# KirillKryukov/naf

Measured on AMD Instinct MI355X. Metric: unnaf GB/s (uncompressed bases out) on 100 GB synthetic FASTA, higher is better.
Workload: dtype u8; 1 GPU; unnaf decode of a 100.0 GB synthetic-ACGT FASTA archive on one GPU (the size BASELINE.json's metric is quoted on; configs[1] at 10 GB rides along as cfg10_*), 100 records, 80-col lines; archive made in-run by the GPU ennaf; .naf 24739662224 B -> FASTA 99999995684 B, text + archive + decoded text resident in HBM; parallelism=one archive, one GPU, no data-path collective

## Files before the change

naf_amd/csrc/ctx.h:

```cpp
#pragma once
#include "common.h"
#include "../../include/naf_gpu.h"
#include <hip/hip_runtime.h>
#include <stdio.h>
#include <stdarg.h>
#include <vector>
#include <functional>
#include <string>

struct ArenaChunk { u8 *base; size_t cap, used; };

struct KTime { const char *name; hipEvent_t a, b; };

#define ZSPLIT_MAX 8
struct ZSplit { int parts; hipEvent_t ev[ZSPLIT_MAX]; u64 out_end[ZSPLIT_MAX]; int done; void *status; };
struct FlatStream { u64 q0, A; };
#define FLAT_DECODED (~0ull)
struct ZFlat { const u8 *src; const FlatStream *si; u64 nslots; const u8 *sym; void *status; bool ready;
               const u8 *tail; u64 tail_q; u32 tail_n;
               const u8 *cls; u32 n_decoded; u32 n_walk;
               struct naf_gpu_ctx *aux; hipEvent_t decoded_ev; void *later; };
struct CtxOpts { std::vector<std::pair<std::string, std::string>> kv; std::string trace; bool tracing = false; };
struct naf_gpu_ctx {
    int device = 0;
    CtxOpts *opts = nullptr;
    naf_gpu_ctx *root = nullptr;
    hipStream_t stream = nullptr;
    bool own_stream = false;
    std::vector<ArenaChunk> chunks;
    size_t high_water = 0;
    u8 *h_stage = nullptr;
    size_t h_stage_cap = 0;
    void *d_predef = nullptr;
    void *d_seqctab = nullptr;
    char err[512] = {0};
    bool timing = false;
    std::vector<KTime> ktimes;
    std::vector<hipEvent_t> ev_pool;
    size_t ev_used = 0;
    std::vector<std::string> agg_names; std::vector<float> agg_ms; std::vector<int> agg_n;
    float stream_ms[5] = { 0, 0, 0, 0, 0 };
    naf_gpu_ctx *side = nullptr;
    naf_gpu_ctx *side2 = nullptr;
    naf_gpu_ctx *side3 = nullptr;
    naf_gpu_ctx *side4 = nullptr;
    void *sides_thread = nullptr; int sides_rc = 0;
    hipEvent_t fork_ev = nullptr;
    struct ZSplit *zsplit = nullptr;
    hipEvent_t split_ev[ZSPLIT_MAX + 2] = {};
    struct ZFlat *zflat = nullptr;
    void *io_pool = nullptr;
    void *shard_state = nullptr;
    struct HostWorker *worker = nullptr;
};

void ctx_worker_start(naf_gpu_ctx *x, std::function<void()> job);
void ctx_worker_join(naf_gpu_ctx *x);
int  ctx_sides_ready(naf_gpu_ctx *c);

int  ctx_fail(naf_gpu_ctx *c, int code, const char *fmt, ...);
const char *ctx_opt(const naf_gpu_ctx *c, const char *name);
static inline bool ctx_opt_is(const naf_gpu_ctx *c, const char *name, char v) { const char *e = ctx_opt(c, name); return e && e[0] == v; }
bool ctx_tracing(const naf_gpu_ctx *c);
void ctx_trace(naf_gpu_ctx *c, const char *fmt, ...);
#define HIP_TRY(c, call) do { hipError_t e_ = (call); if (e_ != hipSuccess) return ctx_fail((c), NAF_GPU_EHIP, "%s: %s (%s:%d)", #call, hipGetErrorString(e_), __FILE__, __LINE__); } while (0)

void  arena_reset(naf_gpu_ctx *c);
void *arena_alloc(naf_gpu_ctx *c, size_t bytes);
void  arena_settle(naf_gpu_ctx *c);
template <typename T> T *arena_new(naf_gpu_ctx *c, size_t n) { return (T *)arena_alloc(c, n * sizeof(T)); }

int ctx_readback(naf_gpu_ctx *c, void *h_dst, const void *d_src, size_t bytes);
int ctx_readback2(naf_gpu_ctx *c, void *h1, const void *d1, size_t n1, void *h2, const void *d2, size_t n2);
int ctx_readbackv(naf_gpu_ctx *c, int n, void *const *h, const void *const *d, const size_t *bytes);

void ktime_begin(naf_gpu_ctx *c, const char *name);
void ktime_end(naf_gpu_ctx *c);

#define LAUNCH(c, name, kern, grid, block, shmem, ...) do { \
    ktime_begin((c), name); \
    hipLaunchKernelGGL(kern, dim3(grid), dim3(block), (shmem), (c)->stream, __VA_ARGS__); \
    ktime_end((c)); } while (0)

static inline u32 cdiv(u64 a, u64 b) { return (u32)((a + b - 1) / b); }

int scan_exclusive_u64(naf_gpu_ctx *c, u64 *d_vals, size_t n, u64 *d_total);
int scan_inclusive_max_i32(naf_gpu_ctx *c, i32 *d_vals, size_t n);
int scan_inclusive_max_i64(naf_gpu_ctx *c, i64 *d_vals, size_t n);
int scan_exclusive_u64_multi(naf_gpu_ctx *c, u64 *const *arrs, int k, size_t n, u64 *const *totals);
int scan_inclusive_max_i64_multi(naf_gpu_ctx *c, i64 *const *arrs, int k, size_t n);

int zstd_decode(naf_gpu_ctx *c, const u8 *d_src, size_t src_len, int has_magic, u8 *d_dst, size_t dst_cap, size_t *out_len, const u8 *head = nullptr);
int zstd_init_tables(naf_gpu_ctx *c);
void ennaf_shard_state_free(naf_gpu_ctx *c);
void io_pool_free(naf_gpu_ctx *c);
struct EmitP;
int zstd_decode_fused_fasta(naf_gpu_ctx *c, const u8 *d_src, size_t src_len, int has_magic, size_t *out_len, const EmitP *P, u8 *text);
struct ZRange { u64 want_lo, want_hi, got_lo, got_hi; bool ranged; u8 *own_buf; };
int zstd_decode_range(naf_gpu_ctx *c, const u8 *d_src, size_t src_len, int has_magic, u8 *d_dst, size_t dst_cap, size_t *out_len, ZRange *rg, const u8 *head = nullptr);
int zstd_split_status(naf_gpu_ctx *c, const ZSplit *sp);
int zstd_flat_later(naf_gpu_ctx *c, ZFlat *zf);
void zstd_flat_drop(ZFlat *zf);
int zstd_small_batch(naf_gpu_ctx *c, int n, const u8 *const *src, const size_t *len, u8 *const *dst, const size_t *cap, bool *ok);
bool zstd_small_fits(size_t len, size_t cap);
int zstd_small_launch(naf_gpu_ctx *c, int n, const u8 *const *src, const size_t *len, u8 *const *dst, const size_t *cap, u32 **d_res_out);
enum { ZENC_PART = 16, ZENC_PART_FIRST = 32, ZENC_PART_LAST = 64, ZENC_PREFER_RAW = 128, ZENC_PREFER_FLAT = 256, ZENC_SHORT_CODES = 512, ZENC_FRAME_TREE = 1024 };
int zenc_level_window(int level);
int zenc_repeat_probe(naf_gpu_ctx *c, const u8 *d_src, size_t n, u32 *share_1024);
static inline u32 zenc_probe_every(u64 n) { u32 e = 64; while (((n >> 20) / e) > 128) e <<= 1; return e; }
struct ZencPlace { u8 *(*fn)(void *ud, size_t frame_len); void *ud; };
struct ZencJob;
#define ZENC_LOC_BND 20
struct ZencLoc { const u8 *loc; const i32 *blk_bnd; const u32 *blk_t0; u64 tiles; };
int zstd_encode_begin(naf_gpu_ctx *c, const u8 *d_src, size_t n, int level, int with_magic, int lz, int block_log_hint, int window_log, ZencJob **job, const u8 *direct = nullptr, u32 nd = 0, const ZencLoc *dloc = nullptr);
int zstd_encode_finish(naf_gpu_ctx *c, ZencJob *job, u8 *d_dst, size_t cap, size_t *out_len, const ZencPlace *place);
void zstd_encode_drop(ZencJob *job);
int zstd_encode_size(naf_gpu_ctx *c, ZencJob *job, size_t *frame_len);
const u64 *zstd_encode_total_ptr(const ZencJob *job);
void zstd_encode_set_total(ZencJob *job, u64 total);
int zstd_encode(naf_gpu_ctx *c, const u8 *d_src, size_t n, int level, u8 *d_dst, size_t cap, size_t *out_len, int with_magic, int lz = 0, int block_log_hint = 0, int window_log = 0, const ZencPlace *place = nullptr);
```

naf_amd/csrc/emit.hip:

```cpp
#include "ctx.h"
#include "wgscan.h"
#include "emit_core.h"
#include <thread>

__device__ __forceinline__ void st_text16(u8 *p, const uint4 &v, int nt)
{
    if (nt) {
        typedef unsigned int u32x4_t __attribute__((ext_vector_type(4)));
        u32x4_t nv; nv.x = v.x; nv.y = v.y; nv.z = v.z; nv.w = v.w;
        __builtin_nontemporal_store(nv, (u32x4_t *)p);
    } else *(uint4 *)p = v;
}

__global__ void k_len_flags(const u32 *units, u64 n, u64 *flag)
{
    u64 i = (u64)blockIdx.x * blockDim.x + threadIdx.x;
    if (i < n) flag[i] = units[i] != 0xFFFFFFFFu;
}
__global__ void k_len_acc(const u32 *units, u64 n, const u64 *ridx, u64 *rec_len, u64 N)
{
    u64 i = (u64)blockIdx.x * blockDim.x + threadIdx.x;
    if (i < n && ridx[i] < N) atomicAdd((unsigned long long *)&rec_len[ridx[i]], (unsigned long long)units[i]);
}

// ... 414 lines not shown
        if (k.qual_copy) { uint4 v; v.x = (u32)a; v.y = (u32)(a >> 32); v.z = (u32)b; v.w = (u32)(b >> 32); memcpy(o, &v, 16); return; }
        if (k.fast) {
            u64 lo, hi, g0 = k.g0;
            if (FOURBIT) { u64 nib = a; if (g0 & 1) nib = (nib >> 4) | (b << 60); expand16(P.lut, nib, lo, hi); }
            else {
                lo = a; hi = b;
                if (P.upper) {
                    auto up = [](u64 v) { u64 r = 0; for (int i = 0; i < 8; i++) { u32 c = (v >> (8 * i)) & 0xFF; if (c >= 'a' && c <= 'z') c -= 32; r |= (u64)c << (8 * i); } return r; };
                    lo = up(lo); hi = up(hi);
                }
            }
            if (any_toggle) {
                u64 kk = upper_bound_u64(P.toggles, klo, khi, g0);
                u32 state = (u32)(kk & 1), m16 = 0; u64 pos = g0;
                for (;;) {
                    u64 nxt = kk < khi ? P.toggles[kk] : ~0ull;
                    u64 end = nxt < g0 + 16 ? nxt : g0 + 16;
                    if (state && end > pos) m16 |= (u32)(((1u << (end - pos)) - 1) << (pos - g0));
                    if (nxt >= g0 + 16) break;
                    pos = nxt; state ^= 1; kk++;
                }
                lo += spread_bits8(m16 & 0xFF); hi += spread_bits8(m16 >> 8);
            } else if (P.masking && (klo & 1)) { lo += 0x2020202020202020ull; hi += 0x2020202020202020ull; }
            if (k.nl_b < 16) splice_newline(lo, hi, k.nl_b);
            u64 j15 = k.j0 + 15 - (15 > k.nl_b ? 1 : 0);
            if (j15 >= k.len) hi = (hi & 0x00FFFFFFFFFFFFFFull) | ((u64)'\n' << 56);
            uint4 v; v.x = (u32)lo; v.y = (u32)(lo >> 32); v.z = (u32)hi; v.w = (u32)(hi >> 32);
            memcpy(o, &v, 16);
            return;
        }
        for (u32 bb = 0; bb < k.nbytes; bb++) o[bb] = (u8)emit_byte<FOURBIT>(P, k.p0 + bb, rlo, rhi, klo, khi);
    };
    for (u64 tile = span_first; tile <= span_last; tile += 8192) {
        Chunk ka = prep(tile), kb = prep(tile + 4096);
        u64 a0, a1, b0, b1;
        fetch(ka, a0, a1); fetch(kb, b0, b1);
        finish(ka, a0, a1); finish(kb, b0, b1);
    }
}

#define ES_SPAN (32u * 1024u)
#define ES_CAP 1024

__device__ __forceinline__ void place16(u64 &lo, u64 &hi, u64 slo, u64 shi, u32 pos, u32 n)
{
    if (n <= 8) { shi = 0; slo &= low_bytes_mask((int)n); } else if (n < 16) shi &= low_bytes_mask((int)n - 8);
    if (pos == 0) { lo |= slo; hi |= shi; }
    else if (pos < 8) { lo |= slo << (8 * pos); hi |= (shi << (8 * pos)) | (slo >> (64 - 8 * pos)); }
    else if (pos == 8) hi |= slo;
    else hi |= slo << (8 * (pos - 8));
}

__device__ __forceinline__ void mask16_from(const u64 *tog, u32 n, u64 klo, u64 g0, u64 &lo, u64 &hi)
{
    u32 a = 0, b = n;
    while (a < b) { u32 mid = (a + b) >> 1; if (tog[mid] <= g0) a = mid + 1; else b = mid; }
    u32 kk = a, state = (u32)((klo + kk) & 1), m16 = 0; u64 pos = g0;
    for (;;) {
        u64 nxt = kk < n ? tog[kk] : ~0ull;
        u64 end = nxt < g0 + 16 ? nxt : g0 + 16;
        if (state && end > pos) m16 |= (u32)(((1u << (end - pos)) - 1) << (pos - g0));
        if (nxt >= g0 + 16) break;
        pos = nxt; state ^= 1; kk++;
    }
    lo += spread_bits8(m16 & 0xFF); hi += spread_bits8(m16 >> 8);
}
__device__ __forceinline__ void mask16(const EmitP &P, u64 klo, u64 khi, bool any_toggle, u64 g0, u64 &lo, u64 &hi)
{
    if (any_toggle) {
        if (khi - klo <= 0x7FFFFFFFull) mask16_from(P.toggles + klo, (u32)(khi - klo), klo, g0, lo, hi);
        else {
            u64 kk = upper_bound_u64(P.toggles, klo, khi, g0);
            u32 state = (u32)(kk & 1), m16 = 0; u64 pos = g0;
            for (;;) {
                u64 nxt = kk < khi ? P.toggles[kk] : ~0ull;
                u64 end = nxt < g0 + 16 ? nxt : g0 + 16;
                if (state && end > pos) m16 |= (u32)(((1u << (end - pos)) - 1) << (pos - g0));
                if (nxt >= g0 + 16) break;
                pos = nxt; state ^= 1; kk++;
            }
            lo += spread_bits8(m16 & 0xFF); hi += spread_bits8(m16 >> 8);
        }
    } else if (P.masking && (klo & 1)) { lo += 0x2020202020202020ull; hi += 0x2020202020202020ull; }
}

__device__ __forceinline__ void span_windows(const EmitP &P, u64 span_first, u64 span_last, u64 *sh)
{
    if (threadIdx.x < 2 && P.mode != EM_SEQ) {
        u64 p = threadIdx.x == 0 ? span_first : span_last;
        sh[threadIdx.x] = upper_bound_u64(P.rec_out, 0, P.N + 1, p) - 1;
    }
    __syncthreads();
    if (threadIdx.x < 2) {
        u64 k = 0;
        if (P.masking) {
            u64 g;
            if (P.mode == EM_SEQ) g = threadIdx.x == 0 ? span_first : span_last + 1;
            else g = threadIdx.x == 0 ? P.rec_base[sh[0]] : P.rec_base[sh[1] + 1];
            if (P.mode != EM_SEQ && threadIdx.x == 0) {
                u64 r = sh[0], off = span_first - P.rec_out[r], hl = P.hdr_len[r];
                if (off > hl) { u64 q = off - hl; u64 j = (P.mode == EM_FASTA && P.L) ? (q / (P.L + 1)) * P.L : (P.mode == EM_FASTQ ? 0 : q); if (j > P.rec_len[r]) j = P.rec_len[r]; g += j; }
            }
            k = upper_bound_u64(P.toggles, 0, P.n_toggles, g);
        }
        sh[2 + threadIdx.x] = k;
    }
    __syncthreads();
}

__global__ void k_hdr_len64(const u32 *hdr_len, u64 r0, u64 n, u64 *out)
{
    u64 i = (u64)blockIdx.x * blockDim.x + threadIdx.x;
    if (i < n) out[i] = hdr_len[r0 + i];
}
__device__ __forceinline__ void store_upto16(u8 *p, u64 lo, u64 hi, u32 n)
{
    if (n >= 16) { uint4 v; v.x = (u32)lo; v.y = (u32)(lo >> 32); v.z = (u32)hi; v.w = (u32)(hi >> 32); memcpy(p, &v, 16); return; }
    if (n & 8) { st64(p, lo); p += 8; lo = hi; }
    if (n & 4) { st32(p, (u32)lo); p += 4; lo >>= 32; }
    if (n & 2) { p[0] = (u8)lo; p[1] = (u8)(lo >> 8); p += 2; lo >>= 16; }
    if (n & 1) p[0] = (u8)lo;
}
template <u32 LANES = 16>
__device__ __forceinline__ void group_copy(u8 *dst, const u8 *src, u64 n, u32 g)
{
    for (u64 i = (u64)g * 16; i < n; i += LANES * 16) {
        u64 lo = ld64(src + i), hi = ld64(src + i + 8);
        store_upto16(dst + i, lo, hi, n - i < 16 ? (u32)(n - i) : 16u);
    }
}

__global__ __launch_bounds__(256) void k_hdr_build(EmitP P, u64 r0, u64 n, const u64 *hdr_off, u8 *text)
{
    u64 i = (u64)blockIdx.x * 32 + (threadIdx.x >> 3);
    u32 g = threadIdx.x & 7;
    if (i >= n) return;
    u64 r = r0 + i; u32 hl = P.hdr_len[r];
    u8 *o = text + hdr_off[i];
    u64 ids0 = 0, idl = 0, nm0 = 0, nml = 0;
    if (P.has_ids) { ids0 = r ? P.idz[r - 1] + 1 : 0; idl = P.idz[r] - ids0; }
    if (P.has_names) { nm0 = r ? P.nmz[r - 1] + 1 : 0; nml = P.nmz[r] - nm0; }
    if (g == 0) { o[0] = P.hdr_char; o[hl - 1] = '\n'; }
    if (P.has_ids) {
        group_copy<8>(o + 1, P.ids + ids0, idl, g);
        if (P.has_names && nml) { if (g == 0) o[1 + idl] = P.sep; group_copy<8>(o + 2 + idl, P.names + nm0, nml, g); }
    } else group_copy<8>(o + 1, P.names + nm0, nml, g);
}

template <bool FOURBIT, typename Geo>
__device__ __forceinline__ void compose_chunk(const EmitP &P, Geo &geo, u64 p0, u32 nbytes, u64 r, u64 klo, u64 khi, bool any_toggle, u32 Lp1_32, u8 *o)
{
    const bool hdrs = P.hdr_text != nullptr;
    u64 ro, rn, len, base, ho; u32 hl;
    geo(r, ro, rn, len, base, ho, hl);
    u64 lo = 0, hi = 0; u32 pos = 0;
    while (pos < nbytes) {
        u64 p = p0 + pos;
        while (p >= rn) { r++; geo(r, ro, rn, len, base, ho, hl); }
        u64 off = p - ro;
        const u8 *src = nullptr; u64 g = 0; bool is_bases = false;
        u64 n_main = 0; u32 tc = 0, n_tc = 0;
        if (off < hl) { src = P.hdr_text + ho + off; n_main = hl - off; }
        else {
            u64 q = off - hl;
            if (P.mode == EM_FASTQ) {
                if (q < len + 3) {
                    u64 skip = 0;
                    if (q < len) { is_bases = true; g = base + q; n_main = len - q; } else skip = q - len;
                    tc = 0x0A2B0Au >> (8 * (u32)skip); n_tc = 3 - (u32)skip;
                } else { src = P.qual + base + (q - len - 3); n_main = 2 * len + 3 - q; tc = '\n'; n_tc = 1; }
            } else {
                tc = '\n'; n_tc = 1;
                if (P.mode == EM_SEQUENCES || P.L == 0) { if (q < len) { is_bases = true; g = base + q; n_main = len - q; } }
                else {
                    u64 line, col;
                    if (Lp1_32 && (q >> 32) == 0) { u32 l32 = (u32)q / Lp1_32; line = l32; col = (u32)q - l32 * Lp1_32; }
                    else { line = q / (P.L + 1); col = q - line * (P.L + 1); }
                    u64 j = line * P.L + col;
                    if (col != P.L && j < len) { is_bases = true; g = base + j; n_main = len - j < P.L - col ? len - j : P.L - col; }
                }
            }
        }
        u32 rem = nbytes - pos;
        u32 n1 = n_main < rem ? (u32)n_main : rem;
        if (n1) {
            u64 slo, shi;
            if (is_bases) { bases16<FOURBIT>(P, g, slo, shi); if (P.mode != EM_FASTQ) mask16(P, klo, khi, any_toggle, g, slo, shi); }
            else if (!hdrs && off < hl) {
                slo = shi = 0;
                for (u32 b = 0; b < n1; b++) { u64 ch = header_char(P, r, off + b, hl); if (b < 8) slo |= ch << (8 * b); else shi |= ch << (8 * (b - 8)); }
            }
            else { slo = ld64(src); shi = n1 > 8 ? ld64(src + 8) : 0; }
            place16(lo, hi, slo, shi, pos, n1);
            pos += n1; rem -= n1;
        }
        if (n1 == n_main && rem && n_tc) { u32 n2 = n_tc < rem ? n_tc : rem; place16(lo, hi, tc, 0, pos, n2); pos += n2; }
    }
    if (nbytes == 16) { uint4 v; v.x = (u32)lo; v.y = (u32)(lo >> 32); v.z = (u32)hi; v.w = (u32)(hi >> 32); memcpy(o, &v, 16); }
    else for (u32 b = 0; b < nbytes; b++) o[b] = (u8)((b < 8 ? lo >> (8 * b) : hi >> (8 * (b - 8))) & 0xFF);
}

struct GeoGlobal {
    const EmitP &P;
    __device__ GeoGlobal(const EmitP &p) : P(p) {}
    __device__ __forceinline__ void operator()(u64 r, u64 &ro, u64 &rn, u64 &len, u64 &base, u64 &ho, u32 &hl) const
    { ro = P.rec_out[r]; rn = P.rec_out[r + 1]; len = P.rec_len[r]; base = P.rec_base[r]; hl = P.hdr_len[r]; ho = P.hdr_text ? P.hdr_off[r - P.hdr_r0] : 0; }
};

template <bool FOURBIT>
__global__ __launch_bounds__(256) void k_emit_short(EmitP P, u8 *out)
{
    __shared__ u64 sh[4];
    __shared__ u64 s_ro[ES_CAP + 1], s_len[ES_CAP], s_base[ES_CAP], s_ho[ES_CAP];
    __shared__ u32 s_hl[ES_CAP];
    u64 span_first = P.out_begin + (u64)blockIdx.x * ES_SPAN, span_last = span_first + ES_SPAN - 1;
    if (span_last >= P.out_end) span_last = P.out_end - 1;
    span_windows(P, span_first, span_last, sh);
    const u64 rlo = sh[0], rhi = sh[1], klo = sh[2], khi = sh[3];
    const bool any_toggle = P.masking && klo < khi;
    const u64 nrec = rhi - rlo + 1;
    const bool in_lds = nrec <= ES_CAP;
    const bool hdrs = P.hdr_text != nullptr;
    if (in_lds) {
        for (u32 i = threadIdx.x; i < (u32)nrec; i += 256) {
            u64 r = rlo + i; s_ro[i] = P.rec_out[r]; s_len[i] = P.rec_len[r]; s_base[i] = P.rec_base[r]; s_hl[i] = P.hdr_len[r];
            s_ho[i] = hdrs ? P.hdr_off[r - P.hdr_r0] : 0;
        }
        if (threadIdx.x == 0) s_ro[nrec] = P.rec_out[rhi + 1];
        __syncthreads();
    }
    const u32 Lp1_32 = (P.L + 1) >> 32 ? 0 : (u32)(P.L + 1);
    auto geo_lds = [&](u64 r, u64 &ro, u64 &rn, u64 &len, u64 &base, u64 &ho, u32 &hl) {
        u32 i = (u32)(r - rlo); ro = s_ro[i]; rn = s_ro[i + 1]; len = s_len[i]; base = s_base[i]; hl = s_hl[i]; ho = s_ho[i];
    };
    GeoGlobal geo_g(P);
    for (u64 tile = span_first; tile <= span_last; tile += 4096) {
        u64 p0 = tile + (u64)threadIdx.x * 16;
        if (p0 > span_last) continue;
        u32 nbytes = P.out_end - p0 < 16 ? (u32)(P.out_end - p0) : 16;
        u8 *o = out + (p0 - P.out_begin);
        if (in_lds) {
            u32 lo_ = 0, hi_ = (u32)nrec; while (lo_ < hi_) { u32 mid = (lo_ + hi_) >> 1; if (s_ro[mid] <= p0) lo_ = mid + 1; else hi_ = mid; }
            compose_chunk<FOURBIT>(P, geo_lds, p0, nbytes, rlo + lo_ - 1, klo, khi, any_toggle, Lp1_32, o);
        } else {
            u64 r = upper_bound_u64(P.rec_out, rlo, rhi + 1, p0) - 1;
            compose_chunk<FOURBIT>(P, geo_g, p0, nbytes, r, klo, khi, any_toggle, Lp1_32, o);
        }
    }
}

#define ER_STAGE 24576u
template <bool FOURBIT, u32 ER_LANES, u32 WGT>
__global__ __launch_bounds__(WGT) void k_emit_fastq_records(EmitP P, u8 *out)
{
    constexpr u32 ER_READS = WGT / ER_LANES, STAGE = ER_STAGE / (256u / WGT);
    __shared__ __attribute__((aligned(16))) u8 stage[STAGE + 32];
    const u32 g = threadIdx.x & (ER_LANES - 1);
    const u64 r0 = (u64)blockIdx.x * ER_READS, r = r0 + threadIdx.x / ER_LANES;
    const u64 rend = r0 + ER_READS < P.N ? r0 + ER_READS : P.N;
    const u64 wbase = P.rec_out[r0], wspan = P.rec_out[rend] - wbase;
    const bool in_lds = wspan <= STAGE;
    if (r < P.N) {
        const u64 len = P.rec_len[r], base = P.rec_base[r];
        const u32 hl = P.hdr_len[r];
        u8 *o = in_lds ? stage + (P.rec_out[r] - wbase) : out + P.rec_out[r];
        u64 ids0 = 0, idl = 0, nm0 = 0, nml = 0;
        if (P.has_ids) { ids0 = r ? P.idz[r - 1] + 1 : 0; idl = P.idz[r] - ids0; }
        if (P.has_names) { nm0 = r ? P.nmz[r - 1] + 1 : 0; nml = P.nmz[r] - nm0; }
        if (g == 0) { o[0] = P.hdr_char; o[hl - 1] = '\n'; }
        if (P.has_ids) {
            group_copy<ER_LANES>(o + 1, P.ids + ids0, idl, g);
            if (P.has_names && nml) { if (g == 0) o[1 + idl] = P.sep; group_copy<ER_LANES>(o + 2 + idl, P.names + nm0, nml, g); }
        } else group_copy<ER_LANES>(o + 1, P.names + nm0, nml, g);
        u8 *os = o + hl;
        for (u64 i = (u64)g * 16; i < len; i += 16 * ER_LANES) {
            u64 lo, hi; bases16<FOURBIT>(P, base + i, lo, hi);
            store_upto16(os + i, lo, hi, len - i < 16 ? (u32)(len - i) : 16u);
        }
        if (g == 0) { os[len] = '\n'; os[len + 1] = '+'; os[len + 2] = '\n'; os[2 * len + 3] = '\n'; }
        group_copy<ER_LANES>(os + len + 3, P.qual + base, len, g);
    }
    if (!in_lds) return;
    __syncthreads();
    u8 *dst = out + wbase; const u32 n = (u32)wspan;
    u32 head = (u32)((16 - ((uintptr_t)dst & 15)) & 15); if (head > n) head = n;
    if (threadIdx.x < head) dst[threadIdx.x] = stage[threadIdx.x];
    u32 words = (n - head) >> 4;
    for (u32 w = threadIdx.x; w < words; w += WGT) {
        u64 a, b2; __builtin_memcpy(&a, stage + head + 16 * w, 8); __builtin_memcpy(&b2, stage + head + 16 * w + 8, 8);
        uint4 v; v.x = (u32)a; v.y = (u32)(a >> 32); v.z = (u32)b2; v.w = (u32)(b2 >> 32);
        st_text16(dst + head + 16 * w, v, P.nt_store);
    }
    for (u32 k = head + 16 * words + threadIdx.x; k < n; k += WGT) dst[k] = stage[k];
}

#define EMIT_TOG_LDS 256u
struct TileIdx { u64 gline, k, khi; u32 col, fast; };
#define TI_HDR 0xFFFFFFFFu
struct TileFlat { u64 q0, A, q1, A1, q2, qf; };
struct TileFlatE { u64 base, a1_addr; u32 a1_sh, K0, K1, d1, d2, qoff, par0, pad; };
static_assert(sizeof(TileFlatE) == sizeof(TileFlat), "the derived record replaces the raw one in place");
#define FLAT_QM 4096
#define TILE_WG 255
__global__ __launch_bounds__(256) void k_tile_index(EmitP P, u64 ntiles, TileIdx *ti, u64 *tr, u32 *list, u32 *count, TileFlat *tsig, u32 spare, u32 *list2)
{
    __shared__ u64 s_k[256], s_r[256];
    const u64 t = (u64)blockIdx.x * TILE_WG + threadIdx.x;
    const u64 p = P.out_begin + t * 4096;
    TileIdx x; x.fast = 0; x.gline = 0; x.khi = 0; x.k = P.n_toggles; x.col = TI_HDR;
    TileFlat f; f.q0 = f.A = f.q1 = f.A1 = f.q2 = f.qf = 0;
    u64 r = ~0ull; u32 cbits = 1;
    const bool inside = t < ntiles && p < P.out_end;
    if (inside) {
        u64 g;
        if (P.mode == EM_SEQ) { r = 0; x.col = 0; g = p; x.gline = p; }
        else {
            r = upper_bound_u64(P.rec_out, 0, P.N + 1, p) - 1;
            u64 off = p - P.rec_out[r], hl = P.hdr_len[r], len = P.rec_len[r], j = 0;
            if (off >= hl) {
                u64 q = off - hl;
                if (P.mode == EM_FASTA && P.L) {
                    u64 line = q / (P.L + 1), col = q - line * (P.L + 1);
                    j = line * P.L + (col < P.L ? col : P.L);
                    if (P.L < 0xFFFFFFF0ull) { x.gline = P.rec_base[r] + line * P.L; x.col = (u32)col; }
                } else if (P.mode != EM_FASTQ) { j = q; x.col = 0; x.gline = P.rec_base[r] + q; }
                if (j > len) j = len;
            }
            g = P.rec_base[r] + j;
        }
        x.k = P.masking ? upper_bound_u64(P.toggles, 0, P.n_toggles, g) : 0;
        if (tsig) {
            const FlatStream *si = (const FlatStream *)P.fsi;
            const u64 q = g >> 1;
            u64 lo, hi, gs = q >> 13; if (gs >= P.fslots) gs = P.fslots - 1;
            if (si[gs].q0 <= q) { lo = gs; hi = gs + 1; u64 st = 1; while (hi < P.fslots && si[hi].q0 <= q) { lo = hi; st <<= 1; hi = lo + st; } if (hi > P.fslots) hi = P.fslots; }
            else { hi = gs; u64 st = 1; lo = gs - 1; while (lo > 0 && si[lo].q0 > q) { hi = lo; st <<= 1; lo = lo > st ? lo - st : 0; } }
            while (hi - lo > 1) { const u64 mid = (lo + hi) >> 1; if (si[mid].q0 <= q) lo = mid; else hi = mid; }
            f.q0 = si[lo].q0; f.A = si[lo].A; f.qf = q;
            if (P.fcls) {
                u32 c = 3; u64 b = lo >> 2; const u64 nb = P.fslots >> 2, qe = q + 2048 + 16;
                for (u32 k = 0; k < 6 && b < nb && si[4 * b].q0 <= qe; k++, b++) c &= P.fcls[b];
                if (b < nb && si[4 * b].q0 <= qe) c = 0;
                cbits = c;
            }
            u64 cs = lo + 1;
            while (cs < P.fslots && si[cs + 1].q0 == si[cs].q0) cs++;
            f.q1 = si[cs].q0; f.A1 = cs < P.fslots ? si[cs].A : 0;
            u64 ce = cs < P.fslots ? cs + 1 : cs;
            while (ce < P.fslots && si[ce + 1].q0 == si[ce].q0) ce++;
            f.q2 = si[ce].q0;
        }
    }
    s_k[threadIdx.x] = x.k; s_r[threadIdx.x] = r;
    __syncthreads();
    if (threadIdx.x == TILE_WG) return;
    TileFlatE e; e.base = (u64)P.fsrc; e.a1_addr = (u64)P.fsrc; e.a1_sh = 4; e.K0 = e.K1 = 0; e.d1 = e.d2 = 0x7FFFFFFFu; e.qoff = 0; e.par0 = 0; e.pad = 0;
    if (t >= ntiles) {
        if (t == ntiles) { tr[t] = ~0ull; ti[t] = x; if (tsig && spare) *(TileFlatE *)&tsig[t] = e; }
        else if (tsig && t < ntiles + spare) { ti[t].fast = 0; *(TileFlatE *)&tsig[t] = e; }
        return;
    }
    tr[t] = r;
    if (!inside) { ti[t] = x; if (tsig) *(TileFlatE *)&tsig[t] = e; list[atomicAdd(count, 1u)] = (u32)t; return; }
    const u64 r_next = s_r[threadIdx.x + 1];
    x.khi = s_k[threadIdx.x + 1];
    const bool wrap = P.mode == EM_FASTA && P.L != 0;
    bool fast = x.col != TI_HDR && r == r_next && P.out_begin + (t + 1) * 4096 <= P.out_end && !P.force_slow && (!wrap || P.L >= 16);
    bool packed = false;
    if (tsig) {
        packed = fast && (cbits & 2);
        if (fast && !(cbits & 1)) fast = false;
        if (fast) {
            fast = f.qf + 2048 + 16 < f.q2 || f.q2 == f.q1;
            if (P.ftail && f.qf + 2048 + 16 >= P.ftail_q) fast = false;
            if (f.q2 != f.q1 && (f.A1 > f.A ? f.A1 - f.A : f.A - f.A1) >= (1ull << 29)) fast = false;
        }
        if (fast) {
            const u64 gline = x.gline;
            const u64 dd1 = f.q1 - f.qf, dd2 = f.q2 - f.qf;
            e.d1 = dd1 > 0x7FFFFFFFull ? 0x7FFFFFFFu : (u32)dd1; e.d2 = dd2 > 0x7FFFFFFFull ? 0x7FFFFFFFu : (u32)dd2;
            const u64 T0 = f.A - 4 * (f.qf - f.q0), T1 = f.A1 + 4 * (u64)e.d1;
            const bool two = f.q2 != f.q1;
            const u64 tmin = two && T1 < T0 ? T1 : T0;
            const u64 ub = (tmin - 40 - 4 * (u64)FLAT_QM) & ~7ull;
            e.base = (u64)P.fsrc + (u64)((i64)ub >> 3);
            e.K0 = (u32)(T0 - 40 - ub); e.K1 = two ? (u32)(T1 - 40 - ub) : e.K0;
            e.qoff = (u32)((gline >> 1) - f.qf); e.par0 = (u32)gline & 1u;
            const u64 t1 = (f.A1 < 40 ? 40 : f.A1) - 40;
            e.a1_addr = (u64)P.fsrc + (t1 >> 3); e.a1_sh = (u32)(t1 & 7) + 4;
        }
        *(TileFlatE *)&tsig[t] = e;
    }
    x.fast = fast ? 1u : (packed ? 2u : 0u);
    ti[t] = x;
    if (!fast) { if (packed) list2[atomicAdd(count + 1, 1u)] = (u32)t; else list[atomicAdd(count, 1u)] = (u32)t; }
}

template <bool FOURBIT>
__device__ __forceinline__ void emit_tile_body(const EmitP &P, const TileIdx &a, u8 *out_tile)
{
    __shared__ u64 s_tog[EMIT_TOG_LDS];
    const u32 ntog = (u32)(a.khi - a.k < EMIT_TOG_LDS ? a.khi - a.k : EMIT_TOG_LDS);
    const bool use_tog = P.masking && a.k < a.khi && a.khi - a.k <= EMIT_TOG_LDS;
    if (use_tog) { for (u32 i = threadIdx.x; i < ntog; i += 256) s_tog[i] = P.toggles[a.k + i]; __syncthreads(); }
    const u32 lane16 = threadIdx.x * 16;
    u64 g0; u32 nl_b = 64;
    if (P.mode == EM_FASTA && P.L != 0) {
        const u32 Lp1 = (u32)P.L + 1;
        u32 c = a.col + lane16, dl;
        if (Lp1 < 32768) dl = __umulhi(c, P.Ldiv_magic); else dl = c >= Lp1 ? 1u : 0u;
        u32 col = c - dl * Lp1;
        g0 = a.gline + (u64)dl * (u32)P.L + col;
        u32 d = (u32)P.L - col;
        nl_b = d < 16 ? d : 64;
    } else g0 = a.gline + lane16;
    u64 lo, hi;
    if (FOURBIT) {
        u64 addr = (u64)P.seq + (g0 >> 1);
        const uint4 q = ldg_at<uint4>(addr & ~7ull);
        u64 q0 = (u64)q.x | ((u64)q.y << 32), q1 = (u64)q.z | ((u64)q.w << 32);
        u32 sh = (u32)(addr & 7) * 8 + (u32)(g0 & 1) * 4;
        expand16(P.lut, sh ? (q0 >> sh) | (q1 << (64 - sh)) : q0, lo, hi);
    } else bases16<false>(P, g0, lo, hi);
    if (use_tog) mask16_from(s_tog, ntog, a.k, g0, lo, hi);
    else mask16(P, a.k, a.khi, P.masking && a.k < a.khi, g0, lo, hi);
    if (nl_b < 16) splice_newline(lo, hi, (int)nl_b);
    uint4 v; v.x = (u32)lo; v.y = (u32)(lo >> 32); v.z = (u32)hi; v.w = (u32)(hi >> 32);
    st_text16(out_tile + lane16, v, P.nt_store);
}
template <bool FOURBIT>
__global__ __launch_bounds__(256) void k_emit_tile(EmitP P, const TileIdx *ti, u8 *out)
{
    const TileIdx a = ti[blockIdx.x];
    if (a.fast != 1) return;
    emit_tile_body<FOURBIT>(P, a, out + (u64)blockIdx.x * 4096);
}
template <bool FOURBIT, u32 TW>
__device__ __forceinline__ void emit_tiles_wave(const EmitP &P, const TileIdx *ti, u8 *out, const u64 (&tn)[TW], u32 want, u64 (*s_tog)[EMIT_TOG_LDS])
{
    const u32 lane = threadIdx.x;
    TileIdx A[TW]; bool live[TW];
#pragma unroll
    for (u32 j = 0; j < TW; j++) { A[j] = ti[tn[j] == ~0ull ? 0 : tn[j]]; live[j] = tn[j] != ~0ull && A[j].fast == want; }
    u64 g0s[TW][4]; u32 nls[TW][4]; uint4 Q[TW][4];
#pragma unroll
    for (u32 j = 0; j < TW; j++) {
        const TileIdx &a = A[j];
#pragma unroll
        for (u32 r = 0; r < 4; r++) {
            const u32 lane16 = (r * 64 + lane) * 16;
            u64 g0; u32 nl_b = 64;
            if (P.mode == EM_FASTA && P.L != 0) {
                const u32 Lp1 = (u32)P.L + 1;
                u32 c = a.col + lane16, dl;
                if (Lp1 < 32768) dl = __umulhi(c, P.Ldiv_magic); else dl = c >= Lp1 ? 1u : 0u;
                u32 col = c - dl * Lp1;
                g0 = a.gline + (u64)dl * (u32)P.L + col;
                u32 d = (u32)P.L - col;
                nl_b = d < 16 ? d : 64;
            } else g0 = a.gline + lane16;
            g0s[j][r] = g0; nls[j][r] = nl_b;
            if (FOURBIT) Q[j][r] = live[j] ? ldg_at<uint4>(((u64)P.seq + (g0 >> 1)) & ~7ull) : make_uint4(0, 0, 0, 0);
        }
    }
    if (P.masking) {
#pragma unroll
        for (u32 j = 0; j < TW; j++) {
            const u64 nt = A[j].khi - A[j].k;
            for (u32 i = lane; i < EMIT_TOG_LDS; i += 64) s_tog[j][i] = (live[j] && i < nt && nt <= EMIT_TOG_LDS) ? P.toggles[A[j].k + i] : 0ull;
        }
        __syncthreads();
    }
#pragma unroll
    for (u32 j = 0; j < TW; j++) {
        if (!live[j]) continue;
        const TileIdx &a = A[j];
        const u32 ntog = (u32)(a.khi - a.k < EMIT_TOG_LDS ? a.khi - a.k : EMIT_TOG_LDS);
        const bool use_tog = P.masking && a.k < a.khi && a.khi - a.k <= EMIT_TOG_LDS;
#pragma unroll
        for (u32 r = 0; r < 4; r++) {
            const u64 g0 = g0s[j][r];
            u64 lo, hi;
            if (FOURBIT) {
                const u64 addr = (u64)P.seq + (g0 >> 1);
                const uint4 q = Q[j][r];
                const u64 q0 = (u64)q.x | ((u64)q.y << 32), q1 = (u64)q.z | ((u64)q.w << 32);
                const u32 sh = (u32)(addr & 7) * 8 + (u32)(g0 & 1) * 4;
                expand16(P.lut, sh ? (q0 >> sh) | (q1 << (64 - sh)) : q0, lo, hi);
            } else bases16<false>(P, g0, lo, hi);
            if (use_tog) mask16_from(s_tog[j], ntog, a.k, g0, lo, hi);
            else mask16(P, a.k, a.khi, P.masking && a.k < a.khi, g0, lo, hi);
            if (nls[j][r] < 16) splice_newline(lo, hi, (int)nls[j][r]);
            uint4 v; v.x = (u32)lo; v.y = (u32)(lo >> 32); v.z = (u32)hi; v.w = (u32)(hi >> 32);
            st_text16(out + tn[j] * 4096 + (r * 64 + lane) * 16, v, P.nt_store);
        }
    }
}
template <bool FOURBIT, u32 TW>
__global__ __launch_bounds__(64) void k_emit_tile_wave(EmitP P, const TileIdx *ti, u8 *out, u64 ntiles)
{
    __shared__ u64 s_tog[TW][EMIT_TOG_LDS];
    u64 tn[TW];
#pragma unroll
    for (u32 j = 0; j < TW; j++) { const u64 t = (u64)blockIdx.x * TW + j; tn[j] = t < ntiles ? t : ~0ull; }
    emit_tiles_wave<FOURBIT, TW>(P, ti, out, tn, 1u, s_tog);
}
template <bool FOURBIT>
__global__ __launch_bounds__(64) void k_emit_tile_list_wave(EmitP P, const TileIdx *ti, const u32 *list, const u32 *count, u8 *out)
{
    __shared__ u64 s_tog[1][EMIT_TOG_LDS];
    const u32 n = *count;
    for (u32 i = blockIdx.x; i < n; i += gridDim.x) {
        const u64 tn[1] = { list[i] };
        emit_tiles_wave<FOURBIT, 1>(P, ti, out, tn, 2u, s_tog);
        __syncthreads();
    }
}
template <bool FOURBIT>
__global__ __launch_bounds__(256) void k_emit_tile_list(EmitP P, const TileIdx *ti, const u32 *list, const u32 *count, u8 *out)
{
    const u32 n = *count;
    for (u32 i = blockIdx.x; i < n; i += gridDim.x) {
        const u32 t = list[i];
        const TileIdx a = ti[t];
        emit_tile_body<FOURBIT>(P, a, out + (u64)t * 4096);
        __syncthreads();
    }
}

__global__ void k_flat_pair(EmitP P, u32 *pair)
{
    const u32 t = threadIdx.x;
    {
        const u32 pa = P.fsym[t >> 4], pb = P.fsym[t & 15];
        pair[16 + t] = expand_codes4(P.lut, (pa & 15u) | ((pa >> 4) << 8) | ((pb & 15u) << 16) | ((pb >> 4) << 24));
        if (t < 16) {
            const u32 d = t; u32 sel[4], orv[4];
            for (u32 i = 0; i < 4; i++) {
                sel[i] = 0; orv[i] = 0;
                for (u32 j = 0; j < 4; j++) { const u32 q = 4 * i + j; sel[i] |= (q < d ? 4 + j : (q == d ? 0x0Cu : 3 + j)) << (8 * j); if (q == d) orv[i] |= 0x0Au << (8 * j); }
            }
            for (u32 i = 0; i < 4; i++) { pair[272 + 8 * d + i] = sel[i]; pair[272 + 8 * d + 4 + i] = orv[i]; }
        }
    }
    if (t >= 12) return;
    const u8 *lut = (const u8 *)P.lut;
    u32 v = 0;
    for (u32 k = 0; k < 4; k++) {
        const u32 pk = P.fsym[4 * (t & 3) + k];
        const u32 b = t < 4 ? pk : (t < 8 ? lut[pk & 15] : lut[pk >> 4]);
        v |= b << (8 * k);
    }
    pair[t] = v;
}
#define FLAT_TPW 8
template <u32 TPW>
__global__ __launch_bounds__(256) void k_emit_tile_flat(EmitP P, const TileIdx *ti, const TileFlat *tsig, u8 *out, u64 ntiles, u32 xcd_chunk)
{
    u32 wg = blockIdx.x;
    if (xcd_chunk) { wg = (blockIdx.x & 7u) * xcd_chunk + (blockIdx.x >> 3); if ((u64)wg * TPW >= ntiles) return; }
    __shared__ u64 s_tog[TPW][EMIT_TOG_LDS];
    __shared__ uint4 s_spl[32];
    if (threadIdx.x < 16) {
        const u32 d = threadIdx.x; u32 sel[4], orv[4];
        for (u32 i = 0; i < 4; i++) {
            sel[i] = 0; orv[i] = 0;
            for (u32 j = 0; j < 4; j++) { const u32 p = 4 * i + j; sel[i] |= (p < d ? 4 + j : (p == d ? 0x0Cu : 3 + j)) << (8 * j); if (p == d) orv[i] |= 0x0Au << (8 * j); }
        }
        s_spl[2 * d] = make_uint4(sel[0], sel[1], sel[2], sel[3]); s_spl[2 * d + 1] = make_uint4(orv[0], orv[1], orv[2], orv[3]);
    }
    __shared__ u32 s_pair[256];
    {
        const u32 pa = P.fsym[threadIdx.x >> 4], pb = P.fsym[threadIdx.x & 15];
        s_pair[threadIdx.x] = expand_codes4(P.lut, (pa & 15u) | ((pa >> 4) << 8) | ((pb & 15u) << 16) | ((pb >> 4) << 24));
    }
    const u32 lane16 = threadIdx.x * 16;
    TileIdx A[TPW]; TileFlatE F[TPW]; bool live[TPW];
    {
        static_assert(sizeof(TileIdx) == 32 && sizeof(TileFlatE) == 48, "records are read as 16-byte words");
        const u64 t0 = (u64)wg * TPW;
        const uint4 *pa = (const uint4 *)(ti + t0), *pf = (const uint4 *)(tsig + t0);
        uint4 ra[2 * TPW], rf[3 * TPW];
#pragma unroll
        for (u32 i = 0; i < 2 * TPW; i++) ra[i] = pa[i];
#pragma unroll
        for (u32 i = 0; i < 3 * TPW; i++) rf[i] = pf[i];
#pragma unroll
        for (u32 j = 0; j < TPW; j++) {
            __builtin_memcpy(&A[j], &ra[2 * j], 32); __builtin_memcpy(&F[j], &rf[3 * j], 48);
            live[j] = t0 + j < ntiles && A[j].fast == 1;
        }
    }
    u64 X[TPW]; u32 offs[TPW], grels[TPW], nls[TPW], haves[TPW];
#pragma unroll
    for (u32 j = 0; j < TPW; j++) {
        const TileIdx &a = A[j]; const TileFlatE &e = F[j];
        u32 grel, nl_b = 64;
        if (P.mode == EM_FASTA && P.L != 0) {
            const u32 Lp1 = (u32)P.L + 1;
            u32 c = a.col + lane16, dl;
            if (Lp1 < 32768) dl = __umulhi(c, P.Ldiv_magic); else dl = c >= Lp1 ? 1u : 0u;
            u32 col = c - dl * Lp1;
            grel = dl * (u32)P.L + col;
            u32 d = (u32)P.L - col;
            nl_b = d < 16 ? d : 64;
        } else grel = lane16;
        grels[j] = grel; nls[j] = nl_b;
        const u32 par = e.par0 + grel;
        const u32 need = 8 + (par & 1u);
        const u32 qrel = (par >> 1) + e.qoff;
        const bool second = qrel >= e.d1;
        const u32 qm = live[j] ? ~0u : 0u;
        const u32 off = (second ? e.K1 : e.K0) - ((4 * qrel) & qm);
        const u32 rem = (second ? e.d2 : e.d1) - qrel;
        X[j] = ldg_at_unaligned<u64>(e.base + (off >> 3));
        offs[j] = off;
        haves[j] = need > rem ? rem : 16u;
    }
    if (P.masking) {
        u64 tg[TPW];
#pragma unroll
        for (u32 j = 0; j < TPW; j++) {
            const u64 nt = A[j].khi - A[j].k;
            tg[j] = (live[j] && threadIdx.x < nt && nt <= EMIT_TOG_LDS) ? P.toggles[A[j].k + threadIdx.x] : 0ull;
        }
#pragma unroll
        for (u32 j = 0; j < TPW; j++) s_tog[j][threadIdx.x] = tg[j];
    }
    __syncthreads();
#pragma unroll
    for (u32 j = 0; j < TPW; j++) {
        const u64 t = (u64)wg * TPW + j;
        if (!live[j]) continue;
        const TileIdx &a = A[j];
        const u64 g0 = a.gline + grels[j];
        u64 h36 = X[j] >> ((offs[j] & 7) + 4);
        if (haves[j] < 9) {
            const u64 y = ldg_at_unaligned<u64>(F[j].a1_addr);
            const u64 n36 = (y >> F[j].a1_sh) & 0xFFFFFFFFFull;
            const u32 keep = 4 * haves[j];
            h36 = (h36 & ~(0xFFFFFFFFFull >> keep)) | (n36 >> keep);
        }
        const u32 h = (u32)(h36 >> 4), n9 = (u32)h36 & 15u;
        u64 lo, hi;
        {
            u32 w0 = s_pair[h >> 24], w1 = s_pair[(h >> 16) & 0xFFu], w2 = s_pair[(h >> 8) & 0xFFu], w3 = s_pair[h & 0xFFu];
            if (g0 & 1) {
                const u32 c9 = s_pair[n9 << 4];
                w0 = __builtin_amdgcn_alignbyte(w1, w0, 1); w1 = __builtin_amdgcn_alignbyte(w2, w1, 1);
                w2 = __builtin_amdgcn_alignbyte(w3, w2, 1); w3 = __builtin_amdgcn_alignbyte(c9, w3, 1);
            }
            lo = (u64)w0 | ((u64)w1 << 32); hi = (u64)w2 | ((u64)w3 << 32);
        }
        const u32 ntog = (u32)(a.khi - a.k < EMIT_TOG_LDS ? a.khi - a.k : EMIT_TOG_LDS);
        const bool use_tog = P.masking && a.k < a.khi && a.khi - a.k <= EMIT_TOG_LDS;
        if (use_tog) mask16_from(s_tog[j], ntog, a.k, g0, lo, hi);
        else mask16(P, a.k, a.khi, P.masking && a.k < a.khi, g0, lo, hi);
        uint4 v; v.x = (u32)lo; v.y = (u32)(lo >> 32); v.z = (u32)hi; v.w = (u32)(hi >> 32);
        if (nls[j] < 16) {
            const uint4 sel = s_spl[2 * nls[j]], orv = s_spl[2 * nls[j] + 1];
            const u32 x0 = v.x, x1 = v.y, x2 = v.z, x3 = v.w;
            v.x = __builtin_amdgcn_perm(x0, 0u, sel.x) | orv.x; v.y = __builtin_amdgcn_perm(x1, x0, sel.y) | orv.y;
            v.z = __builtin_amdgcn_perm(x2, x1, sel.z) | orv.z; v.w = __builtin_amdgcn_perm(x3, x2, sel.w) | orv.w;
        }
        st_text16(out + t * 4096 + lane16, v, P.nt_store);
    }
}

template <u32 TW>
__global__ __launch_bounds__(64) void k_emit_tile_flat_wave(EmitP P, const TileIdx *ti, const TileFlat *tsig, u8 *out, u64 ntiles, u32 xcd_chunk)
{
    u32 wg = blockIdx.x;
    if (xcd_chunk) { wg = (blockIdx.x & 7u) * xcd_chunk + (blockIdx.x >> 3); if ((u64)wg * TW >= ntiles) return; }
    __shared__ u64 s_tog[TW][EMIT_TOG_LDS];
    __shared__ uint4 s_spl[32];
    __shared__ u32 s_pair[256];
    const u32 lane = threadIdx.x;
    if (lane < 32) s_spl[lane] = ((const uint4 *)(P.fpair + 272))[lane];
    ((uint4 *)s_pair)[lane] = ((const uint4 *)(P.fpair + 16))[lane];
    TileIdx A[TW]; TileFlatE F[TW]; bool live[TW];
    {
        const u64 t0 = (u64)wg * TW;
        const uint4 *pa = (const uint4 *)(ti + t0), *pf = (const uint4 *)(tsig + t0);
        uint4 ra[2 * TW], rf[3 * TW];
#pragma unroll
        for (u32 i = 0; i < 2 * TW; i++) ra[i] = pa[i];
#pragma unroll
        for (u32 i = 0; i < 3 * TW; i++) rf[i] = pf[i];
#pragma unroll
        for (u32 j = 0; j < TW; j++) {
            __builtin_memcpy(&A[j], &ra[2 * j], 32); __builtin_memcpy(&F[j], &rf[3 * j], 48);
            live[j] = t0 + j < ntiles && A[j].fast == 1;
        }
    }
    u64 X[TW][4]; u32 grels[TW][4], pk[TW][4];
#pragma unroll
    for (u32 j = 0; j < TW; j++) {
        const TileIdx &a = A[j]; const TileFlatE &e = F[j];
#pragma unroll
        for (u32 r = 0; r < 4; r++) {
            const u32 lane16 = (r * 64 + lane) * 16;
            u32 grel, nl_b = 64;
            if (P.mode == EM_FASTA && P.L != 0) {
                const u32 Lp1 = (u32)P.L + 1;
                u32 c = a.col + lane16, dl;
                if (Lp1 < 32768) dl = __umulhi(c, P.Ldiv_magic); else dl = c >= Lp1 ? 1u : 0u;
                u32 col = c - dl * Lp1;
                grel = dl * (u32)P.L + col;
                u32 d = (u32)P.L - col;
                nl_b = d < 16 ? d : 64;
            } else grel = lane16;
            grels[j][r] = grel;
            const u32 par = e.par0 + grel;
            const u32 need = 8 + (par & 1u);
            const u32 qrel = (par >> 1) + e.qoff;
            const bool second = qrel >= e.d1;
            const u32 qm = live[j] ? ~0u : 0u;
            const u32 off = (second ? e.K1 : e.K0) - ((4 * qrel) & qm);
            const u32 rem = (second ? e.d2 : e.d1) - qrel;
            X[j][r] = ldg_at_unaligned<u64>(e.base + (off >> 3));
            pk[j][r] = nl_b | ((need > rem ? rem : 16u) << 8) | ((off & 7u) << 16);
        }
    }
    if (P.masking) {
#pragma unroll
        for (u32 j = 0; j < TW; j++) {
            const u64 nt = A[j].khi - A[j].k;
            for (u32 i = lane; i < EMIT_TOG_LDS; i += 64) s_tog[j][i] = (live[j] && i < nt && nt <= EMIT_TOG_LDS) ? P.toggles[A[j].k + i] : 0ull;
        }
    }
    __syncthreads();
#pragma unroll
    for (u32 j = 0; j < TW; j++) {
        const u64 t = (u64)wg * TW + j;
        if (!live[j]) continue;
        const TileIdx &a = A[j];
        const u32 ntog = (u32)(a.khi - a.k < EMIT_TOG_LDS ? a.khi - a.k : EMIT_TOG_LDS);
        const bool use_tog = P.masking && a.k < a.khi && a.khi - a.k <= EMIT_TOG_LDS;
#pragma unroll
        for (u32 r = 0; r < 4; r++) {
            const u64 g0 = a.gline + grels[j][r];
            const u32 nl = pk[j][r] & 0xFFu, have = (pk[j][r] >> 8) & 0xFFu;
            u64 h36 = X[j][r] >> ((pk[j][r] >> 16) + 4);
            if (have < 9) {
                const u64 y = ldg_at_unaligned<u64>(F[j].a1_addr);
                const u64 n36 = (y >> F[j].a1_sh) & 0xFFFFFFFFFull;
                const u32 keep = 4 * have;
                h36 = (h36 & ~(0xFFFFFFFFFull >> keep)) | (n36 >> keep);
            }
            const u32 h = (u32)(h36 >> 4), n9 = (u32)h36 & 15u;
            u64 lo, hi;
            {
                u32 w0 = s_pair[h >> 24], w1 = s_pair[(h >> 16) & 0xFFu], w2 = s_pair[(h >> 8) & 0xFFu], w3 = s_pair[h & 0xFFu];
                if (g0 & 1) {
                    const u32 c9 = s_pair[n9 << 4];
                    w0 = __builtin_amdgcn_alignbyte(w1, w0, 1); w1 = __builtin_amdgcn_alignbyte(w2, w1, 1);
                    w2 = __builtin_amdgcn_alignbyte(w3, w2, 1); w3 = __builtin_amdgcn_alignbyte(c9, w3, 1);
                }
                lo = (u64)w0 | ((u64)w1 << 32); hi = (u64)w2 | ((u64)w3 << 32);
            }
            if (use_tog) mask16_from(s_tog[j], ntog, a.k, g0, lo, hi);
            else mask16(P, a.k, a.khi, P.masking && a.k < a.khi, g0, lo, hi);
            uint4 v; v.x = (u32)lo; v.y = (u32)(lo >> 32); v.z = (u32)hi; v.w = (u32)(hi >> 32);
            if (nl < 16) {
                const uint4 sel = s_spl[2 * nl], orv = s_spl[2 * nl + 1];
                const u32 x0 = v.x, x1 = v.y, x2 = v.z, x3 = v.w;
                v.x = __builtin_amdgcn_perm(x0, 0u, sel.x) | orv.x; v.y = __builtin_amdgcn_perm(x1, x0, sel.y) | orv.y;
                v.z = __builtin_amdgcn_perm(x2, x1, sel.z) | orv.z; v.w = __builtin_amdgcn_perm(x3, x2, sel.w) | orv.w;
            }
            st_text16(out + t * 4096 + (r * 64 + lane) * 16, v, P.nt_store);
        }
    }
}

template <bool FOURBIT>
__device__ __forceinline__ void emit_rest_tile(const EmitP &P, const TileIdx *ti, const u64 *tr, u64 t, u8 *out, u32 chunk)
{
    const TileIdx a = ti[t];
    u64 p0 = P.out_begin + t * 4096 + chunk * 16;
    if (p0 >= P.out_end) return;
    u32 nbytes = P.out_end - p0 < 16 ? (u32)(P.out_end - p0) : 16;
    const u32 Lp1_32 = (P.L + 1) >> 32 ? 0 : (u32)(P.L + 1);
    u8 *o = out + (p0 - P.out_begin);
    if (P.mode == EM_SEQ) {
        for (u32 bb = 0; bb < nbytes; bb++) o[bb] = (u8)emit_byte<FOURBIT>(P, p0 + bb, 0, 0, a.k, a.khi);
        return;
    }
    u64 rlo = tr[t], rhi = tr[t + 1] == ~0ull ? P.N - 1 : tr[t + 1];
    u64 r = upper_bound_u64(P.rec_out, rlo, rhi + 1, p0) - 1;
    GeoGlobal geo_g(P);
    compose_chunk<FOURBIT>(P, geo_g, p0, nbytes, r, a.k, a.khi, P.masking && a.k < a.khi, Lp1_32, o);
}
#define EMIT_REST_GRID 4096
template <bool FOURBIT>
__global__ __launch_bounds__(64) void k_emit_rest(EmitP P, const TileIdx *ti, const u64 *tr, const u32 *list, const u32 *count, u8 *out)
{
    const u32 n = *count;
    for (u32 i = blockIdx.x; i < 4 * n; i += gridDim.x) emit_rest_tile<FOURBIT>(P, ti, tr, list[i >> 2], out, (i & 3) * 64 + threadIdx.x);
}

__global__ void k_range_bases(EmitP P, u64 *out2)
{
    if (threadIdx.x || blockIdx.x) return;
    if (P.mode == EM_SEQ) { out2[0] = P.out_begin; out2[1] = P.out_end; out2[2] = out2[3] = 0; return; }
    u64 pb = P.out_begin, pe = P.out_end - 1;
    u64 r0 = upper_bound_u64(P.rec_out, 0, P.N + 1, pb) - 1, r1 = upper_bound_u64(P.rec_out, 0, P.N + 1, pe) - 1;
    out2[2] = r0; out2[3] = r1;
    auto lower = [&](u64 r, u64 p) -> u64 {
        u64 off = p - P.rec_out[r], hl = P.hdr_len[r], len = P.rec_len[r];
        if (off <= hl) return 0;
        u64 q = off - hl, j;
        if (P.mode == EM_FASTQ) j = 0;
        else if (P.mode == EM_FASTA && P.L) j = (q / (P.L + 1)) * P.L;
        else j = q;
        return j > len ? len : j;
    };
    auto upper = [&](u64 r, u64 p) -> u64 {
        u64 off = p - P.rec_out[r], hl = P.hdr_len[r], len = P.rec_len[r];
        if (off < hl) return 0;
        u64 q = off - hl, j;
        if (P.mode == EM_FASTQ) j = len;
        else if (P.mode == EM_FASTA && P.L) j = (q / (P.L + 1) + 1) * P.L;
        else j = q + 1;
        return j > len ? len : j;
    };
    out2[0] = P.rec_base[r0] + lower(r0, pb);
    out2[1] = P.rec_base[r1] + upper(r1, pe);
}

__global__ void k_last_nonempty(const u64 *rec_len, u64 N, unsigned long long *out)
{
    u64 r = (u64)blockIdx.x * blockDim.x + threadIdx.x;
    if (r < N && rec_len[r]) atomicMax(out, (unsigned long long)(r + 1));
}
template <bool FOURBIT>
__global__ void k_emit_surplus(EmitP P, u64 base0, u64 S, u64 cc, u64 L, int wrap, u64 lo, u64 hi, u8 *out)
{
    const u64 j = lo + (u64)blockIdx.x * blockDim.x + threadIdx.x;
    if (j >= hi) return;
    u64 g; bool nl = false;
    if (!wrap || L == 0 || S <= cc) g = base0 + j;
    else if (j < cc) g = base0 + j;
    else if (j == cc) { nl = true; g = 0; }
    else { const u64 j2 = j - cc - 1, line = j2 / (L + 1), col = j2 - line * (L + 1); if (col == L) { nl = true; g = 0; } else g = base0 + cc + line * L + col; }
    u32 ch = '\n';
    if (!nl) { ch = base_char<FOURBIT>(P, g); if (P.masking && base_masked(P, g, 0, P.n_toggles)) ch += 32; }
    out[j - lo] = (u8)ch;
}

static int zero_positions(naf_gpu_ctx *c, const u8 *d_buf, u64 n, u64 N, u64 **out, bool names)
{
    u64 *pos = arena_new<u64>(c, N + 1);
    if (!pos) return NAF_GPU_ENOMEM;
    u64 tiles = (n + ZT_TILE - 1) / ZT_TILE;
    u64 *cnt = arena_new<u64>(c, tiles + 2);
    if (!cnt) return NAF_GPU_ENOMEM;
    u64 *d_total = cnt + tiles + 1;
    if (tiles) LAUNCH(c, "unnaf_zero_count", k_zero_count, tiles, 256, 0, d_buf, n, cnt);
    int rc = scan_exclusive_u64(c, cnt, tiles, d_total); if (rc) return rc;
    u64 total = 0;
    rc = ctx_readback(c, &total, d_total, 8); if (rc) return rc;
    if (total < N) return ctx_fail(c, NAF_GPU_EFORMAT, names ? "corrupted names - can't read name %llu\n" : "currupted ids - can't read id %llu\n", (unsigned long long)total);
    if (tiles) LAUNCH(c, "unnaf_zero_scatter", k_zero_scatter, tiles, 256, 0, d_buf, n, (const u64 *)cnt, pos, N);
    *out = pos;
    return 0;
}

enum { H_OK = 0, H_EMPTY, H_TRUNC, H_MAGIC, H_VERSION, H_SEQTYPE, H_SEPARATOR, H_VLE_LEAD, H_VLE_OVERFLOW, H_SANE_SECTION , H_SANE_COUNT = H_SANE_SECTION + 6 };
struct ContainerOut { naf_gpu_header h; int code; u8 frame_head[6][24]; };
NAF_HD int naf_parse_container(const u8 *p, size_t len, naf_gpu_header *h)
{
    size_t pos = 0;
    memset(h, 0, sizeof *h);
    if (len == 0) return H_EMPTY;
    if (len < 3) return H_TRUNC;
    if (p[0] != 0x01 || p[1] != 0xF9 || p[2] != 0xEC) return H_MAGIC;
    pos = 3;
    if (pos >= len) return H_TRUNC;
    h->version = p[pos++];
    if (h->version < 1 || h->version > 2) return H_VERSION;
    h->seq_type = NAF_SEQ_DNA;
    if (h->version > 1) {
        if (pos >= len) return H_TRUNC;
        int t = p[pos++];
        h->seq_type = t;
        if (t < 1 || t > 3) return H_SEQTYPE;
    }
    if (len - pos < 2) return H_TRUNC;
    h->flags = p[pos++]; h->separator = p[pos++];
    if (h->separator < 0x20 || h->separator > 0x7E) return H_SEPARATOR;
    int e = 0;
    auto rd = [&](u64 *v) -> int {
        u64 a = 0; if (pos >= len) return H_TRUNC;
        u8 ch = p[pos++];
        if (ch == 128) return H_VLE_LEAD;
        while (ch & 128) { if (a & (127ull << 57)) return H_VLE_OVERFLOW; a = (a << 7) | (ch & 127); if (pos >= len) return H_TRUNC; ch = p[pos++]; }
        if (a & (127ull << 57)) return H_VLE_OVERFLOW;
        *v = (a << 7) | ch; return 0;
    };
    if ((e = rd(&h->line_length)) || (e = rd(&h->n_sequences))) return e;
    if (h->flags & 0x40) { if ((e = rd(&h->title_len))) return e; h->title_off = pos; if (h->title_len > len - pos) return H_TRUNC; pos += h->title_len; }
    const int bit[6] = { 0x20, 0x10, 0x08, 0x04, 0x02, 0x01 };
    for (int i = 0; i < 6; i++) {
        if (!(h->flags & bit[i])) continue;
        if ((e = rd(&h->orig_size[i])) || (e = rd(&h->comp_size[i]))) return e;
        if (h->comp_size[i] > len - pos) return H_TRUNC;
        h->payload_off[i] = pos; pos += h->comp_size[i];
    }
    for (int i = 0; i < 6; i++) {
        const u64 cs = h->comp_size[i] + 4;
        const u64 lim = cs > (1ull << 46) ? ~0ull : cs << (i == 4 ? 17 : 16);
        if (h->orig_size[i] > lim) return H_SANE_SECTION + i;
    }
    if (h->n_sequences > ((u64)len << 16)) return H_SANE_COUNT;
    return H_OK;
}
static void container_error_text(int code, const naf_gpu_header *h, char *buf, size_t cap)
{
    static const char *what[6] = { "can't decompress ids\n", "can't decompress names\n", "can't decompress lengths\n", "can't decompress mask\n",
                                   "can't decompress sequence\n", "can't decompress quality\n" };
    switch (code) {
    case H_EMPTY: snprintf(buf, cap, "empty input"); break;
    case H_TRUNC: snprintf(buf, cap, "incomplete or truncated input\n"); break;
    case H_MAGIC: snprintf(buf, cap, "not a NAF format\n"); break;
    case H_VERSION: snprintf(buf, cap, "unknown version (%d) of NAF format\n", h->version); break;
    case H_SEQTYPE: snprintf(buf, cap, "unknown sequence type (%d) found in NAF file\n", h->seq_type); break;
    case H_SEPARATOR: snprintf(buf, cap, "unsupported name separator character\n"); break;
    case H_VLE_LEAD: snprintf(buf, cap, "invalid input: error parsing variable length encoded number\n"); break;
    case H_VLE_OVERFLOW: snprintf(buf, cap, "invalid input: overflow reading a variable length encoded number\n"); break;
    case H_SANE_COUNT: snprintf(buf, cap, "corrupted header: more sequences than the archive can describe\n"); break;
    default: if (code >= H_SANE_SECTION && code < H_SANE_SECTION + 6) snprintf(buf, cap, "%s", what[code - H_SANE_SECTION]); else snprintf(buf, cap, "malformed NAF header\n");
    }
}

extern "C" int naf_gpu_parse_header_host(const void *h_naf, size_t len, naf_gpu_header *h, char errbuf[128])
{
    if (!h) return NAF_GPU_EARG;
    const int code = naf_parse_container((const u8 *)h_naf, len, h);
    if (!code) return 0;
    if (errbuf) container_error_text(code, h, errbuf, 128);
    return NAF_GPU_EFORMAT;
}

__global__ void k_parse_container(const u8 *d, u64 len, ContainerOut *out)
{
    if (threadIdx.x || blockIdx.x) return;
    out->code = naf_parse_container(d, (size_t)len, &out->h);
    for (int i = 0; i < 6; i++) {
        const u64 n = out->code ? 0 : (out->h.comp_size[i] < 24 ? out->h.comp_size[i] : 24);
        for (u64 k = 0; k < 24; k++) out->frame_head[i][k] = k < n ? d[out->h.payload_off[i] + k] : 0;
    }
}

static int parse_container_device(naf_gpu_ctx *c, const void *d_naf, size_t len, ContainerOut *co)
{
    ContainerOut *d_co = arena_new<ContainerOut>(c, 1); if (!d_co) return NAF_GPU_ENOMEM;
    LAUNCH(c, "unnaf_parse_container", k_parse_container, 1, 64, 0, (const u8 *)d_naf, (u64)len, d_co);
    int rc = ctx_readback(c, co, d_co, sizeof *co); if (rc) return rc;
    if (co->code) { char buf[160]; container_error_text(co->code, &co->h, buf, sizeof buf); return ctx_fail(c, NAF_GPU_EFORMAT, "%s", buf); }
    return 0;
}

extern "C" int naf_gpu_parse_header(naf_gpu_ctx *c, const void *d_naf, size_t len, naf_gpu_header *h)
{
    if (!c || !h) return NAF_GPU_EARG;
    arena_reset(c);
    ContainerOut co;
    int rc = parse_container_device(c, d_naf, len, &co);
    *h = co.h;
    return rc;
}

enum { S_IDS = 0, S_NAMES, S_LEN, S_MASK, S_SEQ, S_QUAL };

struct UnnafPlan {
    naf_gpu_header h; u8 frame_head[6][24]; EmitP P; u64 total; bool fourbit; bool empty;
    u64 seq_bytes; bool need_qual;
    u64 main_total, surplus, sur_c, sur_base0;
};

static int load_section(naf_gpu_ctx *c, const u8 *d_naf, const naf_gpu_header &h, int i, u64 expect, const char *what, u8 **out, const u8 *head = nullptr)
{
    u8 *buf = (u8 *)arena_alloc(c, expect + 32);
    if (!buf) return NAF_GPU_ENOMEM;
    size_t n = 0;
    int rc = zstd_decode(c, d_naf + h.payload_off[i], h.comp_size[i], 0, buf, expect, &n, head);
    if (rc == NAF_GPU_ECAP || (rc == 0 && n != expect)) return ctx_fail(c, NAF_GPU_EFORMAT, "can't decompress %s\n", what);
    if (rc) return rc;
    *out = buf;
    return 0;
}

static int unnaf_prepare(naf_gpu_ctx *c, const u8 *d_naf, size_t naf_len, const naf_gpu_unnaf_opts *o, UnnafPlan &pl)
{
    ContainerOut co;
    int rc = parse_container_device(c, d_naf, naf_len, &co); if (rc) return rc;
    pl.h = co.h; memcpy(pl.frame_head, co.frame_head, sizeof pl.frame_head);
    const naf_gpu_header &h = pl.h;
    EmitP &P = pl.P; memset(&P, 0, sizeof P);
    int has_mask = (h.flags >> 2) & 1, has_data = (h.flags >> 1) & 1, has_qual = h.flags & 1;
    int mode = o->out_type == NAF_OUT_DEFAULT ? (has_qual ? NAF_OUT_FASTQ : NAF_OUT_FASTA) : o->out_type;
    pl.empty = false; pl.total = 0; pl.need_qual = false; pl.main_total = pl.surplus = pl.sur_c = pl.sur_base0 = 0;
    pl.fourbit = h.seq_type <= NAF_SEQ_RNA;
    u64 N = h.n_sequences, T = h.orig_size[S_SEQ];
    pl.seq_bytes = pl.fourbit ? (T + 1) / 2 : T;
    if (N == 0 || !has_data) { pl.empty = true; return 0; }
    if (mode == NAF_OUT_FASTQ && !has_qual) return ctx_fail(c, NAF_GPU_EFORMAT, "FASTQ output requested, but input has no qualities\n");
    if (mode == NAF_OUT_4BIT) {
        if (!pl.fourbit) return ctx_fail(c, NAF_GPU_EFORMAT, "input has no 4-bit encoded data, but %s sequences\n", h.seq_type == NAF_SEQ_PROTEIN ? "protein" : "text");
        P.mode = -1; pl.total = pl.main_total = pl.seq_bytes; return 0;
    }
    P.mode = mode == NAF_OUT_FASTA ? EM_FASTA : mode == NAF_OUT_FASTQ ? EM_FASTQ : mode == NAF_OUT_SEQ ? EM_SEQ : EM_SEQUENCES;
    P.N = N; P.T = T;
    P.L = o->line_length >= 0 ? (u64)o->line_length : h.line_length;
    P.sep = h.separator; P.hdr_char = P.mode == EM_FASTQ ? '@' : '>';
    P.masking = o->use_mask && has_mask && P.mode != EM_FASTQ && pl.fourbit;
    P.upper = !pl.fourbit && !o->use_mask;
    const char *tab = h.seq_type == NAF_SEQ_RNA ? "-UGKCYSBAWRDMHVN" : "-TGKCYSBAWRDMHVN";
    memcpy(P.lut, tab, 16);
    const char *fs = ctx_opt(c, "FORCE_SLOW"); P.force_slow = fs && fs[0] == '1';
    P.nt_store = 1;
    pl.need_qual = P.mode == EM_FASTQ;

    return 0;
}

template <typename Hook>
static int unnaf_sections_main(naf_gpu_ctx *c, const u8 *d_naf, UnnafPlan &pl, naf_gpu_ctx *aux, Hook early, bool early_has_work, naf_gpu_ctx *aux_names)
{
    const naf_gpu_header &h = pl.h;
    EmitP &P = pl.P;
    int has_ids = (h.flags >> 5) & 1, has_names = (h.flags >> 4) & 1, has_len = (h.flags >> 3) & 1;
    u64 N = h.n_sequences, T = h.orig_size[S_SEQ];
    int rc;
    if (P.mode == EM_SEQ) {
        pl.total = pl.main_total = T;
    } else {
        if (!has_len) return ctx_fail(c, NAF_GPU_EFORMAT, "archive has no lengths");
        P.has_ids = 0; P.has_names = 0;
        const bool want_names = P.mode == EM_FASTA || P.mode == EM_FASTQ;
        if (want_names) { P.has_ids = has_ids; P.has_names = has_names; }
        u8 *pre[3] = { nullptr, nullptr, nullptr };
        auto small3 = [&](naf_gpu_ctx *x) -> int {
            const int sec[3] = { S_IDS, S_NAMES, S_LEN }; const bool wanted[3] = { want_names && has_ids != 0, want_names && has_names != 0, true };
            const u8 *src[3]; size_t len[3], cap[3]; u8 *dst[3]; bool ok[3]; int idx[3], m = 0;
            for (int k = 0; k < 3; k++) {
                if (!wanted[k] || h.orig_size[sec[k]] == 0) continue;
                u8 *b = (u8 *)arena_alloc(x, h.orig_size[sec[k]] + 32); if (!b) return NAF_GPU_ENOMEM;
                src[m] = d_naf + h.payload_off[sec[k]]; len[m] = h.comp_size[sec[k]]; dst[m] = b; cap[m] = h.orig_size[sec[k]]; idx[m++] = k;
            }
            if (!m) return 0;
            int r = zstd_small_batch(x, m, src, len, dst, cap, ok); if (r) return r;
            for (int q = 0; q < m; q++) if (ok[q]) pre[idx[q]] = dst[q];
            return 0;
        };
        auto ids_names = [&](naf_gpu_ctx *x, int which = 3) -> int {
            int r;
            if ((which & 1) && want_names && has_ids) {
                u8 *b = pre[0]; u64 *z = nullptr;
                if (h.orig_size[S_IDS] == 0) return ctx_fail(x, NAF_GPU_EFORMAT, "corrupted ids - not 0-terminated\n");
                if (!b && (r = load_section(x, d_naf, h, S_IDS, h.orig_size[S_IDS], "ids", &b, pl.frame_head[S_IDS]))) return r;
                if ((r = zero_positions(x, b, h.orig_size[S_IDS], N, &z, false))) return r;
                P.ids = b; P.idz = z;
            }
            if ((which & 2) && want_names && has_names) {
                u8 *b = pre[1]; u64 *z = nullptr;
                if (h.orig_size[S_NAMES] == 0) return ctx_fail(x, NAF_GPU_EFORMAT, "corrupted names - not 0-terminated\n");
                if (!b && (r = load_section(x, d_naf, h, S_NAMES, h.orig_size[S_NAMES], "names", &b, pl.frame_head[S_NAMES]))) return r;
                if ((r = zero_positions(x, b, h.orig_size[S_NAMES], N, &z, true))) return r;
                P.names = b; P.nmz = z;
            }
            return 0;
        };
        u64 *rec_len = nullptr;
        auto lengths = [&](naf_gpu_ctx *x) -> int {
            int r;
            u8 *lens = pre[2];
            if (!lens && (r = load_section(x, d_naf, h, S_LEN, h.orig_size[S_LEN], "lengths", &lens, pl.frame_head[S_LEN]))) return r;
            u64 n_len = h.orig_size[S_LEN] / 4;
            u64 *flag = arena_new<u64>(x, n_len + 2); rec_len = arena_new<u64>(x, N + 1);
            if (!flag || !rec_len) return NAF_GPU_ENOMEM;
            HIP_TRY(x, hipMemsetAsync(rec_len, 0, (N + 1) * 8, x->stream));
            if (n_len) LAUNCH(x, "unnaf_len_flags", k_len_flags, cdiv(n_len, 256), 256, 0, (const u32 *)lens, n_len, flag);
            if ((r = scan_exclusive_u64(x, flag, n_len, flag + n_len + 1))) return r;
            if (n_len) LAUNCH(x, "unnaf_len_acc", k_len_acc, cdiv(n_len, 256), 256, 0, (const u32 *)lens, n_len, (const u64 *)flag, rec_len, N);
            u64 nrec = 0;
            if ((r = ctx_readback(x, &nrec, flag + n_len + 1, 8))) return r;
            if (nrec < N) return ctx_fail(x, NAF_GPU_EFORMAT, "corrupted lengths: %llu records described, %llu expected", (unsigned long long)nrec, (unsigned long long)N);
            return 0;
        };
        u64 tot[2] = { 0, 0 };
        bool fused_done = false;
        {
            const char *sf = ctx_opt(c, "SIDE_FUSED");
            const int sec[3] = { S_IDS, S_NAMES, S_LEN }; const bool wanted[3] = { want_names && has_ids != 0, want_names && has_names != 0, true };
            bool fits = !(sf && sf[0] == '0') && N <= SIDE_FUSED_N && h.orig_size[S_LEN] % 4 == 0;
            for (int k = 0; k < 3; k++) if (wanted[k] && !zstd_small_fits(h.comp_size[sec[k]], h.orig_size[sec[k]])) fits = false;
            for (int k = 0; k < 3; k++) if (wanted[k] && h.orig_size[sec[k]] == 0) fits = false;
            if (fits) {
                u64 st[6] = { 0, 0, 0, 0, 0, 0 };
                auto fused = [&](naf_gpu_ctx *x) -> int {
                    const u8 *src[3]; size_t len[3], cap[3]; u8 *dst[3]; u8 *buf[3] = { nullptr, nullptr, nullptr }; int m = 0, r;
                    SideJob J; memset(&J, 0, sizeof J);
                    for (int k = 0; k < 3; k++) {
                        if (!wanted[k]) continue;
                        u8 *b = (u8 *)arena_alloc(x, h.orig_size[sec[k]] + 32); if (!b) return NAF_GPU_ENOMEM;
                        src[m] = d_naf + h.payload_off[sec[k]]; len[m] = h.comp_size[sec[k]]; dst[m] = b; cap[m] = h.orig_size[sec[k]];
                        J.cap[m] = (u32)cap[m]; J.len[m] = (u32)len[m]; buf[k] = b; m++;
                    }
                    u32 *d_res = nullptr;
                    if ((r = zstd_small_launch(x, m, src, len, dst, cap, &d_res))) return r;
                    J.res = d_res; J.n_jobs = (u32)m;
                    J.ids = buf[0]; J.ids_n = h.orig_size[S_IDS]; J.names = buf[1]; J.names_n = h.orig_size[S_NAMES];
                    J.lens = (const u32 *)buf[2]; J.n_len = h.orig_size[S_LEN] / 4;
                    J.N = N; J.L = P.L; J.has_ids = P.has_ids; J.has_names = P.has_names; J.mode = P.mode;
                    J.idz = P.has_ids ? arena_new<u64>(x, N + 1) : nullptr; J.nmz = P.has_names ? arena_new<u64>(x, N + 1) : nullptr;
                    J.rec_len = arena_new<u64>(x, N + 1); J.hdr_len = arena_new<u32>(x, N + 1);
                    J.rec_out = arena_new<u64>(x, N + 2); J.rec_base = arena_new<u64>(x, N + 2); J.status = arena_new<u64>(x, 8);
                    if ((P.has_ids && !J.idz) || (P.has_names && !J.nmz) || !J.rec_len || !J.hdr_len || !J.rec_out || !J.rec_base || !J.status) return NAF_GPU_ENOMEM;
                    LAUNCH(x, "unnaf_side_tables", k_side_tables, 1, 256, 0, J);
                    if ((r = ctx_readback(x, st, J.status, sizeof st))) return r;
                    if (st[0] != 1) return 0;
                    P.ids = buf[0]; P.idz = J.idz; P.names = buf[1]; P.nmz = J.nmz;
                    P.rec_len = J.rec_len; P.hdr_len = J.hdr_len; P.rec_out = J.rec_out; P.rec_base = J.rec_base;
                    fused_done = true;
                    return 0;
                };
                int rf = 0;
                if (aux) { ctx_worker_start(aux, [&] { rf = fused(aux); }); early(); ctx_worker_join(aux); if (rf) memcpy(c->err, aux->err, sizeof c->err); }
                else rf = fused(c);
                if (rf) return rf;
                if (fused_done) {
                    if (st[3] < N) return ctx_fail(c, NAF_GPU_EFORMAT, "corrupted lengths: %llu records described, %llu expected", (unsigned long long)st[3], (unsigned long long)N);
                    if (P.has_ids && st[1] < N) return ctx_fail(c, NAF_GPU_EFORMAT, "currupted ids - can't read id %llu\n", (unsigned long long)st[1]);
                    if (P.has_names && st[2] < N) return ctx_fail(c, NAF_GPU_EFORMAT, "corrupted names - can't read name %llu\n", (unsigned long long)st[2]);
                    tot[0] = st[4]; tot[1] = st[5];
                }
            }
        }
        if (fused_done) rec_len = (u64 *)P.rec_len;
        else {
        const bool aux_run = aux && want_names && (has_ids || has_names);
        int rc_aux = 0, rc_len = 0;
        const bool len_on_aux = aux_run && early_has_work;
        int rc_small = 0;
        if (aux_run && !len_on_aux) rc_small = small3(c);
        bool names_beside = aux_run && aux_names && !len_on_aux && has_ids && has_names && h.orig_size[S_IDS] >= (1u << 20) && h.orig_size[S_NAMES] >= (1u << 20);
        { const char *nb = ctx_opt(c, "NAMES_BESIDE"); if (nb && nb[0] == '0') names_beside = false; }
        int rc_names = 0;
        if (names_beside) ctx_worker_start(aux_names, [&] { rc_names = ids_names(aux_names, 2); });
        if (aux_run) ctx_worker_start(aux, [&] { if (len_on_aux) rc_small = small3(aux); rc_aux = rc_small ? rc_small : ids_names(aux, names_beside ? 1 : 3); if (len_on_aux && !rc_small) rc_len = lengths(aux); });
        early();
        if (!aux_run) rc_small = small3(c);
        if (!len_on_aux) rc_len = rc_small ? rc_small : lengths(c);
        if (aux_run) { ctx_worker_join(aux); hipStreamSynchronize(aux->stream); }
        if (names_beside) { ctx_worker_join(aux_names); hipStreamSynchronize(aux_names->stream); }
        if (rc_len) { if (len_on_aux) memcpy(c->err, aux->err, sizeof c->err); return rc_len; }
        if (!aux_run) rc_aux = ids_names(c);
        else if (rc_aux) memcpy(c->err, aux->err, sizeof c->err);
        if (rc_aux) return rc_aux;
        if (rc_names) { memcpy(c->err, aux_names->err, sizeof c->err); return rc_names; }
        P.rec_len = rec_len;
        u32 *hdr_len = arena_new<u32>(c, N + 1);
        u64 *rec_out = arena_new<u64>(c, N + 2), *rec_base = arena_new<u64>(c, N + 2);
        if (!hdr_len || !rec_out || !rec_base) return NAF_GPU_ENOMEM;
        LAUNCH(c, "unnaf_rec_sizes", k_rec_sizes, cdiv(N, 256), 256, 0, N, (const u64 *)rec_len, P.idz, P.nmz, P.has_ids, P.has_names, P.mode, P.L, hdr_len, rec_out, rec_base);
        HIP_TRY(c, hipMemsetAsync(rec_out + N, 0, 8, c->stream));
        HIP_TRY(c, hipMemsetAsync(rec_base + N, 0, 8, c->stream));
        if ((rc = scan_exclusive_u64(c, rec_out, N + 1, (u64 *)nullptr))) return rc;
        if ((rc = scan_exclusive_u64(c, rec_base, N + 1, (u64 *)nullptr))) return rc;
        if ((rc = ctx_readback2(c, &tot[0], rec_out + N, 8, &tot[1], rec_base + N, 8))) return rc;
        P.hdr_len = hdr_len; P.rec_out = rec_out; P.rec_base = rec_base;
        }
        if (tot[1] > T) return ctx_fail(c, NAF_GPU_EFORMAT, "sum of lengths (%llu) exceeds the stored sequence length (%llu)", (unsigned long long)tot[1], (unsigned long long)T);
        if (P.mode == EM_FASTQ && h.orig_size[S_QUAL] < tot[1])
            return ctx_fail(c, NAF_GPU_EFORMAT, "corrupted quality: %llu quality codes stored for %llu bases\n", (unsigned long long)h.orig_size[S_QUAL], (unsigned long long)tot[1]);
        if (P.mode == EM_SEQUENCES && T == 0) tot[0] = 0;
        pl.total = pl.main_total = tot[0]; pl.surplus = 0; pl.sur_c = 0;
        if (tot[1] < T && P.mode != EM_FASTQ) {
            const u64 S = T - tot[1];
            u64 tail = S;
            if (P.mode == EM_FASTA) {
                unsigned long long *d_last = arena_new<unsigned long long>(c, 2); if (!d_last) return NAF_GPU_ENOMEM;
                HIP_TRY(c, hipMemsetAsync(d_last, 0, 16, c->stream));
                LAUNCH(c, "unnaf_last_nonempty", k_last_nonempty, cdiv(N, 256), 256, 0, (const u64 *)rec_len, N, d_last);
                u64 last1 = 0; if ((rc = ctx_readback(c, &last1, d_last, 8))) return rc;
                if (last1 == 0) tail = 0;
                else {
                    u64 len_last = 0; if ((rc = ctx_readback(c, &len_last, rec_len + (last1 - 1), 8))) return rc;
                    const u64 L = P.L;
                    const u64 cc = L ? ((len_last % L) ? L - len_last % L : 0) : 0;
                    pl.sur_c = cc;
                    if (L && S > cc) { const u64 R = S - cc; tail = cc + 1 + R + (R - 1) / L; }
                }
            }
            pl.surplus = tail ? S : 0; pl.sur_base0 = tot[1];
            pl.total = pl.main_total + tail;
        }
    }
    return 0;
}

static int unnaf_sections(naf_gpu_ctx *c, const u8 *d_naf, UnnafPlan &pl, naf_gpu_ctx *aux = nullptr, naf_gpu_ctx *aux_mask = nullptr, naf_gpu_ctx *aux_names = nullptr)
{
    const naf_gpu_header &h = pl.h;
    EmitP &P = pl.P;
    auto mask_part = [&](naf_gpu_ctx *x) -> int {
        int r;
        u8 *mu = nullptr; u64 n_mask = h.orig_size[S_MASK];
        {
            const char *mr = ctx_opt(c, "MASK_RLE");
            const u64 cs = h.comp_size[S_MASK];
            if (cs >= 4 && cs <= MASK_RLE_SRC && n_mask >= 2 * cs && !(mr && mr[0] == '0')) {
                const u8 fhd = pl.frame_head[S_MASK][0];
                const u32 fcs_flag = fhd >> 6, single = (fhd >> 5) & 1;
                struct { u32 hdr_size; bool ok; } fh;
                fh.hdr_size = 1 + (single ? 0 : 1) + (fcs_flag == 0 ? single : (fcs_flag == 1 ? 2 : (fcs_flag == 2 ? 4 : 8)));
                fh.ok = !(fhd & 0x0F);
                if (fh.ok && fh.hdr_size < cs) {
                    u64 *tg = arena_new<u64>(x, MASK_RLE_TOG + 1), *d_res = arena_new<u64>(x, 4);
                    if (!tg || !d_res) return NAF_GPU_ENOMEM;
                    LAUNCH(x, "unnaf_mask_rle", k_mask_rle_frame, 1, 256, (u32)((cs + 15) & ~15ull), d_naf + h.payload_off[S_MASK], (u32)cs, fh.hdr_size, n_mask, tg, MASK_RLE_TOG, d_res);
                    u64 res[3] = { 0, 0, 0 };
                    if ((r = ctx_readback(x, res, d_res, 24))) return r;
                    if (res[0] == 1) { P.toggles = tg; P.n_toggles = res[1]; return 0; }
                }
            }
        }
        if ((r = load_section(x, d_naf, h, S_MASK, n_mask, "mask", &mu, pl.frame_head[S_MASK]))) return r;
        u64 tiles = (n_mask + MT_TILE - 1) / MT_TILE;
        u64 *ts = arena_new<u64>(x, tiles + 2), *tc = arena_new<u64>(x, tiles + 2);
        if (!ts || !tc) return NAF_GPU_ENOMEM;
        if (tiles) LAUNCH(x, "unnaf_mask_count", k_mask_count, tiles, 256, 0, (const u8 *)mu, n_mask, ts, tc);
        if ((r = scan_exclusive_u64(x, ts, tiles, (u64 *)nullptr))) return r;
        if ((r = scan_exclusive_u64(x, tc, tiles, tc + tiles + 1))) return r;
        u64 ntog = 0;
        if ((r = ctx_readback(x, &ntog, tc + tiles + 1, 8))) return r;
        u64 *tg = arena_new<u64>(x, ntog + 1);
        if (!tg) return NAF_GPU_ENOMEM;
        if (tiles) LAUNCH(x, "unnaf_mask_scatter", k_mask_scatter, tiles, 256, 0, (const u8 *)mu, n_mask, (const u64 *)ts, (const u64 *)tc, tg, ntog);
        P.toggles = tg; P.n_toggles = ntog;
        return 0;
    };
    int rc_mask = 0;
    const bool mask_started = P.masking && aux_mask;
    if (mask_started) ctx_worker_start(aux_mask, [&] { rc_mask = mask_part(aux_mask); });
    bool mask_early = false; char mask_err[sizeof c->err];
    auto early = [&]() {
        if (P.masking && !mask_started && P.mode != EM_SEQ && aux) { mask_early = true; rc_mask = mask_part(c); if (rc_mask) memcpy(mask_err, c->err, sizeof c->err); }
    };
    int rc = unnaf_sections_main(c, d_naf, pl, aux, early, P.masking && !mask_started && P.mode != EM_SEQ && aux != nullptr, aux_names);
    if (mask_started) { ctx_worker_join(aux_mask); hipStreamSynchronize(aux_mask->stream); }
    if (rc) return rc;
    if (mask_started && rc_mask) { memcpy(c->err, aux_mask->err, sizeof c->err); return rc_mask; }
    if (mask_early) { if (rc_mask) { memcpy(c->err, mask_err, sizeof c->err); return rc_mask; } }
    else if (P.masking && !mask_started && (rc = mask_part(c))) return rc;
    return 0;
}

static int unnaf_run(naf_gpu_ctx *c, const u8 *d_naf, size_t naf_len, const naf_gpu_unnaf_opts *o,
                     u64 out_begin, u64 out_end, bool whole, u8 *d_out, size_t out_cap, size_t *out_len, bool size_only)
{
    if (!c || !d_naf || !o || !out_len) return NAF_GPU_EARG;
    arena_reset(c);
    if (whole && !size_only) { int rs = ctx_sides_ready(c); if (rs) return rs; }
    UnnafPlan pl;
    int rc = unnaf_prepare(c, d_naf, naf_len, o, pl); if (rc) return rc;
    if (pl.empty) { *out_len = 0; return 0; }
    const naf_gpu_header &h = pl.h;
    ZRange rgs, rgq; ZRange *prs = nullptr, *prq = nullptr;
    memset(&rgs, 0, sizeof rgs); memset(&rgq, 0, sizeof rgq);
    u8 *seq = nullptr;
    auto payload_seq = [&]() -> int {
        int r;
        u64 seq_need = prs ? (rgs.want_hi - rgs.want_lo) + 2 * 131072 + 64 : pl.seq_bytes + 64;
        if (seq_need > pl.seq_bytes + 64) seq_need = pl.seq_bytes + 64;
        seq = (u8 *)arena_alloc(c, seq_need);
        if (!seq) return NAF_GPU_ENOMEM;
        size_t n = 0;
        r = zstd_decode_range(c, d_naf + h.payload_off[S_SEQ], h.comp_size[S_SEQ], 0, seq, prs ? seq_need : pl.seq_bytes, &n, prs, pl.frame_head[S_SEQ]);
        if (r == NAF_GPU_ECAP && prs) {
            seq = (u8 *)arena_alloc(c, pl.seq_bytes + 64); if (!seq) return NAF_GPU_ENOMEM;
            r = zstd_decode(c, d_naf + h.payload_off[S_SEQ], h.comp_size[S_SEQ], 0, seq, pl.seq_bytes, &n); prs = nullptr;
        }
        if (r == NAF_GPU_ECAP || (r == 0 && n != pl.seq_bytes)) return ctx_fail(c, NAF_GPU_EFORMAT, "can't decompress sequence\n");
        if (r) return r;
        pl.P.seq = (prs && prs->ranged) ? (prs->own_buf ? prs->own_buf : seq) - prs->got_lo : seq;
        return 0;
    };
    auto payload_qual = [&](naf_gpu_ctx *qc) -> int {
        int r;
        u64 qn = h.orig_size[S_QUAL];
        u64 q_need = prq ? (rgq.want_hi - rgq.want_lo) + 2 * 131072 + 64 : qn + 64;
        if (q_need > qn + 64) q_need = qn + 64;
        u8 *q = (u8 *)arena_alloc(qc, q_need); if (!q) return NAF_GPU_ENOMEM;
        size_t qgot = 0;
        r = zstd_decode_range(qc, d_naf + h.payload_off[S_QUAL], h.comp_size[S_QUAL], 0, q, prq ? q_need : qn, &qgot, prq, pl.frame_head[S_QUAL]);
        if (r == NAF_GPU_ECAP && prq) {
            q = (u8 *)arena_alloc(qc, qn + 64); if (!q) return NAF_GPU_ENOMEM;
            r = zstd_decode(qc, d_naf + h.payload_off[S_QUAL], h.comp_size[S_QUAL], 0, q, qn, &qgot); prq = nullptr;
        }
        if (r == NAF_GPU_ECAP || (r == 0 && qgot != qn)) return ctx_fail(qc, NAF_GPU_EFORMAT, "can't decompress quality\n");
        if (r) return r;
        pl.P.qual = (prq && prq->ranged) ? (prq->own_buf ? prq->own_buf : q) - prq->got_lo : q;
        return 0;
    };
    auto payload = [&]() -> int { int r = payload_seq(); if (r) return r; return pl.need_qual ? payload_qual(c) : 0; };
    const char *fuse = ctx_opt(c, "FUSE");
    const bool fuse_on = fuse && fuse[0] == '1';
    const bool par = whole && !size_only && pl.P.mode != -1 && c->side && !fuse_on;
    bool payload_done = false;
    ZSplit split; split.parts = 0; split.done = 0; split.status = nullptr;
    ZFlat zflat; memset(&zflat, 0, sizeof zflat);
    struct FlatGuard { ZFlat *z; ~FlatGuard() { zstd_flat_drop(z); } } flat_guard{ &zflat };
    const char *ff = ctx_opt(c, "FLAT_FUSE"), *ek0 = ctx_opt(c, "EMIT");
    const bool try_flat = !size_only && pl.fourbit && !fuse_on && !pl.P.force_slow && !(ff && ff[0] == '0') && !(ek0 && ek0[0]) &&
                          (pl.P.mode == EM_FASTA || pl.P.mode == EM_SEQ || pl.P.mode == EM_SEQUENCES) && pl.P.N && h.orig_size[S_SEQ] / pl.P.N >= 16384 &&
                          (pl.P.mode != EM_FASTA || pl.P.L == 0 || pl.P.L >= 16);
    if (par) {
        arena_reset(c->side);
        HIP_TRY(c, hipEventRecord(c->fork_ev, c->stream));
        HIP_TRY(c, hipStreamWaitEvent(c->side->stream, c->fork_ev, 0));
        int rc_side = 0, rc_q = 0;
        const bool qpar = pl.need_qual && c->side2;
        if (qpar) { arena_reset(c->side2); HIP_TRY(c, hipStreamWaitEvent(c->side2->stream, c->fork_ev, 0)); }
        if (c->side3) { arena_reset(c->side3); HIP_TRY(c, hipStreamWaitEvent(c->side3->stream, c->fork_ev, 0)); }
        if (c->side4) { arena_reset(c->side4); HIP_TRY(c, hipStreamWaitEvent(c->side4->stream, c->fork_ev, 0)); }
        ctx_worker_start(c->side, [&] { rc_side = unnaf_sections(c->side, d_naf, pl, c->side3, nullptr, c->side4); });
        if (qpar) ctx_worker_start(c->side2, [&] { rc_q = payload_qual(c->side2); });
        const char *nsp = ctx_opt(c, "SPLIT");
        const int nparts = nsp ? atoi(nsp) : 4;
        if (!pl.need_qual && c->side2 && nparts >= 2 && nparts <= ZSPLIT_MAX && pl.P.mode != -1) {
            split.parts = nparts; split.done = 0;
            for (int k = 0; k < nparts; k++) split.ev[k] = c->split_ev[k];
            c->zsplit = &split;
            arena_reset(c->side2);
        }
        if (try_flat) { zflat.ready = false; zflat.aux = c->zsplit ? c->side2 : nullptr; c->zflat = &zflat; }
        rc = payload_seq();
        c->zsplit = nullptr; c->zflat = nullptr;
        if (!rc && pl.need_qual && !qpar) rc = payload_qual(c);
        ctx_worker_join(c->side);
        if (qpar) ctx_worker_join(c->side2);
        if (rc_side) { memcpy(c->err, c->side->err, sizeof c->err); return rc_side; }
        if (rc) return rc;
        if (rc_q) { memcpy(c->err, c->side2->err, sizeof c->err); return rc_q; }
        HIP_TRY(c, hipStreamSynchronize(c->side->stream));
        if (qpar) HIP_TRY(c, hipStreamSynchronize(c->side2->stream));
        payload_done = true;
    } else if (pl.P.mode != -1) {
        if ((rc = unnaf_sections(c, d_naf, pl))) return rc;
    }
    if (whole) { out_begin = 0; out_end = pl.total; }
    if (out_end > pl.total) out_end = pl.total;
    if (out_begin > out_end) out_begin = out_end;
    *out_len = out_end - out_begin;
    if (size_only) { *out_len = pl.total; return 0; }
    if (*out_len > out_cap) return ctx_fail(c, NAF_GPU_ECAP, "unnaf output needs %llu bytes, capacity %zu", (unsigned long long)*out_len, out_cap);
    if (*out_len == 0) return 0;
    const u64 m_begin = out_begin < pl.main_total ? out_begin : pl.main_total, m_end = out_end < pl.main_total ? out_end : pl.main_total;
    const bool has_main = m_end > m_begin, has_tail = out_end > pl.main_total;
    pl.P.out_begin = m_begin; pl.P.out_end = m_end;
    u64 rec0 = 0, rec1 = pl.P.N ? pl.P.N - 1 : 0;
    if (!whole && pl.P.mode != -1) {
        u64 g[4] = { pl.sur_base0, pl.sur_base0, rec1, rec1 };
        if (has_main) {
            u64 *d_g = arena_new<u64>(c, 4); if (!d_g) return NAF_GPU_ENOMEM;
            LAUNCH(c, "unnaf_range_bases", k_range_bases, 1, 64, 0, pl.P, d_g);
            if ((rc = ctx_readback(c, g, d_g, 32))) return rc;
        }
        rec0 = g[2]; rec1 = g[3];
        if (g[1] < g[0]) g[1] = g[0];
        if (has_tail) g[1] = pl.P.T;
        rgs.want_lo = pl.fourbit ? g[0] / 2 : g[0]; rgs.want_hi = pl.fourbit ? (g[1] + 1) / 2 : g[1];
        rgq.want_lo = g[0]; rgq.want_hi = g[1];
        prs = &rgs; prq = &rgq;
    }
    if (whole && pl.P.mode == EM_FASTA && pl.fourbit && (pl.P.L == 0 || pl.P.L >= 16) && !pl.P.force_slow && fuse_on && !pl.surplus) {
        size_t n2 = 0;
        rc = zstd_decode_fused_fasta(c, d_naf + h.payload_off[S_SEQ], h.comp_size[S_SEQ], 0, &n2, &pl.P, d_out);
        if (rc == 0) {
            if (n2 != pl.seq_bytes) return ctx_fail(c, NAF_GPU_EFORMAT, "can't decompress sequence\n");
            return 0;
        }
        if (rc != -100) return rc;
    }
    if (!payload_done) {
        if (try_flat) { zflat.ready = false; c->zflat = &zflat; }
        rc = payload();
        c->zflat = nullptr;
        if (rc) return rc;
    }
    if (zflat.ready) { pl.P.fsrc = zflat.src; pl.P.fsi = zflat.si; pl.P.fslots = zflat.nslots; pl.P.fsym = zflat.sym; pl.P.ftail = zflat.tail; pl.P.ftail_q = zflat.tail_q; pl.P.ftail_n = zflat.tail_n; pl.P.fcls = zflat.cls; }
    if (pl.P.mode == -1) {
        HIP_TRY(c, hipMemcpyAsync(d_out, seq + out_begin, out_end - out_begin, hipMemcpyDeviceToDevice, c->stream));
        return 0;
    }
    if (has_main) {
        const char *ek = ctx_opt(c, "EMIT");
        bool short_rec = pl.P.mode != EM_SEQ && pl.total / pl.P.N < 16384;
        if (ek && !strcmp(ek, "short")) short_rec = pl.P.mode != EM_SEQ;
        if (ek && !strcmp(ek, "long")) short_rec = false;
        if (pl.P.force_slow) { short_rec = false; ek = "span"; }
        if (whole && pl.P.mode == EM_FASTQ && !pl.P.force_slow && !(ek && ek[0])) {
            {
                const u64 avg = pl.P.N ? (pl.P.out_end - pl.P.out_begin) / pl.P.N + 1 : 1;
                const u32 lanes = avg * 64 <= ER_STAGE * 7 / 8 ? 4u : avg * 32 <= ER_STAGE * 7 / 8 ? 8u : 16u;
                const bool w1 = !(ctx_opt(c, "EMIT_WAVE") && ctx_opt(c, "EMIT_WAVE")[0] == '0');
                const u32 wgt = w1 ? 64u : 256u, grid = (u32)cdiv(pl.P.N, wgt / lanes);
#define ER_LAUNCH(FB, LN) do { if (w1) LAUNCH(c, "unnaf_emit_records", (k_emit_fastq_records<FB, LN, 64>), grid, 64, 0, pl.P, d_out); \
                               else LAUNCH(c, "unnaf_emit_records", (k_emit_fastq_records<FB, LN, 256>), grid, 256, 0, pl.P, d_out); } while (0)
                if (pl.fourbit) { if (lanes == 4) ER_LAUNCH(true, 4); else if (lanes == 8) ER_LAUNCH(true, 8); else ER_LAUNCH(true, 16); }
                else { if (lanes == 4) ER_LAUNCH(false, 4); else if (lanes == 8) ER_LAUNCH(false, 8); else ER_LAUNCH(false, 16); }
#undef ER_LAUNCH
            }
        } else if (short_rec) {
            if (pl.P.mode == EM_FASTA || pl.P.mode == EM_FASTQ) {
                u64 nr = rec1 - rec0 + 1, htot = 0;
                u64 *ho = arena_new<u64>(c, nr + 2); if (!ho) return NAF_GPU_ENOMEM;
                LAUNCH(c, "unnaf_hdr_len64", k_hdr_len64, cdiv(nr, 256), 256, 0, pl.P.hdr_len, rec0, nr, ho);
                if ((rc = scan_exclusive_u64(c, ho, nr, ho + nr + 1))) return rc;
                if ((rc = ctx_readback(c, &htot, ho + nr + 1, 8))) return rc;
                u8 *ht = (u8 *)arena_alloc(c, htot + 32); if (!ht) return NAF_GPU_ENOMEM;
                LAUNCH(c, "unnaf_hdr_build", k_hdr_build, cdiv(nr, 32), 256, 0, pl.P, rec0, nr, (const u64 *)ho, ht);
                pl.P.hdr_off = ho; pl.P.hdr_text = ht; pl.P.hdr_r0 = rec0;
            }
            u32 grid = cdiv(m_end - m_begin, ES_SPAN);
            if (pl.fourbit) LAUNCH(c, "unnaf_emit_short", k_emit_short<true>, grid, 256, 0, pl.P, d_out);
            else LAUNCH(c, "unnaf_emit_short", k_emit_short<false>, grid, 256, 0, pl.P, d_out);
        } else if (ek && !strcmp(ek, "span")) {
            u32 grid = cdiv(m_end - m_begin, EMIT_SPAN);
            if (pl.fourbit) LAUNCH(c, "unnaf_emit", k_emit<true>, grid, 256, 0, pl.P, d_out);
            else LAUNCH(c, "unnaf_emit", k_emit<false>, grid, 256, 0, pl.P, d_out);
        } else {
            u64 ntiles = cdiv(m_end - m_begin, 4096);
            TileIdx *ti = arena_new<TileIdx>(c, ntiles + 2 + FLAT_TPW); u64 *tr = arena_new<u64>(c, ntiles + 2);
            u32 *list = arena_new<u32>(c, ntiles + 1), *cnt = arena_new<u32>(c, 2);
            u32 *list2 = (zflat.ready && zflat.cls) ? arena_new<u32>(c, ntiles + 1) : list;
            if (!ti || !tr || !list || !cnt || !list2) return NAF_GPU_ENOMEM;
            if (!split.done) HIP_TRY(c, hipMemsetAsync(cnt, 0, 8, c->stream));
            u64 Lp1 = pl.P.L + 1;
            pl.P.Ldiv_magic = (Lp1 >= 2 && Lp1 < 32768) ? (u32)((1ull << 32) / Lp1 + 1) : 0;
            naf_gpu_ctx *ic = split.done ? c->side2 : c;
            const bool tile_wave = !(ctx_opt(c, "EMIT_WAVE") && ctx_opt(c, "EMIT_WAVE")[0] == '0');
            if (split.done) HIP_TRY(c, hipMemsetAsync(cnt, 0, 8, ic->stream));
            TileFlat *tsig = nullptr;
            if (zflat.ready) {
                tsig = arena_new<TileFlat>(c, ntiles + 2 + FLAT_TPW); u32 *fpair = arena_new<u32>(c, 400); if (!tsig || !fpair) return NAF_GPU_ENOMEM;
                LAUNCH(ic, "unnaf_flat_pair", k_flat_pair, 1, 256, 0, pl.P, fpair);
                pl.P.fpair = fpair;
            }
            LAUNCH(ic, "unnaf_tile_index", k_tile_index, cdiv(ntiles + 1 + FLAT_TPW, TILE_WG), 256, 0, pl.P, ntiles, ti, tr, list, cnt, tsig, (u32)FLAT_TPW, list2);
            naf_gpu_ctx *xc = c;
            const bool flat_job = zflat.ready && zflat.later;
            if (zflat.ready && zflat.aux) {
                HIP_TRY(c, hipEventRecord(c->split_ev[0], c->stream));
                if (!flat_job) { HIP_TRY(c, hipStreamWaitEvent(zflat.aux->stream, c->split_ev[0], 0)); xc = zflat.aux; }
            }
            u64 t_done = 0;
            if (split.done) {
                HIP_TRY(c, hipEventRecord(c->split_ev[ZSPLIT_MAX], ic->stream));
                for (int k = 0; k + 1 < split.parts; k++) {
                    u64 bases_ready = split.out_end[k] * (pl.fourbit ? 2u : 1u);
                    u64 t_hi = bases_ready / 4096; t_hi = t_hi > 1 ? t_hi - 1 : 0;
                    if (t_hi > ntiles) t_hi = ntiles;
                    if (t_hi <= t_done) continue;
                    HIP_TRY(c, hipStreamWaitEvent(ic->stream, split.ev[k], 0));
                    if (tile_wave && pl.fourbit) LAUNCH(ic, "unnaf_emit", (k_emit_tile_wave<true, 2>), cdiv(t_hi - t_done, 2u), 64, 0, pl.P, (const TileIdx *)(ti + t_done), d_out + t_done * 4096, (u64)(t_hi - t_done));
                    else if (tile_wave) LAUNCH(ic, "unnaf_emit", (k_emit_tile_wave<false, 2>), cdiv(t_hi - t_done, 2u), 64, 0, pl.P, (const TileIdx *)(ti + t_done), d_out + t_done * 4096, (u64)(t_hi - t_done));
                    else if (pl.fourbit) LAUNCH(ic, "unnaf_emit", k_emit_tile<true>, (u32)(t_hi - t_done), 256, 0, pl.P, (const TileIdx *)(ti + t_done), d_out + t_done * 4096);
                    else LAUNCH(ic, "unnaf_emit", k_emit_tile<false>, (u32)(t_hi - t_done), 256, 0, pl.P, (const TileIdx *)(ti + t_done), d_out + t_done * 4096);
                    t_done = t_hi;
                }
                HIP_TRY(c, hipEventRecord(c->split_ev[ZSPLIT_MAX + 1], ic->stream));
                HIP_TRY(c, hipStreamWaitEvent(c->stream, c->split_ev[ZSPLIT_MAX], 0));
            }
            if (zflat.ready) {
                const u32 nwg = cdiv(ntiles, 4u), chunk = (nwg + 7) / 8;
                const char *ew = ctx_opt(c, "EMIT_WAVE");
                const bool mixed = flat_job || (zflat.cls && zflat.n_decoded);
                const bool wave = !(ew && ew[0] == '0') && (!mixed || zflat.n_walk == 0);
                if (wave && pl.P.masking && pl.P.n_toggles >= ntiles) { const u32 ch = ((u32)ntiles + 7) / 8; LAUNCH(c, "unnaf_emit_flat", k_emit_tile_flat_wave<1>, ch * 8, 64, 0, pl.P, (const TileIdx *)ti, (const TileFlat *)tsig, d_out, (u64)ntiles, ch); }
                else if (wave) { const u32 ch = (cdiv(ntiles, 2u) + 7) / 8; LAUNCH(c, "unnaf_emit_flat", k_emit_tile_flat_wave<2>, ch * 8, 64, 0, pl.P, (const TileIdx *)ti, (const TileFlat *)tsig, d_out, (u64)ntiles, ch); }
                else
                LAUNCH(c, "unnaf_emit_flat", k_emit_tile_flat<4>, chunk * 8, 256, 0, pl.P, (const TileIdx *)ti, (const TileFlat *)tsig, d_out, (u64)ntiles, chunk);
                if (flat_job) {
                    if ((rc = zstd_flat_later(c, &zflat))) return rc;
                    if (zflat.aux) xc = zflat.aux;
                }
                if (zflat.cls && zflat.n_decoded) {
                    const u64 est = (u64)zflat.n_decoded * 64 + 64;
                    const u32 lgrid = (u32)(est < ntiles ? (est < 16384 ? est : 16384) : (ntiles < 16384 ? ntiles : 16384));
                    if (wave) LAUNCH(xc, "unnaf_emit", k_emit_tile_list_wave<true>, lgrid, 64, 0, pl.P, (const TileIdx *)ti, (const u32 *)list2, (const u32 *)(cnt + 1), d_out);
                    else LAUNCH(xc, "unnaf_emit", k_emit_tile_list<true>, lgrid, 256, 0, pl.P, (const TileIdx *)ti, (const u32 *)list2, (const u32 *)(cnt + 1), d_out);
                }
            }
            else if (t_done < ntiles) {
                if (tile_wave && pl.fourbit) LAUNCH(c, "unnaf_emit", (k_emit_tile_wave<true, 2>), cdiv(ntiles - t_done, 2u), 64, 0, pl.P, (const TileIdx *)(ti + t_done), d_out + t_done * 4096, (u64)(ntiles - t_done));
                else if (tile_wave) LAUNCH(c, "unnaf_emit", (k_emit_tile_wave<false, 2>), cdiv(ntiles - t_done, 2u), 64, 0, pl.P, (const TileIdx *)(ti + t_done), d_out + t_done * 4096, (u64)(ntiles - t_done));
                else if (pl.fourbit) LAUNCH(c, "unnaf_emit", k_emit_tile<true>, (u32)(ntiles - t_done), 256, 0, pl.P, (const TileIdx *)(ti + t_done), d_out + t_done * 4096);
                else LAUNCH(c, "unnaf_emit", k_emit_tile<false>, (u32)(ntiles - t_done), 256, 0, pl.P, (const TileIdx *)(ti + t_done), d_out + t_done * 4096);
            }
            const u32 rest_grid = 4u * (u32)(ntiles < EMIT_REST_GRID ? ntiles : EMIT_REST_GRID);
            if (pl.fourbit) LAUNCH(xc, "unnaf_emit_rest", k_emit_rest<true>, rest_grid, 64, 0, pl.P, (const TileIdx *)ti, (const u64 *)tr, (const u32 *)list, (const u32 *)cnt, d_out);
            else LAUNCH(xc, "unnaf_emit_rest", k_emit_rest<false>, rest_grid, 64, 0, pl.P, (const TileIdx *)ti, (const u64 *)tr, (const u32 *)list, (const u32 *)cnt, d_out);
            if (xc != c) { HIP_TRY(c, hipEventRecord(c->split_ev[1], xc->stream)); HIP_TRY(c, hipStreamWaitEvent(c->stream, c->split_ev[1], 0)); }
            if (split.done) HIP_TRY(c, hipStreamWaitEvent(c->stream, c->split_ev[ZSPLIT_MAX + 1], 0));
            if (zflat.ready && ctx_tracing(c)) {
                u32 hc[2] = { 0, 0 };
                if (!ctx_readback(c, hc, cnt, 8)) ctx_trace(c, "[flat tiles] total %llu rest %u decoded %u\n", (unsigned long long)ntiles, hc[0], hc[1]);
            }
        }
    }
    if (has_tail) {
        const u64 lo = (out_begin > pl.main_total ? out_begin : pl.main_total) - pl.main_total, hi = out_end - pl.main_total;
        u8 *dst = d_out + (pl.main_total + lo - out_begin);
        const int wrap = pl.P.mode == EM_FASTA;
        if (pl.fourbit) LAUNCH(c, "unnaf_emit_surplus", k_emit_surplus<true>, cdiv(hi - lo, 256), 256, 0, pl.P, pl.sur_base0, pl.surplus, pl.sur_c, pl.P.L, wrap, lo, hi, dst);
        else LAUNCH(c, "unnaf_emit_surplus", k_emit_surplus<false>, cdiv(hi - lo, 256), 256, 0, pl.P, pl.sur_base0, pl.surplus, pl.sur_c, pl.P.L, wrap, lo, hi, dst);
    }
    HIP_TRY(c, hipGetLastError());
    if ((rc = zstd_split_status(c, &split))) return rc;
    if (zflat.ready) { ZSplit fs; fs.parts = 0; fs.done = 1; fs.status = zflat.status; if ((rc = zstd_split_status(c, &fs))) return rc; }
    return 0;
}

extern "C" int naf_gpu_unnaf_size(naf_gpu_ctx *c, const void *d_naf, size_t naf_len, const naf_gpu_unnaf_opts *o, size_t *out_len)
{
    return unnaf_run(c, (const u8 *)d_naf, naf_len, o, 0, 0, true, nullptr, 0, out_len, true);
}
extern "C" int naf_gpu_unnaf(naf_gpu_ctx *c, const void *d_naf, size_t naf_len, const naf_gpu_unnaf_opts *o, void *d_out, size_t out_cap, size_t *out_len)
{
    int rc = unnaf_run(c, (const u8 *)d_naf, naf_len, o, 0, 0, true, (u8 *)d_out, out_cap, out_len, false);
    if (c) arena_settle(c);
    return rc;
}
extern "C" int naf_gpu_unnaf_range(naf_gpu_ctx *c, const void *d_naf, size_t naf_len, const naf_gpu_unnaf_opts *o,
                                   uint64_t out_begin, uint64_t out_end, void *d_out, size_t out_cap, size_t *out_len)
{
    int rc = unnaf_run(c, (const u8 *)d_naf, naf_len, o, out_begin, out_end, false, (u8 *)d_out, out_cap, out_len, false);
    if (c) arena_settle(c);
    return rc;
}

#include "emit_select.h"

__global__ __launch_bounds__(256) void k_histogram(const u8 *p, u64 n, unsigned long long *counts)
{
    __shared__ u32 h[4][256];
    for (u32 i = threadIdx.x; i < 1024; i += 256) ((u32 *)h)[i] = 0;
    __syncthreads();
    u32 *my = h[threadIdx.x >> 6];
    const u64 per = 65536;
    u64 lo = (u64)blockIdx.x * per, hi = lo + per < n ? lo + per : n;
    for (u64 i = lo + (u64)threadIdx.x * 8; i < hi; i += 256 * 8) {
        if (i + 8 <= hi) { u64 w = ld64(p + i); for (int k = 0; k < 8; k++) atomicAdd(&my[(w >> (8 * k)) & 0xFF], 1u); }
        else for (u64 k = i; k < hi; k++) atomicAdd(&my[p[k]], 1u);
    }
    __syncthreads();
    u32 v = h[0][threadIdx.x] + h[1][threadIdx.x] + h[2][threadIdx.x] + h[3][threadIdx.x];
    if (v) atomicAdd(&counts[threadIdx.x], (unsigned long long)v);
}
extern "C" int naf_gpu_histogram(naf_gpu_ctx *c, const void *d_buf, size_t n, uint64_t counts[256])
{
    if (!c || !counts || (!d_buf && n)) return NAF_GPU_EARG;
    arena_reset(c);
    unsigned long long *d = arena_new<unsigned long long>(c, 256); if (!d) return NAF_GPU_ENOMEM;
    HIP_TRY(c, hipMemsetAsync(d, 0, 256 * 8, c->stream));
    if (n) LAUNCH(c, "histogram", k_histogram, cdiv(n, 65536), 256, 0, (const u8 *)d_buf, (u64)n, d);
    return ctx_readback(c, counts, d, 256 * 8);
}
```

naf_amd/csrc/zstd_dec.hip:

```cpp
#include "ctx.h"
#include "wgscan.h"
#include "zstd_dec_core.h"
#include "emit_core.h"

struct ZStat {
    u32 nblk; u32 err; u64 end_off;
    u32 n_huf_def, n_seq_blk, max_huf_log, rep_slow;
    u32 huf_pool_used, fse_pool_used;
    u64 total_seq, total_out;
    u32 ticket, n_plain_huf;
    u32 max_seq_regen, n_flat;
    u32 n_huf_distinct, n_huf_built;
    u32 max_lit_regen, n_huf_pending;
    u32 last_raw, flat_main_inv;
    u32 n_exec_done, n_wave;
#ifdef NAF_EXEC_PROF
    unsigned long long prof[8];
#endif
};

static __device__ __forceinline__ void set_err(ZStat *st, u32 e) { if (e) atomicMax(&st->err, e); }
static __device__ __forceinline__ u64 shfl_u64(u64 v, int l) { u32 lo = __shfl((u32)v, l, 64), hi = __shfl((u32)(v >> 32), l, 64); return ((u64)hi << 32) | lo; }

#define SCAN_WIN (48u * 1024u)
// ... 3117 lines not shown
            __syncthreads();
            out += size;
            if (last) break;
            continue;
        }
        ZBlock b; b.src_off = 0; b.bsize = size; b.btype = BT_COMP; b.last = (u8)last;
        zstd_parse_block(c, b);
        if (b.err) { err = b.err; break; }
        if ((u64)out + b.lit_regen > cap) { err = SMALL_TOO_BIG; break; }
        u8 *lp = b.nseq ? lit : dst + out;
        if (b.lit_type == LIT_RAW) for (u32 k = lane; k < b.lit_regen; k += 64) lp[k] = c[b.lit_off + k];
        else if (b.lit_type == LIT_RLE) { const u8 v = c[b.lit_off]; for (u32 k = lane; k < b.lit_regen; k += 64) lp[k] = v; }
        else {
            if (b.lit_type == LIT_HUF) {
                __syncthreads();
                if (lane == 0) { W.b = b; W.b.src_off = 0; }
                __syncthreads();
                build_huf_one_lds(c, &W.b, 0, nullptr, 0, &W.st, W.H, (u8 *)huf);
                __syncthreads();
                const u32 lg = W.H.log;
                if (!lg) { err = ZE_CORRUPT; break; }
                huf_log = lg; have_huf = true;
            } else if (!have_huf) { err = ZE_CORRUPT; break; }
            const u8 *sp = c + b.huf_streams_off;
            bool bad = false;
            if (b.nstreams == 1) { if (lane == 0) bad = huf_decode_stream(sp, b.huf_streams_size, (const u16 *)huf, huf_log, lp, b.lit_regen) != 0; }
            else {
                const u32 s1 = ld16(sp), s2 = ld16(sp + 2), s3 = ld16(sp + 4), tot = b.huf_streams_size - 6, per = (b.lit_regen + 3) / 4;
                if (s1 + s2 + s3 >= tot || !s1 || !s2 || !s3 || per * 3 > b.lit_regen) { err = ZE_CORRUPT; break; }
                if (lane < 4) {
                    const u32 k = lane;
                    const u32 o = k == 0 ? 0 : (k == 1 ? s1 : (k == 2 ? s1 + s2 : s1 + s2 + s3)), z = k == 0 ? s1 : (k == 1 ? s2 : (k == 2 ? s3 : tot - s1 - s2 - s3));
                    bad = huf_decode_stream(sp + 6 + o, z, (const u16 *)huf, huf_log, lp + k * per, k < 3 ? per : b.lit_regen - 3 * per) != 0;
                }
            }
            if (__ballot(bad)) { err = ZE_CORRUPT; break; }
        }
        __syncthreads();
        if (!b.nseq) { out += b.lit_regen; if (last) break; continue; }
        if (b.nseq > SMALL_SEQ) { err = SMALL_TOO_BIG; break; }
        u32 p = b.seq_off; bool tbad = false;
        for (int k = 0; k < 3 && !tbad; k++) {
            const u32 m = b.modes[k];
            if (m == SM_PREDEF) { tab[k].t = predef + po[k]; tab[k].log = pl[k]; tab[k].rle = false; tab[k].rle_sym = 0; have_tab[k] = true; }
            else if (m == SM_RLE) { tab[k].t = predef; tab[k].log = 0; tab[k].rle = true; tab[k].rle_sym = b.fse_tab[k]; have_tab[k] = true; p++; }
            else if (m == SM_FSE) {
                u32 nsym, lg;
                const u32 d = fse_read_ncount(c + p, b.bsize - p, max_log[k], max_sym[k], norm, &nsym, &lg);
                if (!d || lg != b.fse_log[k] || !fse_build_table(fse + fo[k], norm, nsym, lg, nx)) { tbad = true; break; }
                p += d; tab[k].t = fse + fo[k]; tab[k].log = lg; tab[k].rle = false; tab[k].rle_sym = 0; have_tab[k] = true;
            } else if (!have_tab[k]) tbad = true;
        }
        if (tbad || p != b.seq_bits_off) { err = ZE_CORRUPT; break; }
        u64 tl = 0, tm = 0; u32 ro[3];
        u8 e = 0xFF;
        if (b.modes[0] == SM_PREDEF && b.modes[1] == SM_PREDEF && b.modes[2] == SM_PREDEF)
            e = zstd_decode_sequences_predef<const FseE *, const u32 *, false>(c + b.seq_bits_off, b.seq_bits_size, b.nseq, predef, predef + 64, predef + 96, llt, mlt, sll, sml, sof, ro, &tl, &tm, nullptr);
        if (e == 0xFF) e = zstd_decode_sequences(c + b.seq_bits_off, b.seq_bits_size, b.nseq, tab, sll, sml, sof, ro, &tl, &tm);
        if (e) { err = e; break; }
        if (tl > b.lit_regen) { err = ZE_CORRUPT; break; }
        const u64 regen = b.lit_regen + tm;
        if (regen > ZBLOCK_MAX) { err = ZE_CORRUPT; break; }
        if ((u64)out + regen > cap) { err = SMALL_TOO_BIG; break; }
        __syncthreads();
        u32 op = out, l = 0; bool xbad = false;
        for (u32 q0 = 0; q0 < b.nseq && !xbad; q0 += 64) {
            const u32 q = q0 + lane; const bool on = q < b.nseq;
            const u32 ll = on ? sll[q] : 0, ml = on ? sml[q] : 0;
            const u32 ill = wave_scan_inclusive<u32, OpAdd>(ll), iml = wave_scan_inclusive<u32, OpAdd>(ml);
            const u32 my_l = l + ill - ll, my_op = op + (ill - ll) + (iml - ml);
            { u32 k = 0; for (; k + 8 <= ll; k += 8) st64(dst + my_op + k, ld64(lit + my_l + k)); for (; k < ll; k++) dst[my_op + k] = lit[my_l + k]; }
            __syncthreads();
            const u32 cnt = b.nseq - q0 < 64 ? b.nseq - q0 : 64;
            for (u32 j = 0; j < cnt; j++) {
                const u32 mop = (u32)__shfl((int)(my_op + ll), (int)j, 64), mlj = (u32)__shfl((int)ml, (int)j, 64), of = sym_resolve(sof[q0 + j], rep);
                if (of == 0 || of > mop) { xbad = true; break; }
                if (of >= mlj || of >= 64) for (u32 k0 = 0; k0 < mlj; k0 += 64) { const u32 k = k0 + lane; if (k < mlj) { const u8 v = dst[mop + k - of]; dst[mop + k] = v; } __syncthreads(); }
                else { for (u32 k = lane; k < mlj; k += 64) dst[mop + k] = dst[mop - of + k % of]; __syncthreads(); }
            }
            op += (u32)__shfl((int)(ill + iml), 63, 64); l += (u32)__shfl((int)ill, 63, 64);
        }
        if (xbad) { err = ZE_CORRUPT; break; }
        { const u32 rest = b.lit_regen - l; for (u32 k = lane; k < rest; k += 64) dst[op + k] = lit[l + k]; op += rest; }
        __syncthreads();
        { const u32 r0 = sym_resolve(ro[0], rep), r1 = sym_resolve(ro[1], rep), r2 = sym_resolve(ro[2], rep); rep[0] = r0; rep[1] = r1; rep[2] = r2; }
        out = op;
        if (last) break;
    }
    if (!err && fh.checksum) { if (pos + 4 > len) err = ZE_TRUNC; else pos += 4; }
    if (!err && fh.has_fcs && fh.content_size != out) err = ZE_CORRUPT;
    res->err = err; res->out = out; res->pos = pos;
}
__global__ __launch_bounds__(64) void k_small_frame(const u8 *src, u32 len, u8 *dst, u32 cap, const FseE *predef, u32 *res)
{
    __builtin_amdgcn_s_setprio(3);
    __shared__ __attribute__((aligned(16))) u8 s_src[SMALL_SRC + 16], s_out[SMALL_OUT + 16], s_lit[SMALL_OUT + 16];
    __shared__ u32 s_ll[SMALL_SEQ], s_ml[SMALL_SEQ], s_of[SMALL_SEQ];
    __shared__ SmallWS W;
    __shared__ __attribute__((aligned(16))) u16 huf[HUF_TAB_MAX / 2];
    __shared__ FseE fse[512 + 256 + 512];
    __shared__ FseE s_predef[160];
    __shared__ i16 norm[64];
    __shared__ u16 nx[64];
    __shared__ SmallRes r;
    __shared__ u32 s_llt[36], s_mlt[53];
    zstd_seq_code_tables(s_llt, s_mlt, threadIdx.x, 64);
    for (u32 k = threadIdx.x; k < len; k += 64) s_src[k] = src[k];
    for (u32 k = threadIdx.x; k < 16; k += 64) s_src[len + k] = 0;
    for (u32 k = threadIdx.x; k < 160; k += 64) s_predef[k] = predef[k];
    __syncthreads();
    small_frame_decode(s_src, len, s_out, cap < SMALL_OUT ? cap : SMALL_OUT, s_lit, s_ll, s_ml, s_of, s_predef, W, huf, fse, norm, nx, &r, s_llt, s_mlt);
    __syncthreads();
    if (r.err == 0) for (u32 k = threadIdx.x; k < r.out; k += 64) dst[k] = s_out[k];
    if (threadIdx.x == 0) { res[0] = r.err; res[1] = r.out; res[2] = r.pos; }
}

struct SmallJobs { const u8 *src[4]; u8 *dst[4]; u32 len[4], cap[4]; };
__global__ __launch_bounds__(64) void k_small_frames(SmallJobs J, const FseE *predef, u32 *res)
{
    __builtin_amdgcn_s_setprio(3);
    __shared__ __attribute__((aligned(16))) u8 s_src[SMALL_SRC + 16], s_out[SMALL_OUT + 16], s_lit[SMALL_OUT + 16];
    __shared__ u32 s_ll[SMALL_SEQ], s_ml[SMALL_SEQ], s_of[SMALL_SEQ];
    __shared__ SmallWS W;
    __shared__ __attribute__((aligned(16))) u16 huf[HUF_TAB_MAX / 2];
    __shared__ FseE fse[512 + 256 + 512];
    __shared__ FseE s_predef[160];
    __shared__ i16 norm[64];
    __shared__ u16 nx[64];
    __shared__ SmallRes r;
    __shared__ u32 s_llt[36], s_mlt[53];
    zstd_seq_code_tables(s_llt, s_mlt, threadIdx.x, 64);
    const u32 j = blockIdx.x;
    const u8 *src = J.src[j]; const u32 len = J.len[j], cap = J.cap[j]; u8 *dst = J.dst[j];
    for (u32 k = threadIdx.x; k < len; k += 64) s_src[k] = src[k];
    for (u32 k = threadIdx.x; k < 16; k += 64) s_src[len + k] = 0;
    for (u32 k = threadIdx.x; k < 160; k += 64) s_predef[k] = predef[k];
    __syncthreads();
    small_frame_decode(s_src, len, s_out, cap < SMALL_OUT ? cap : SMALL_OUT, s_lit, s_ll, s_ml, s_of, s_predef, W, huf, fse, norm, nx, &r, s_llt, s_mlt);
    __syncthreads();
    if (r.err == 0) for (u32 k = threadIdx.x; k < r.out; k += 64) dst[k] = s_out[k];
    if (threadIdx.x == 0) { res[4 * j] = r.err; res[4 * j + 1] = r.out; res[4 * j + 2] = r.pos; }
}
int zstd_small_batch(naf_gpu_ctx *c, int n, const u8 *const *src, const size_t *len, u8 *const *dst, const size_t *cap, bool *ok)
{
    SmallJobs J; memset(&J, 0, sizeof J); int m = 0, map[4];
    for (int k = 0; k < n && k < 4; k++) {
        ok[k] = false;
        if (len[k] == 0 || len[k] > SMALL_SRC || cap[k] > SMALL_OUT) continue;
        J.src[m] = src[k]; J.len[m] = (u32)len[k]; J.dst[m] = dst[k]; J.cap[m] = (u32)cap[k]; map[m++] = k;
    }
    if (!m) return 0;
    u32 *d_res = arena_new<u32>(c, 16); if (!d_res) return NAF_GPU_ENOMEM;
    LAUNCH(c, "zstd_small_frame", k_small_frames, m, 64, 0, J, (const FseE *)c->d_predef, d_res);
    u32 res[16]; int rc = ctx_readback(c, res, d_res, 16 * (size_t)m); if (rc) return rc;
    for (int q = 0; q < m; q++) ok[map[q]] = res[4 * q] == 0 && res[4 * q + 1] == J.cap[q] && res[4 * q + 2] == J.len[q];
    return 0;
}
bool zstd_small_fits(size_t len, size_t cap) { return len != 0 && len <= SMALL_SRC && cap <= SMALL_OUT; }
int zstd_small_launch(naf_gpu_ctx *c, int n, const u8 *const *src, const size_t *len, u8 *const *dst, const size_t *cap, u32 **d_res_out)
{
    SmallJobs J; memset(&J, 0, sizeof J);
    if (n < 1 || n > 4) return NAF_GPU_EARG;
    for (int k = 0; k < n; k++) { if (!zstd_small_fits(len[k], cap[k])) return NAF_GPU_EARG; J.src[k] = src[k]; J.len[k] = (u32)len[k]; J.dst[k] = dst[k]; J.cap[k] = (u32)cap[k]; }
    u32 *d_res = arena_new<u32>(c, 16); if (!d_res) return NAF_GPU_ENOMEM;
    LAUNCH(c, "zstd_small_frame", k_small_frames, n, 64, 0, J, (const FseE *)c->d_predef, d_res);
    *d_res_out = d_res;
    return 0;
}

int zstd_init_tables(naf_gpu_ctx *c)
{
    static const i16 LL[36] = { 4,3,2,2,2,2,2,2,2,2,2,2,2,1,1,1,2,2,2,2,2,2,2,2,2,3,2,1,1,1,1,1,-1,-1,-1,-1 };
    static const i16 OF[29] = { 1,1,1,1,1,1,2,2,2,1,1,1,1,1,1,1,1,1,1,1,1,1,1,1,-1,-1,-1,-1,-1 };
    static const i16 ML[53] = { 1,4,3,2,2,2,2,2,2,1,1,1,1,1,1,1,1,1,1,1,1,1,1,1,1,1,1,1,1,1,1,1,1,1,1,1,1,1,1,1,1,1,1,1,1,1,-1,-1,-1,-1,-1,-1,-1 };
    FseE tabs[64 + 32 + 64]; u16 next[64];
    if (!fse_build_table(tabs, LL, 36, 6, next) || !fse_build_table(tabs + 64, OF, 29, 5, next) || !fse_build_table(tabs + 96, ML, 53, 6, next))
        return ctx_fail(c, NAF_GPU_EZSTD, "predefined FSE tables");
    HIP_TRY(c, hipMalloc(&c->d_predef, sizeof tabs));
    HIP_TRY(c, hipMemcpy(c->d_predef, tabs, sizeof tabs, hipMemcpyHostToDevice));
    return 0;
}


static u32 huf_par_plog(const naf_gpu_ctx *c, u32 max_lit_regen, u64 n_blocks)
{
    const char *e = ctx_opt(c, "HUF_PAR");
    if (e && e[0] == '0') return 0;
    const char *t = ctx_opt(c, "HUF_PART");
    u32 target = t ? (u32)atoi(t) : 128u; if (target < 64) target = 64;
    const u32 nmax = (max_lit_regen + 3) / 4;
    u32 plog = 0;
    while (plog < 6 && (nmax >> (plog + 1)) >= target) plog++;
    if (e && e[0] >= '1' && e[0] <= '6') { const u32 f = (u32)(e[0] - '0'); return f < plog ? f : plog; }
    if (n_blocks * (u64)max_lit_regen >= (u64)nmax * 86016) return 0;
    const char *ll = ctx_opt(c, "HUF_LANES_LOG");
    const u32 lanes_log = ll && atoi(ll) >= 10 && atoi(ll) <= 24 ? (u32)atoi(ll) : (nmax >= 16384 ? 20u : 18u);
    while (plog && ((n_blocks * 4) << plog) > (1ull << lanes_log)) plog--;
    return plog;
}
static u32 huf_par_margin_env(const naf_gpu_ctx *c) { const char *m = ctx_opt(c, "HUF_MARGIN"); return m ? (u32)atoi(m) : 0u; }

#define ZSTD_NEED_TWO_PASS (-100)
static int launch_build_huf(naf_gpu_ctx *c, u32 count, const u8 *src, ZBlock *blk, u32 nblk, u8 *pool, u32 pool_cap, ZStat *st, u32 first, const u64 *range4, u32 always_table, const i32 *own_huf, u32 gate, u32 phase)
{
    const char *e = ctx_opt(c, "HUF_BUILD16");
    if (e && e[0] == '0') LAUNCH(c, "zstd_build_huf", k_build_huf, cdiv(count, 64), 64, 0, src, blk, nblk, pool, pool_cap, st, first, range4, always_table, own_huf, gate, phase);
    else if (ctx_opt_is(c, "HUF_BUILD_WG", '1')) LAUNCH(c, "zstd_build_huf", k_build_huf16<16>, cdiv(count, 16), 256, 0, src, blk, nblk, pool, pool_cap, st, first, range4, always_table, own_huf, gate, phase);
    else LAUNCH(c, "zstd_build_huf", k_build_huf16<4>, cdiv(count, 4), 64, 0, src, blk, nblk, pool, pool_cap, st, first, range4, always_table, own_huf, gate, phase);
    return 0;
}
static int zerr(naf_gpu_ctx *c, u32 e, const char *where)
{
    const char *m = e == ZE_TRUNC ? "truncated" : e == ZE_CORRUPT ? "corrupt" : e == ZE_UNSUP ? "unsupported feature" : "table pool";
    return ctx_fail(c, NAF_GPU_EZSTD, "zstd frame %s (%s)", m, where);
}

static int zstd_decode_one(naf_gpu_ctx *c, const u8 *d_src, size_t src_len, u8 *d_dst, size_t dst_cap,
                           size_t *out_len, size_t *consumed, ZRange *rg, const EmitP *fuse, u8 *text, const u8 *head = nullptr)
{
    int rc;
    if (!rg && !fuse && src_len && src_len <= SMALL_SRC && dst_cap <= SMALL_OUT) {
        u32 *d_res = arena_new<u32>(c, 4);
        if (!d_res) return NAF_GPU_ENOMEM;
        LAUNCH(c, "zstd_small_frame", k_small_frame, 1, 64, 0, d_src, (u32)src_len, d_dst, (u32)dst_cap, (const FseE *)c->d_predef, d_res);
        u32 res[3]; if ((rc = ctx_readback(c, res, d_res, 12))) return rc;
        if (res[0] == 0) { *out_len = res[1]; *consumed = res[2]; return 0; }
        if (res[0] != SMALL_TOO_BIG) return zerr(c, res[0], "small frame");
    }
    u8 hb[18]; size_t hl = src_len < 18 ? src_len : 18;
    if (head) memcpy(hb, head, hl);
    else { rc = ctx_readback(c, hb, d_src, hl); if (rc) return rc; }
    ZFrameHdr fh = zstd_parse_frame_header(hb, hl);
    if (fh.err) return zerr(c, (u32)fh.err, "frame header");

    ZStat *st = arena_new<ZStat>(c, 1);
    if (!st) return NAF_GPU_ENOMEM;
    HIP_TRY(c, hipMemsetAsync(st, 0, sizeof(ZStat), c->stream));
    ZBlock *blk = nullptr; ZStat hs; bool indexed = false;
    const char *nospec = ctx_opt(c, "SERIAL_INDEX");
    const char *fl_env = ctx_opt(c, "FLAT");
    const u32 always_table = (fl_env && fl_env[0] == '0') ? 1u : 0u;
    const char *smin = ctx_opt(c, "SPEC_MIN");
    const u32 spec_min = smin ? (u32)atoi(smin) : 512u;
    const char *un_env = ctx_opt(c, "UNIFORM");
    const bool uni_wanted = c->zflat && !fuse && !always_table && !(un_env && un_env[0] == '0');
    u32 chunk = SPEC_CHUNK, win1 = SPEC_WINDOW1, win2 = SPEC_WINDOW;
    if (src_len <= 4ull * SPEC_CHUNK) {
        chunk = 256; while (chunk < SPEC_CHUNK_SMALL && (u64)chunk * 128 < src_len) chunk *= 2;
        win1 = win2 = chunk;
    } else if (src_len <= 256ull * SPEC_CHUNK && fh.hdr_size + 3 <= hl) {
        const u32 h0 = (u32)hb[fh.hdr_size] | ((u32)hb[fh.hdr_size + 1] << 8) | ((u32)hb[fh.hdr_size + 2] << 16);
        const u32 b0 = ((h0 >> 1) & 3) == 1 ? 4u : (h0 >> 3) + 3;
        u32 want = SPEC_CHUNK_SMALL; while (want < SPEC_CHUNK && want < 16 * b0) want *= 2;
        if (want < SPEC_CHUNK) { chunk = want; if (win1 > chunk) win1 = chunk; if (win2 > chunk) win2 = chunk; }
    }
    if (src_len >= 2048 && !(nospec && nospec[0] == '1')) {
        u32 nchunks = (u32)((src_len + chunk - 1) / chunk);
        u64 *first = arena_new<u64>(c, nchunks + 1), *land = arena_new<u64>(c, nchunks + 2), *G = arena_new<u64>(c, nchunks + 1);
        u64 *start = arena_new<u64>(c, nchunks + 2), *cnt = arena_new<u64>(c, (size_t)nchunks + 4);
        if (!first || !land || !G || !start || !cnt) return NAF_GPU_ENOMEM;
        HIP_TRY(c, hipMemsetAsync(first, 0xFF, (size_t)nchunks * 8, c->stream));
        u64 *h0 = (u64 *)c->h_stage; *h0 = fh.hdr_size;
        HIP_TRY(c, hipMemcpyAsync(first, h0, 8, hipMemcpyHostToDevice, c->stream));
        u32 gl = cdiv(nchunks, 64);
        {
            const char *se = ctx_opt(c, "STRIDE_INDEX");
            if (ctx_tracing(c)) ctx_trace(c, "[stride?] len %zu hdr %u hl %zu first %02x %02x %02x\n", src_len, fh.hdr_size, hl, hb[fh.hdr_size], hb[fh.hdr_size + 1], hb[fh.hdr_size + 2]);
            if (src_len > 4ull * SPEC_CHUNK && fh.hdr_size + 3 <= hl && !(se && se[0] == '0')) {
                const u32 h0 = (u32)hb[fh.hdr_size] | ((u32)hb[fh.hdr_size + 1] << 8) | ((u32)hb[fh.hdr_size + 2] << 16);
                const u32 S = 3 + (h0 >> 3);
                const u64 nmax64 = (src_len - fh.hdr_size) / S;
                if (((h0 >> 1) & 3) == BT_COMP && !(h0 & 1) && (h0 >> 3) <= ZBLOCK_MAX && S >= 256 && nmax64 >= 64 && nmax64 < 0x7FFFFF00ull) {
                    const u32 nmax = (u32)nmax64;
                    u32 *sres = (u32 *)(cnt + nchunks + 2); ZBlock *sblk = arena_new<ZBlock>(c, (size_t)nmax + STRIDE_TAIL);
                    if (!sblk) return NAF_GPU_ENOMEM;
                    HIP_TRY(c, hipMemsetAsync(sres, 0xFF, 8, c->stream));
                    LAUNCH(c, "zstd_index_stride", k_stride_probe, cdiv(nmax, 256), 256, 0, d_src, (u64)src_len, (u64)fh.hdr_size, S, h0, nmax, sres);
                    LAUNCH(c, "zstd_index_stride", k_stride_tail, 1, 64, 0, d_src, (u64)src_len, (u64)fh.hdr_size, S, nmax, sres, sblk, st);
                    UniInfo *U = nullptr; FlatStream *usi = nullptr; u8 *usym = nullptr;
                    if (uni_wanted) {
                        U = arena_new<UniInfo>(c, 1); ZBlock *ublk = arena_new<ZBlock>(c, STRIDE_TAIL + 1);
                        usi = arena_new<FlatStream>(c, 4 * ((size_t)nmax + STRIDE_TAIL) + 1); usym = (u8 *)arena_alloc(c, 16);
                        if (!U || !ublk || !usi || !usym) return NAF_GPU_ENOMEM;
                        LAUNCH(c, "zstd_flat_uniform", k_uni_head, 1, 64, 0, d_src, (u64)fh.hdr_size, S, h0, nmax, (const u32 *)sres, (const ZBlock *)sblk, (const ZStat *)st, U, ublk, spec_min);
                        LAUNCH(c, "zstd_flat_uniform", k_uni_streams, cdiv(4ull * ((u64)nmax + STRIDE_TAIL) + 1, 256) + 1, 256, 0, d_src, (u64)fh.hdr_size, S, (const ZBlock *)ublk, U, usi, usym);
                    }
                    LAUNCH(c, "zstd_index_stride", k_stride_write, cdiv(nmax, 256), 256, 0, (u64)fh.hdr_size, S, h0, (const u32 *)sres, sblk, (const u32 *)U);
                    u32 res2[2] = { 0, 0 }; UniInfo hu; memset(&hu, 0, sizeof hu);
                    if (U) { void *hp[3] = { &hs, res2, &hu }; const void *dp[3] = { st, sres, U }; const size_t nb[3] = { sizeof hs, 8, sizeof hu }; rc = ctx_readbackv(c, 3, hp, dp, nb); }
                    else rc = ctx_readback2(c, &hs, st, sizeof hs, res2, sres, 8);
                    if (rc) return rc;
                    if (ctx_tracing(c)) ctx_trace(c, "[stride] len %zu S %u nmax %u prefix %u verdict %u err %u nblk %u\n", src_len, S, nmax, res2[0], res2[1], hs.err, hs.nblk);
                    if (ctx_tracing(c) && U) ctx_trace(c, "[uniform?] ok %u bad %u prefix %u blocks %u huffman %u regen %u total %llu\n", hu.ok, hu.bad, hu.np, hu.nblk, hu.nhb, hu.regen0, (unsigned long long)hu.total_out);
                    if (res2[1] == 1u && !hs.err && hs.nblk && hu.ok && !hu.bad) {
                        ZFlat *zf = c->zflat;
                        const size_t frame_end = hs.end_off + (fh.checksum ? 4 : 0);
                        if (frame_end > src_len) return zerr(c, ZE_TRUNC, "checksum");
                        *consumed = frame_end;
                        const bool flat_tail = hu.last_raw != 0;
                        zf->src = d_src; zf->si = usi; zf->nslots = 4ull * hu.nhb; zf->sym = usym; zf->status = st; zf->ready = true;
                        const u32 tn = hu.last_raw & 0x7FFFFFFFu; const bool rle = (hu.last_raw >> 31) != 0;
                        zf->tail = flat_tail ? d_src + (hs.end_off - (rle ? 1u : tn)) : nullptr; zf->tail_q = hu.total_out - (flat_tail ? tn : 0u);
                        zf->tail_n = flat_tail ? (rle ? tn | 0x80000000u : tn) : 0u;
                        if (rg) { rg->got_lo = 0; rg->got_hi = hu.total_out; rg->ranged = false; }
                        *out_len = hu.total_out;
                        if (fh.has_fcs && fh.content_size != hu.total_out) return zerr(c, ZE_CORRUPT, "content size mismatch");
                        return 0;
                    }
                    if (res2[1] == 1u && !hs.err && hs.nblk) { blk = sblk; indexed = true; }
                    if (res2[1] == 2u && !hs.err && uni_wanted && !ctx_opt_is(c, "STRIDE_RUNS", '0')) {
                        UniRuns *R = arena_new<UniRuns>(c, 1); ZBlock *odd = arena_new<ZBlock>(c, STRIDE_TAIL + 1), *ublk0 = arena_new<ZBlock>(c, 1);
                        u32 *probe = arena_new<u32>(c, 2); UniInfo *U2 = arena_new<UniInfo>(c, 1);
                        FlatStream *usi2 = arena_new<FlatStream>(c, 4 * ((size_t)nmax + USEG_MAX) + 1); u8 *usym2 = (u8 *)arena_alloc(c, 16);
                        if (!R || !odd || !ublk0 || !probe || !U2 || !usi2 || !usym2) return NAF_GPU_ENOMEM;
                        for (u32 r = 0; r <= URUN_MAX; r++) {
                            LAUNCH(c, "zstd_index_stride", k_runs_next, 1, 64, 0, d_src, (u64)src_len, (u64)fh.hdr_size, S, h0, (const u32 *)sres, R, odd, probe, r == 0 ? 1 : 0);
                            if (r < URUN_MAX) LAUNCH(c, "zstd_index_stride", k_runs_probe, cdiv(nmax, 256), 256, 0, d_src, (u64)src_len, S, h0, (const UniRuns *)R, probe);
                        }
                        LAUNCH(c, "zstd_flat_uniform", k_uni_head_runs, 1, 64, 0, d_src, (u64)fh.hdr_size, h0, R, odd, U2, ublk0, spec_min);
                        LAUNCH(c, "zstd_flat_uniform", k_uni_streams_runs, cdiv(4ull * ((u64)nmax + USEG_MAX) + 1, 256) + 1, 256, 0, d_src, S, (const UniRuns *)R, (const ZBlock *)odd, (const ZBlock *)ublk0, U2, usi2, usym2);
                        UniInfo hu2; memset(&hu2, 0, sizeof hu2);
                        if ((rc = ctx_readback(c, &hu2, U2, sizeof hu2))) return rc;
                        if (ctx_tracing(c)) ctx_trace(c, "[runs?] ok %u bad %u first run %u blocks %u huffman %u total %llu\n", hu2.ok, hu2.bad, hu2.np, hu2.nblk, hu2.nhb, (unsigned long long)hu2.total_out);
                        if (hu2.ok && !hu2.bad) {
                            ZFlat *zf = c->zflat;
                            const size_t frame_end = hu2.end_off + (fh.checksum ? 4 : 0);
                            if (frame_end > src_len) return zerr(c, ZE_TRUNC, "checksum");
                            *consumed = frame_end;
                            const bool flat_tail = hu2.last_raw != 0;
                            zf->src = d_src; zf->si = usi2; zf->nslots = 4ull * hu2.nhb; zf->sym = usym2; zf->status = st; zf->ready = true;
                            const u32 tn = hu2.last_raw & 0x7FFFFFFFu; const bool rle = (hu2.last_raw >> 31) != 0;
                            zf->tail = flat_tail ? d_src + (hu2.end_off - (rle ? 1u : tn)) : nullptr; zf->tail_q = hu2.total_out - (flat_tail ? tn : 0u);
                            zf->tail_n = flat_tail ? (rle ? tn | 0x80000000u : tn) : 0u;
                            if (rg) { rg->got_lo = 0; rg->got_hi = hu2.total_out; rg->ranged = false; }
                            *out_len = hu2.total_out;
                            if (fh.has_fcs && fh.content_size != hu2.total_out) return zerr(c, ZE_CORRUPT, "content size mismatch");
                            return 0;
                        }
                    }
                }
            }
        }
        const u32 *skip = nullptr;
        if (!indexed) {
        const u32 win0 = chunk == SPEC_CHUNK ? SPEC_WINDOW0 : win1;
        LAUNCH(c, "zstd_index_find", k_spec_find, cdiv(win0, 256 * 16) * (nchunks - 1), 256, 0, d_src, (u64)src_len, nchunks, first, 0u, win0, chunk, skip);
        if (win1 > win0) LAUNCH(c, "zstd_index_find2", k_spec_find, cdiv(win1 - win0, 256 * 16) * (nchunks - 1), 256, 0, d_src, (u64)src_len, nchunks, first, win0, win1, chunk, skip);
        if (win2 > win1) LAUNCH(c, "zstd_index_find2", k_spec_find, cdiv(win2 - win1, 256 * 16) * (nchunks - 1), 256, 0, d_src, (u64)src_len, nchunks, first, win1, win2, chunk, skip);
        LAUNCH(c, "zstd_index_land", k_spec_land, gl, 64, 0, d_src, (u64)src_len, (const u64 *)first, nchunks, land, chunk, skip);
        LAUNCH(c, "zstd_index_land2", k_spec_land2, gl, 64, 0, d_src, (u64)src_len, (const u64 *)first, (const u64 *)land, nchunks, G, chunk, skip);
        LAUNCH(c, "zstd_index_resolve", k_spec_resolve, 1, 64, 0, d_src, (u64)src_len, (const u64 *)land, (const u64 *)G, nchunks, start, st, chunk, skip);
        LAUNCH(c, "zstd_index_count", (k_spec_walk<false>), gl, 64, 0, d_src, (u64)src_len, (const u64 *)start, nchunks, cnt, (ZBlock *)nullptr, st, skip);
        u64 *d_tot = cnt + nchunks + 1;
        if ((rc = scan_exclusive_u64(c, cnt, nchunks, d_tot))) return rc;
        u64 tot = 0;
        rc = ctx_readback2(c, &hs, st, sizeof hs, &tot, d_tot, 8); if (rc) return rc;
        if (!hs.err && tot > 0 && tot < 0x7FFFFFFFull) {
            blk = arena_new<ZBlock>(c, tot);
            if (!blk) return NAF_GPU_ENOMEM;
            LAUNCH(c, "zstd_index_write", (k_spec_walk<true>), gl, 64, 0, d_src, (u64)src_len, (const u64 *)start, nchunks, cnt, blk, st, (const u32 *)nullptr);
            hs.nblk = (u32)tot; indexed = true;
        } else {
            HIP_TRY(c, hipMemsetAsync(st, 0, sizeof(ZStat), c->stream));
        }
        }
    }
    if (!indexed) {
        u32 cap = (u32)(src_len / 16 + 1024);
        for (int attempt = 0; attempt < 2; attempt++) {
            blk = arena_new<ZBlock>(c, cap);
            if (!blk) return NAF_GPU_ENOMEM;
            const u32 win = src_len < SCAN_WIN ? (u32)((src_len + 15) & ~15ull) + 16 : SCAN_WIN;
            LAUNCH(c, "zstd_scan_blocks", k_scan_blocks, 1, 64, win + 16, d_src, (u64)src_len, (u64)fh.hdr_size, blk, cap, st, win);
            rc = ctx_readback(c, &hs, st, sizeof hs); if (rc) return rc;
            if (hs.err) return zerr(c, hs.err, "block headers");
            if (hs.nblk <= cap) break;
            cap = hs.nblk;
        }
    }
    u32 nblk = hs.nblk;
    size_t frame_end = hs.end_off + (fh.checksum ? 4 : 0);
    if (frame_end > src_len) return zerr(c, ZE_TRUNC, "checksum");
    *consumed = frame_end;

    i32 *own = arena_new<i32>(c, (size_t)nblk * 4);
    u64 *seq_cnt = arena_new<u64>(c, (size_t)nblk + 1), *sizes = arena_new<u64>(c, (size_t)nblk + 1);
    if (!own || !seq_cnt || !sizes) return NAF_GPU_ENOMEM;
    i32 *own_huf = own, *own_ll = own + nblk, *own_of = own + 2 * (size_t)nblk, *own_ml = own + 3 * (size_t)nblk;
    u32 g = cdiv(nblk, 64);
    LAUNCH(c, "zstd_parse_blocks", k_parse_blocks, g, 64, 0, d_src, blk, nblk, own_huf, own_ll, own_of, own_ml, seq_cnt, sizes, st);
    LAUNCH(c, "zstd_huf_dedup", k_huf_dedup, g, 64, 0, d_src, (const ZBlock *)blk, nblk, own_huf, st);
    if ((rc = scan_inclusive_max_i32(c, own_huf, nblk))) return rc;
    u64 *d_total_out = (u64 *)((u8 *)st + offsetof(ZStat, total_out));
    const bool spec = nblk > spec_min && !fuse;
    u64 *r4 = nullptr, *ends = nullptr; u8 *huf_pool = nullptr; u32 pool_cap = 0; bool tables_built = false; bool ranged_build = false; bool two_phase = false;
    u64 h4[5] = { 0, 0, 0, 0, 0 }, hends[ZSPLIT_MAX] = { 0 };
    bool late_build = false;
    if (spec) {
        if ((rc = scan_exclusive_u64(c, sizes, nblk, d_total_out))) return rc;
        u64 *extra = arena_new<u64>(c, 8 + ZSPLIT_MAX); if (!extra) return NAF_GPU_ENOMEM;
        if (rg && rg->want_hi > rg->want_lo) {
            r4 = extra;
            LAUNCH(c, "zstd_find_range", k_find_range, 1, 64, 0, (const u64 *)sizes, nblk, (const u64 *)d_total_out, rg->want_lo, rg->want_hi, (const i32 *)own_huf, r4);
            ranged_build = true;
        }
        const u64 want_pool = (u64)nblk * HUF_TAB_MAX + 4096;
        pool_cap = want_pool > 0xFFFFF000ull ? 0xFFFFF000u : (u32)want_pool;
        huf_pool = (u8 *)arena_alloc(c, pool_cap);
        if (!huf_pool) return NAF_GPU_ENOMEM;
        if (nblk <= 16384) {
            LAUNCH(c, "zstd_build_huf", k_build_huf_lds, nblk, 64, 0, d_src, blk, nblk, huf_pool, pool_cap, st, 0u, (const i32 *)own_huf);
        } else {
            LAUNCH(c, "zstd_build_huf", k_build_huf_few, 1024, 64, 0, d_src, blk, nblk, huf_pool, pool_cap, st, (const u64 *)r4, (const i32 *)own_huf);
            two_phase = c->zflat && !rg && !always_table;
            if (two_phase) LAUNCH(c, "zstd_build_huf", k_flat_find_main, FIND_MAIN_TREES, 64, 0, d_src, blk, nblk, huf_pool, pool_cap, st, (const i32 *)own_huf);
            else late_build = true;
        }
        ZSplit *sp = c->zsplit;
        if (sp && !rg && sp->parts >= 2) {
            ends = extra + 8;
            for (int k = 0; k + 1 < sp->parts; k++) {
                u32 hi_b = (u32)((u64)nblk * (k + 1) / sp->parts) & ~(HUF_BLOCKS_PER_WG - 1u);
                HIP_TRY(c, hipMemcpyAsync(ends + k, sizes + hi_b, 8, hipMemcpyDeviceToDevice, c->stream));
            }
        }
        u64 hx[8 + ZSPLIT_MAX];
        rc = ctx_readback2(c, &hs, st, sizeof hs, hx, extra, sizeof hx); if (rc) return rc;
        memcpy(h4, hx, sizeof h4); memcpy(hends, hx + 8, sizeof hends);
        if (late_build && !hs.err && hs.n_huf_distinct > HUF_FEW) {
            if ((rc = launch_build_huf(c, nblk, d_src, blk, nblk, huf_pool, pool_cap, st, 0u, (const u64 *)r4, always_table, (const i32 *)own_huf, 1u, 0u))) return rc;
            rc = ctx_readback(c, &hs, st, sizeof hs); if (rc) return rc;
        }
        tables_built = true;
    } else {
        rc = ctx_readback(c, &hs, st, sizeof hs); if (rc) return rc;
    }
    if (hs.err) return zerr(c, hs.err, "block parse");
    u32 n_seq_blk = hs.n_seq_blk, n_huf_def = hs.n_huf_def;
    if (fuse && !(n_seq_blk == 0 && hs.n_plain_huf == nblk && nblk > 0)) return ZSTD_NEED_TWO_PASS;
    const bool lit_only_spec = spec && n_seq_blk == 0;
    if (spec && n_seq_blk && ranged_build) {
        tables_built = false;
        HIP_TRY(c, hipMemsetAsync((u8 *)st + offsetof(ZStat, huf_pool_used), 0, 4, c->stream));
        HIP_TRY(c, hipMemsetAsync((u8 *)st + offsetof(ZStat, max_huf_log), 0, 4, c->stream));
        HIP_TRY(c, hipMemsetAsync((u8 *)st + offsetof(ZStat, n_flat), 0, 4, c->stream));
        HIP_TRY(c, hipMemsetAsync((u8 *)st + offsetof(ZStat, n_huf_built), 0, 4, c->stream));
    }
    const bool flat_tail = hs.last_raw != 0 && nblk >= 2 && hs.n_plain_huf == nblk - 1;
    if (ctx_tracing(c) && c->zflat) ctx_trace(c, "[flat?] spec %d nblk %u seq_blk %u distinct %u built %u n_flat %u log %u plain %u last_raw %u always %u\n", (int)spec, nblk, n_seq_blk, hs.n_huf_distinct, hs.n_huf_built, hs.n_flat, hs.max_huf_log, hs.n_plain_huf, hs.last_raw, always_table);
    if (c->zflat && lit_only_spec && nblk > 0 && hs.n_huf_distinct == 1 && hs.n_huf_built == 1 && hs.n_flat == 1 && hs.max_huf_log == 4 && (hs.n_plain_huf == nblk || flat_tail) && !always_table) {
        ZFlat *zf = c->zflat;
        const u32 nhb = flat_tail ? nblk - 1 : nblk;
        FlatStream *si = arena_new<FlatStream>(c, 4 * (size_t)nhb + 1); u8 *d_sym = (u8 *)arena_alloc(c, 16);
        if (!si || !d_sym) return NAF_GPU_ENOMEM;
        LAUNCH(c, "zstd_set_offsets", k_set_offsets, g, 64, 0, blk, nblk, (const u64 *)sizes, (u32 *)nullptr, (u32 *)nullptr, (u32 *)nullptr);
        LAUNCH(c, "zstd_flat_streams", k_flat_streams, cdiv(4ull * nhb, 256), 256, 0, d_src, (const ZBlock *)blk, nhb, (const i32 *)own_huf, (const u8 *)huf_pool, si, d_sym, st, (const u64 *)d_total_out, flat_tail ? (u64)(hs.last_raw & 0x7FFFFFFFu) : 0ull);
        zf->src = d_src; zf->si = si; zf->nslots = 4ull * nhb; zf->sym = d_sym; zf->status = st; zf->ready = true;
        {
            const u32 tn = hs.last_raw & 0x7FFFFFFFu; const bool rle = (hs.last_raw >> 31) != 0;
            zf->tail = flat_tail ? d_src + (hs.end_off - (rle ? 1u : tn)) : nullptr; zf->tail_q = hs.total_out - (flat_tail ? tn : 0u);
            zf->tail_n = flat_tail ? (rle ? tn | 0x80000000u : tn) : 0u;
        }
        if (rg) { rg->got_lo = 0; rg->got_hi = hs.total_out; rg->ranged = false; }
        *out_len = hs.total_out;
        if (fh.has_fcs && fh.content_size != hs.total_out) return zerr(c, ZE_CORRUPT, "content size mismatch");
        return 0;
    }
    {
        const char *fm = ctx_opt(c, "FLAT_MIXED");
        if (c->zflat && lit_only_spec && nblk > 0 && !always_table && !rg && hs.flat_main_inv && d_dst && hs.total_out <= dst_cap && !(fm && fm[0] == '0')) {
            const u32 main = 0xFFFFFFFFu - hs.flat_main_inv;
            ZFlat *zf = c->zflat;
            FlatStream *si = arena_new<FlatStream>(c, 4 * (size_t)nblk + 1); u8 *d_sym = (u8 *)arena_alloc(c, 16);
            u8 *cls0 = (u8 *)arena_alloc(c, nblk), *cls = (u8 *)arena_alloc(c, nblk); u32 *d_nx = arena_new<u32>(c, 2);
            if (!si || !d_sym || !cls0 || !cls || !d_nx) return NAF_GPU_ENOMEM;
            HIP_TRY(c, hipMemsetAsync(d_nx, 0, 8, c->stream));
            LAUNCH(c, "zstd_set_offsets", k_set_offsets, g, 64, 0, blk, nblk, (const u64 *)sizes, (u32 *)nullptr, (u32 *)nullptr, (u32 *)nullptr);
            LAUNCH(c, "zstd_flat_class", k_flat_mark_owner, g, 64, 0, d_src, blk, nblk, (const i32 *)own_huf, main, two_phase ? 1u : 0u);
            LAUNCH(c, "zstd_flat_class", k_flat_sym, 1, 256, 0, d_src, (const ZBlock *)blk, main, (const u8 *)huf_pool, d_sym);
            LAUNCH(c, "zstd_flat_class", k_flat_class, g, 64, 0, (const ZBlock *)blk, nblk, (const i32 *)own_huf, cls0, d_nx + 1);
            LAUNCH(c, "zstd_flat_class", k_flat_class2, g, 64, 0, (const u8 *)cls0, nblk, cls, d_nx);
            u32 nx2[2] = { 0, 0 };
            if ((rc = ctx_readback(c, nx2, d_nx, 8))) return rc;
            const u32 n_dec = nx2[0], n_walk = nx2[1];
            if (ctx_tracing(c)) ctx_trace(c, "[flat mixed] nblk %u decoded %u main %u\n", nblk, n_dec, main);
            if ((u64)n_dec * 2 <= nblk) {
                LAUNCH(c, "zstd_flat_streams", k_flat_streams_mixed, cdiv(4ull * nblk, 256), 256, 0, d_src, (const ZBlock *)blk, nblk, (const u8 *)cls, si, st, (const u64 *)d_total_out);
                zf->decoded_ev = nullptr; zf->later = nullptr;
                if (n_dec) {
                    const bool pending = two_phase && hs.n_huf_distinct > HUF_FEW;
                    const ZStat hs0 = hs; naf_gpu_ctx *mc = c; naf_gpu_ctx *aux = zf->aux;
                    const u64 src_len64 = (u64)src_len;
                    zf->later = new std::function<int()>([=]() -> int {
                        naf_gpu_ctx *c = aux ? aux : mc;
                        if (c != mc) HIP_TRY(mc, hipStreamWaitEvent(c->stream, mc->split_ev[0], 0));
                        const u32 plog = n_walk ? huf_par_plog(c, hs0.max_lit_regen, n_walk) : 0u;
                        u32 max_log = hs0.max_huf_log;
                        if (pending && n_walk && !plog) {
                            { int r3 = launch_build_huf(c, nblk, d_src, blk, nblk, huf_pool, pool_cap, st, 0u, (const u64 *)nullptr, 0u, (const i32 *)own_huf, 1u, 2u); if (r3) { if (c != mc) memcpy(mc->err, c->err, sizeof mc->err); return r3; } }
                            ZStat h2; int r2 = ctx_readback(c, &h2, st, sizeof h2);
                            if (r2) { if (c != mc) memcpy(mc->err, c->err, sizeof mc->err); return r2; }
                            if (h2.err) return zerr(mc, h2.err, "Huffman tables");
                            max_log = h2.max_huf_log;
                        }
                        if (hs0.n_plain_huf != nblk) LAUNCH(c, "zstd_copy_fill", k_copy_fill<64>, 4 * nblk, 64, 0, d_src, (const ZBlock *)blk, nblk, d_dst, (u8 *)nullptr, 0u, (const u8 *)cls);
                        LAUNCH(c, "zstd_flat_literals", k_flat_literals<64>, 4 * nblk, 64, 0, d_src, (const ZBlock *)blk, nblk, (const i32 *)own_huf, (const u8 *)huf_pool, d_dst, (u8 *)nullptr, st, 0u, (const u8 *)cls);
                        if (n_walk && plog) {
                            const u32 slot = pending ? (u32)HUF_TAB_MAX : huf_slot_bytes(max_log);
                            LAUNCH(c, "zstd_huf_literals", k_huf_par, cdiv((u64)nblk << (plog + 2), 64), 64, (plog >= 4 ? 1u : 16u >> plog) * slot,
                                   d_src, (const ZBlock *)blk, nblk, (const i32 *)own_huf, (const u8 *)huf_pool, slot, d_dst, (u8 *)nullptr, st, 0u, plog, (const u8 *)cls, 1u, huf_par_margin_env(c), pending ? 1u : 0u, src_len64);
                        } else if (n_walk) {
                            const u32 slot = huf_slot_bytes(max_log), ipitch = max_log > 7 ? HUF_IROW_BIG : HUF_IROW;
                            EmitP ep; memset(&ep, 0, sizeof ep);
                            LAUNCH(c, "zstd_huf_literals", (k_huf_literals<false>), cdiv(nblk, HUF_BLOCKS_PER_WG), 64, slot * HUF_BLOCKS_PER_WG + 64 * ipitch + 64 * HUF_OROW + 512,
                                   d_src, (const ZBlock *)blk, nblk, (const i32 *)own_huf, (const u8 *)huf_pool, slot, d_dst, (u8 *)nullptr, st, 0u, ep, (u8 *)nullptr, ipitch, src_len64, 1u, (const u8 *)cls);
                        }
                        return 0;
                    });
                }
                zf->src = d_src; zf->si = si; zf->nslots = 4ull * nblk; zf->sym = d_sym; zf->status = st; zf->ready = true;
                zf->tail = nullptr; zf->tail_q = hs.total_out; zf->tail_n = 0; zf->cls = cls; zf->n_decoded = n_dec; zf->n_walk = n_walk;
                *out_len = hs.total_out;
                if (fh.has_fcs && fh.content_size != hs.total_out) return zerr(c, ZE_CORRUPT, "content size mismatch");
                return 0;
            }
        }
    }
    if (two_phase && hs.n_huf_distinct > HUF_FEW) {
        if ((rc = launch_build_huf(c, nblk, d_src, blk, nblk, huf_pool, pool_cap, st, 0u, (const u64 *)nullptr, 0u, (const i32 *)own_huf, 1u, 2u))) return rc;
        rc = ctx_readback(c, &hs, st, sizeof hs); if (rc) return rc;
        if (hs.err) return zerr(c, hs.err, "Huffman tables");
    }
    u64 *d_total_seq = (u64 *)((u8 *)st + offsetof(ZStat, total_seq));
    FseE *fse_pool = nullptr; u32 *o_ll = nullptr, *o_ml = nullptr, *o_of = nullptr;
    if (n_seq_blk) {
        if ((rc = scan_inclusive_max_i32(c, own_ll, nblk))) return rc;
        if ((rc = scan_inclusive_max_i32(c, own_of, nblk))) return rc;
        if ((rc = scan_inclusive_max_i32(c, own_ml, nblk))) return rc;
        if ((rc = scan_exclusive_u64(c, seq_cnt, nblk, d_total_seq))) return rc;
        u32 fse_cap = n_seq_blk * (512 + 256 + 512);
        fse_pool = arena_new<FseE>(c, fse_cap);
        if (!fse_pool) return NAF_GPU_ENOMEM;
        LAUNCH(c, "zstd_build_fse", k_build_fse, cdiv(3 * (u64)nblk, 64), 64, 0, d_src, blk, nblk, fse_pool, fse_cap, st);
        rc = ctx_readback(c, &hs, st, sizeof hs); if (rc) return rc;
        if (hs.err) return zerr(c, hs.err, "table build");
        size_t ns = hs.total_seq ? hs.total_seq : 1;
        o_ll = arena_new<u32>(c, ns); o_ml = arena_new<u32>(c, ns); o_of = arena_new<u32>(c, ns);
        if (!o_ll || !o_ml || !o_of) return NAF_GPU_ENOMEM;
    }
    u32 *seq_list = nullptr;
    u64 *seq_rank = nullptr;
    if (n_seq_blk) {
        seq_list = arena_new<u32>(c, n_seq_blk);
        u64 *flag = arena_new<u64>(c, (size_t)nblk + 1); seq_rank = flag;
        if (!seq_list || !flag) return NAF_GPU_ENOMEM;
        LAUNCH(c, "zstd_seq_flag", k_seq_flag, g, 64, 0, (const ZBlock *)blk, nblk, flag);
        if ((rc = scan_exclusive_u64(c, flag, nblk, (u64 *)nullptr))) return rc;
        LAUNCH(c, "zstd_seq_list", k_seq_list, g, 64, 0, (const ZBlock *)blk, nblk, (const u64 *)flag, seq_list);
    }
    if (!lit_only_spec) {
        const u32 dsl = nblk < 32768 ? 16u : 64u;
        const u32 all_wave = ctx_opt_is(c, "SEQ_WAVE", 'a') ? 1u : 0u;
        const u32 own_tabs = (n_seq_blk && !ctx_opt_is(c, "SEQ_WAVE", '0')) ? 1u + all_wave : 0u;
        u32 *wave_list = own_tabs ? arena_new<u32>(c, n_seq_blk) : nullptr;
        if (own_tabs && !wave_list) return NAF_GPU_ENOMEM;
        LAUNCH(c, "zstd_decode_seq", k_decode_seq, cdiv(nblk, dsl), dsl, 0, d_src, blk, nblk, (const i32 *)own_ll, (const i32 *)own_of, (const i32 *)own_ml,
               (const u64 *)seq_cnt, (const FseE *)fse_pool, (const FseE *)c->d_predef, o_ll, o_ml, o_of, sizes, st, own_tabs, wave_list);
        const u32 wgrid = n_seq_blk < 8192u ? n_seq_blk : 8192u;
        if (own_tabs && ctx_opt_is(c, "SEQ_WAVE", 'l'))
            LAUNCH(c, "zstd_decode_seq", k_decode_seq_wave, wgrid, 64, 0, d_src, blk, (const u32 *)wave_list, (const i32 *)own_ll, (const i32 *)own_of, (const i32 *)own_ml,
                   (const u64 *)seq_cnt, (const FseE *)fse_pool, (const FseE *)c->d_predef, o_ll, o_ml, o_of, sizes, st);
        else if (own_tabs)
            LAUNCH(c, "zstd_decode_seq", k_decode_seq_wave2, wgrid, 64, 0, d_src, blk, (const u32 *)wave_list, (const i32 *)own_ll, (const i32 *)own_of, (const i32 *)own_ml,
                   (const u64 *)seq_cnt, (const FseE *)fse_pool, (const FseE *)c->d_predef, o_ll, o_ml, o_of, sizes, st, all_wave | (ctx_opt_is(c, "SEQ_REP", 'w') ? 2u : 0u));
        if (n_seq_blk) LAUNCH(c, "zstd_rep_fast", k_rep_fast, cdiv(n_seq_blk, 256), 256, 0, blk, (const u32 *)seq_list, n_seq_blk, st);
        if ((rc = scan_exclusive_u64(c, sizes, nblk, d_total_out))) return rc;
        rc = ctx_readback(c, &hs, st, sizeof hs); if (rc) return rc;
        if (hs.err) return zerr(c, hs.err, "sequences");
    }
    const u32 max_seq_regen = hs.max_seq_regen;
    if (ctx_tracing(c) && n_seq_blk) ctx_trace(c, "[seq] blocks %u with sequences %u sequences %llu out %llu\n", nblk, n_seq_blk, (unsigned long long)hs.total_seq, (unsigned long long)hs.total_out);
    if (n_seq_blk && (hs.rep_slow & 1)) LAUNCH(c, "zstd_rep_chain", k_rep_chain, 1, 64, 0, blk, nblk);
    *out_len = hs.total_out;
    if (fh.has_fcs && fh.content_size != hs.total_out) return zerr(c, ZE_CORRUPT, "content size mismatch");
    {
        const char *fm = ctx_opt(c, "FLAT_MIXED"), *fsq = ctx_opt(c, "FLAT_SEQ");
        if (c->zflat && spec && n_seq_blk && tables_built && !fuse && !always_table && !rg && hs.flat_main_inv && d_dst && hs.total_out <= dst_cap &&
            (u64)n_seq_blk * 8 <= nblk && !(fm && fm[0] == '0') && !(fsq && fsq[0] == '0')) {
            const u32 main = 0xFFFFFFFFu - hs.flat_main_inv;
            ZFlat *zf = c->zflat;
            FlatStream *si = arena_new<FlatStream>(c, 4 * (size_t)nblk + 1); u8 *d_sym = (u8 *)arena_alloc(c, 16);
            u8 *cls0 = (u8 *)arena_alloc(c, nblk), *cls = (u8 *)arena_alloc(c, nblk); u32 *d_nx = arena_new<u32>(c, 2);
            u32 *done2 = arena_new<u32>(c, nblk); u8 *lits = (u8 *)arena_alloc(c, hs.total_out + 16);
            if (!si || !d_sym || !cls0 || !cls || !d_nx || !done2 || !lits) return NAF_GPU_ENOMEM;
            HIP_TRY(c, hipMemsetAsync(d_nx, 0, 8, c->stream));
            LAUNCH(c, "zstd_set_offsets", k_set_offsets, g, 64, 0, blk, nblk, (const u64 *)sizes, done2, (u32 *)nullptr, (u32 *)nullptr);
            LAUNCH(c, "zstd_flat_class", k_flat_mark_owner, g, 64, 0, d_src, blk, nblk, (const i32 *)own_huf, main, 0u);
            LAUNCH(c, "zstd_flat_class", k_flat_sym, 1, 256, 0, d_src, (const ZBlock *)blk, main, (const u8 *)huf_pool, d_sym);
            LAUNCH(c, "zstd_flat_class", k_flat_class, g, 64, 0, (const ZBlock *)blk, nblk, (const i32 *)own_huf, cls0, d_nx + 1);
            LAUNCH(c, "zstd_flat_class", k_seq_sources, cdiv(n_seq_blk, 64), 64, 0, (const ZBlock *)blk, (const u32 *)seq_list, n_seq_blk, (const u64 *)sizes, (const u32 *)o_ll, (const u32 *)o_ml, (const u32 *)o_of, cls0);
            LAUNCH(c, "zstd_flat_class", k_flat_class2, g, 64, 0, (const u8 *)cls0, nblk, cls, d_nx);
            u32 nx2[2] = { 0, 0 };
            if ((rc = ctx_readback(c, nx2, d_nx, 8))) return rc;
            const u32 n_dec = nx2[0], n_walk = nx2[1];
            if (ctx_tracing(c)) ctx_trace(c, "[flat mixed] nblk %u decoded %u main %u (blocks with sequences %u)\n", nblk, n_dec, main, n_seq_blk);
            if ((u64)n_dec * 2 <= nblk) {
// ... 255 lines not shown
```

naf_amd/synth.py:

```python
import numpy as np

_ACGT = np.frombuffer(b"ACGT", dtype=np.uint8)


def wrap_lines(seq: np.ndarray, width: int) -> bytes:
    n = len(seq)
    if n == 0:
        return b""
    if width <= 0:
        return seq.tobytes() + b"\n"
    full, rem = divmod(n, width)
    out = np.empty(n + full + (1 if rem else 0), dtype=np.uint8)
    if full:
        body = out[: full * (width + 1)].reshape(full, width + 1)
        body[:, :width] = seq[: full * width].reshape(full, width)
        body[:, width] = 10
    if rem:
        out[full * (width + 1): full * (width + 1) + rem] = seq[full * width:]
        out[-1] = 10
    return out.tobytes()


def fasta_acgt(n_bases: int, n_records: int = 1, width: int = 80, seed: int = 12345,
               name=lambda k: b">seq%d synthetic random ACGT" % (k + 1)) -> bytes:
    rng = np.random.Generator(np.random.PCG64(seed))
    parts = []
    per = n_bases // n_records
    for k in range(n_records):
        n = per if k + 1 < n_records else n_bases - per * (n_records - 1)
        seq = _ACGT[rng.integers(0, 4, n, dtype=np.uint8)]
        parts.append(name(k) + b"\n" + wrap_lines(seq, width))
    return b"".join(parts)


def fasta_mixed(n_records: int = 20, mean_len: int = 3000, width: int = 60, seed: int = 1,
                p_lower: float = 0.3, iupac: bool = True, empty_every: int = 7) -> bytes:
    rng = np.random.Generator(np.random.PCG64(seed))
    alpha = np.frombuffer(b"ACGT" * 8 + (b"RYSWKMBDHVN-" if iupac else b""), dtype=np.uint8)
    parts = []
    for k in range(n_records):
        if empty_every and k % empty_every == empty_every - 1:
            n = 0
        else:
            n = int(rng.integers(1, 2 * mean_len))
        seq = alpha[rng.integers(0, len(alpha), n)]
        pos = 0
        while pos < n:
            run = int(rng.geometric(1.0 / 300))
            if rng.random() < p_lower:
                seg = seq[pos:pos + run]
                letters = seg != ord("-")
                seg[letters] |= 0x20
            pos += run
        if n > 600 and rng.random() < 0.5:
            a = int(rng.integers(0, n - 520))
            seq[a:a + 510] = ord("N")
        hdr = b">rec%d" % k + (b" some comment %d" % (k * 7) if k % 3 else b"")
        parts.append(hdr + b"\n" + wrap_lines(seq, width))
    return b"".join(parts)


def fastq_reads(n_reads: int, read_len: int = 150, seed: int = 7, var_len: bool = False) -> bytes:
    rng = np.random.Generator(np.random.PCG64(seed))
    alpha = np.frombuffer(b"ACGTacgtN", dtype=np.uint8)
    p = np.array([0.22] * 4 + [0.025] * 4 + [0.02])
    parts = []
    for k in range(n_reads):
        n = int(rng.integers(1, read_len + 1)) if var_len else read_len
        seq = alpha[rng.choice(9, n, p=p)]
        qual = rng.integers(33, 74, n, dtype=np.uint8)
        parts.append(b"@read%d len=%d\n" % (k + 1, n) + seq.tobytes() + b"\n+\n" + qual.tobytes() + b"\n")
    return b"".join(parts)


def fasta_acgt_device(total_bytes: int, n_records: int = 100, width: int = 80, seed: int = 2024, device="cuda"):
    import torch
    g = torch.Generator(device=device)
    g.manual_seed(seed)
    hdrs = [b">chr%d synthetic random ACGT record %d\n" % (k + 1, k + 1) for k in range(n_records)]
    hdr_total = sum(len(h) for h in hdrs)
    rows_total = max(n_records, (total_bytes - hdr_total) // (width + 1))
    rows_per = rows_total // n_records
    lut = torch.tensor(list(b"ACGT"), dtype=torch.uint8, device=device)
    total = hdr_total + rows_per * n_records * (width + 1)
    out = torch.empty(total, dtype=torch.uint8, device=device)
    pos = 0
    for k in range(n_records):
        h = torch.tensor(list(hdrs[k]), dtype=torch.uint8, device=device)
        out[pos:pos + len(h)] = h
        pos += len(h)
        body = out[pos:pos + rows_per * (width + 1)].view(rows_per, width + 1)
        idx = torch.randint(0, 4, (rows_per, width), dtype=torch.int64, device=device, generator=g)
        body[:, :width] = lut[idx]
        body[:, width] = 10
        pos += rows_per * (width + 1)
    return out


def fastq_reads_device(total_bytes: int, read_len: int = 150, seed: int = 7, device="cuda", chunk_reads: int = 1 << 22):
    import torch
    g = torch.Generator(device=device)
    g.manual_seed(seed)
    base_lut = torch.tensor(list(b"A" * 220 + b"C" * 220 + b"G" * 220 + b"T" * 220 + b"a" * 25 + b"c" * 25 + b"g" * 25 + b"t" * 25 + b"N" * 20),
                            dtype=torch.uint8, device=device)
    tail = b" len=%d\n" % read_len
    parts, made, n = [], 0, 1
    while made < total_bytes:
        digits = len(str(n))
        width = 5 + digits + len(tail) + read_len + 3 + read_len + 1
        cnt = min(10 ** digits - n, chunk_reads, max(1, (total_bytes - made + width - 1) // width))
        m = torch.empty((cnt, width), dtype=torch.uint8, device=device)
        m[:, 0:5] = torch.tensor(list(b"@read"), dtype=torch.uint8, device=device)
        ids = torch.arange(n, n + cnt, dtype=torch.int64, device=device)
        for d in range(digits):
            m[:, 5 + d] = ((ids // (10 ** (digits - 1 - d))) % 10 + 48).to(torch.uint8)
        p = 5 + digits
        m[:, p:p + len(tail)] = torch.tensor(list(tail), dtype=torch.uint8, device=device)
        p += len(tail)
        m[:, p:p + read_len] = base_lut[torch.randint(0, 1000, (cnt, read_len), dtype=torch.int64, device=device, generator=g)]
        p += read_len
        m[:, p:p + 3] = torch.tensor(list(b"\n+\n"), dtype=torch.uint8, device=device)
        p += 3
        m[:, p:p + read_len] = torch.randint(33, 74, (cnt, read_len), dtype=torch.int64, device=device, generator=g).to(torch.uint8)
        m[:, p + read_len] = 10
        parts.append(m.reshape(-1))
        made += cnt * width
        n += cnt
    return torch.cat(parts)


def repeat_genome(seed=3, unit=40000, copies=50):
    rng = np.random.Generator(np.random.PCG64(seed))
    acgt = np.frombuffer(b"ACGT", dtype=np.uint8)
    base = acgt[rng.integers(0, 4, unit)]
    parts = []
    for i in range(copies):
        s = base.copy()
        idx = rng.integers(0, unit, 150)
        s[idx] = acgt[rng.integers(0, 4, 150)]
        if i % 3 == 0:
            s[1000:3000] |= 0x20
        parts.append(s)
        parts.append(acgt[rng.integers(0, 4, int(rng.integers(10, 4000)))])
    seq = np.concatenate(parts)
    third = len(seq) // 3
    out = b""
    for k in range(3):
        out += b">rep%d repeat-rich synthetic\n" % k + wrap_lines(seq[k * third:(k + 1) * third], 60)
    return out


def softmask_device(text, seed=3, lo=20, hi=600):
    import torch
    n = text.numel()
    gen = torch.Generator(device=text.device); gen.manual_seed(seed)
    nruns = n // ((lo + hi) // 2 - 60) + 16
    bounds = torch.cumsum(torch.randint(lo, hi, (nruns,), device=text.device, generator=gen), 0)
    CH = 1 << 28
    for s in range(0, n, CH):
        e = min(n, s + CH)
        pos = torch.arange(s, e, device=text.device)
        par = torch.searchsorted(bounds, pos, right=True) & 1
        seg = text[s:e]
        seg[((seg >= 65) & (seg <= 90)) & (par == 1)] += 32
    return text


def realistic_genome_device(total_bytes: int, n_records: int = 24, width: int = 60, seed: int = 11, device="cuda",
                            gc: float = 0.41, cpg_keep: float = 0.22, n_run_every: int = 40_000_000, iupac_every: int = 1_000_000,
                            softmask: bool = True):
    import torch
    g = torch.Generator(device=device)
    g.manual_seed(seed)
    w = torch.linspace(5.0, 1.0, n_records, dtype=torch.float64)
    hdrs = [b">REF%d L=%d SYN\n" % (k + 1, k) for k in range(n_records)]
    hdr_total = sum(len(h) for h in hdrs)
    rows_total = max(n_records, (total_bytes - hdr_total) // (width + 1))
    rows = [max(1, int(rows_total * float(x) / float(w.sum()))) for x in w]
    total = hdr_total + sum(rows) * (width + 1)
    out = torch.empty(total, dtype=torch.uint8, device=device)
    at, cg = (1.0 - gc) / 2, gc / 2
    cum = torch.tensor([at, at + cg, at + 2 * cg], dtype=torch.float32, device=device)
    lut = torch.tensor(list(b"ACGT"), dtype=torch.uint8, device=device)
    iupac = torch.tensor(list(b"RYKMSWBDHV"), dtype=torch.uint8, device=device)
    pos = 0
    CH = 1 << 22
    for k in range(n_records):
        h = torch.tensor(list(hdrs[k]), dtype=torch.uint8, device=device)
        out[pos:pos + len(h)] = h
        pos += len(h)
        nb = rows[k] * (width + 1)
        body = out[pos:pos + nb].view(rows[k], width + 1)
        for r0 in range(0, rows[k], CH):
            r1 = min(rows[k], r0 + CH)
            u = torch.rand((r1 - r0) * width, dtype=torch.float32, device=device, generator=g)
            s = lut[torch.bucketize(u, cum)]
            cpg = (s[:-1] == 67) & (s[1:] == 71) & (torch.rand(s.numel() - 1, dtype=torch.float32, device=device, generator=g) >= cpg_keep)
            s[1:][cpg] = 65
            body[r0:r1, :width] = s.view(r1 - r0, width)
            del u, s, cpg
        body[:, width] = 10
        seg = out[pos:pos + nb]
        nbases = rows[k] * width
        runs = [(0, min(nb, 10_000 + 167 * k)), (max(0, nb - 10_000 - 61 * k), nb)]
        n_gaps = int(nbases // n_run_every)
        if n_gaps:
            starts = torch.randint(0, max(1, nb - 200_000), (n_gaps,), device="cpu", generator=torch.Generator().manual_seed(seed * 1000 + k))
            lens = torch.randint(5_000, 100_000, (n_gaps,), device="cpu", generator=torch.Generator().manual_seed(seed * 1000 + k + 500))
            runs += [(int(a), int(a) + int(l)) for a, l in zip(starts.tolist(), lens.tolist())]
        for a, b in runs:
            piece = seg[a:b]
            piece[piece != 10] = 78
        n_iu = int(nbases // iupac_every)
        if n_iu:
            p = torch.randint(0, nb, (n_iu,), device=device, generator=g)
            cur = seg[p]
            ok = (cur == 65) | (cur == 67) | (cur == 71) | (cur == 84)
            seg[p[ok]] = iupac[torch.randint(0, iupac.numel(), (int(ok.sum().item()),), device=device, generator=g)]
        pos += nb
    if softmask:
        softmask_device(out, seed=seed + 1)
    return out


def repeat_genome_device(total_bytes: int, n_records: int = 8, width: int = 60, seed: int = 5, device="cuda",
                         families: int = 96, coverage: float = 0.45, div_lo: float = 0.003, div_hi: float = 0.06):
    import torch
    g = torch.Generator(device=device); g.manual_seed(seed)
    hdrs = [b">scaffold%d repeat-rich synthetic\n" % (k + 1) for k in range(n_records)]
    hdr_total = sum(len(h) for h in hdrs)
    rows_per = max(1, (total_bytes - hdr_total) // (width + 1) // n_records)
    nb = rows_per * n_records * width
    seq = torch.randint(0, 4, (nb,), dtype=torch.uint8, device=device, generator=g)
    cpu = torch.Generator().manual_seed(seed * 7 + 1)
    lens = torch.randint(300, 6000, (families,), generator=cpu).tolist()
    per_family = int(nb * coverage / families)
    for f, L in enumerate(lens):
        unit = torch.randint(0, 4, (L,), dtype=torch.uint8, device=device, generator=g)
        copies = max(1, per_family // L)
        at = torch.randint(0, nb - L, (copies,), dtype=torch.int64, device=device, generator=g)
        rate = div_lo + (div_hi - div_lo) * torch.rand((copies, 1), device=device, generator=g)
        body = unit.repeat(copies, 1)
        hit = torch.rand((copies, L), device=device, generator=g) < rate
        body[hit] = torch.randint(0, 4, (int(hit.sum().item()),), dtype=torch.uint8, device=device, generator=g)
        idx = at[:, None] + torch.arange(L, device=device)[None, :]
        seq[idx.reshape(-1)] = body.reshape(-1)
        del body, hit, idx
    lut = torch.tensor(list(b"ACGT"), dtype=torch.uint8, device=device)
    out = torch.empty(hdr_total + rows_per * n_records * (width + 1), dtype=torch.uint8, device=device)
    pos = 0
    for k in range(n_records):
        h = torch.tensor(list(hdrs[k]), dtype=torch.uint8, device=device)
        out[pos:pos + len(h)] = h; pos += len(h)
        body = out[pos:pos + rows_per * (width + 1)].view(rows_per, width + 1)
        body[:, :width] = lut[seq[k * rows_per * width:(k + 1) * rows_per * width].to(torch.int64)].view(rows_per, width)
        body[:, width] = 10
        pos += rows_per * (width + 1)
    return out
```

Measured before the change: 4248 GB/s.

## Emit flat tiles from per-group span descriptors instead of per-tile index

Adds a group-level index (one descriptor per 255 tiles) that marks spans lying entirely inside one record's sequence with no mask toggles and a uniform 4-stream zstd layout. For those spans a new wave kernel derives each tile's flat-decode parameters arithmetically with magic-number division, so the per-tile index and signature records no longer have to be written and read back. Only the non-pure groups are remapped through a gather map and handled by the existing tile-index, edge and rest kernels. The cost is more per-tile arithmetic and more code paths, and correctness now depends on the uniform-layout metadata captured during zstd decode.

```diff
diff --git a/naf_amd/csrc/ctx.h b/naf_amd/csrc/ctx.h
--- a/naf_amd/csrc/ctx.h
+++ b/naf_amd/csrc/ctx.h
@@ -16,7 +16,8 @@
 struct ZSplit { int parts; hipEvent_t ev[ZSPLIT_MAX]; u64 out_end[ZSPLIT_MAX]; int done; void *status; };
 struct FlatStream { u64 q0, A; };
 #define FLAT_DECODED (~0ull)
-struct ZFlat { const u8 *src; const FlatStream *si; u64 nslots; const u8 *sym; void *status; bool ready;
+struct ZFlatUni { bool ok; u32 np, regen0, per, n3, S, hso0, off[4]; u64 off0; };
+struct ZFlat { const u8 *src; const FlatStream *si; u64 nslots; const u8 *sym; void *status; bool ready; ZFlatUni uni;
                const u8 *tail; u64 tail_q; u32 tail_n;
                const u8 *cls; u32 n_decoded; u32 n_walk;
                struct naf_gpu_ctx *aux; hipEvent_t decoded_ev; void *later; };
diff --git a/naf_amd/csrc/emit.hip b/naf_amd/csrc/emit.hip
--- a/naf_amd/csrc/emit.hip
+++ b/naf_amd/csrc/emit.hip
@@ -740,10 +740,12 @@
 static_assert(sizeof(TileFlatE) == sizeof(TileFlat), "the derived record replaces the raw one in place");
 #define FLAT_QM 4096
 #define TILE_WG 255
-__global__ __launch_bounds__(256) void k_tile_index(EmitP P, u64 ntiles, TileIdx *ti, u64 *tr, u32 *list, u32 *count, TileFlat *tsig, u32 spare, u32 *list2)
+#define FLAT_TPW 8
+__global__ __launch_bounds__(256) void k_tile_index(EmitP P, u64 ntiles, TileIdx *ti, u64 *tr, u32 *list, u32 *count, TileFlat *tsig, u32 spare, u32 *list2, const u32 *gmap)
 {
     __shared__ u64 s_k[256], s_r[256];
-    const u64 t = (u64)blockIdx.x * TILE_WG + threadIdx.x;
+    const u64 t = (u64)(gmap ? gmap[blockIdx.x] : blockIdx.x) * TILE_WG + threadIdx.x;
+    const u64 ui = gmap ? (u64)blockIdx.x * TILE_WG + threadIdx.x : t, tri = gmap ? (u64)blockIdx.x * (TILE_WG + 1) + threadIdx.x : t;
     const u64 p = P.out_begin + t * 4096;
     TileIdx x; x.fast = 0; x.gline = 0; x.khi = 0; x.k = P.n_toggles; x.col = TI_HDR;
     TileFlat f; f.q0 = f.A = f.q1 = f.A1 = f.q2 = f.qf = 0;
@@ -791,15 +793,16 @@
     }
     s_k[threadIdx.x] = x.k; s_r[threadIdx.x] = r;
     __syncthreads();
-    if (threadIdx.x == TILE_WG) return;
+    if (threadIdx.x == TILE_WG) { if (gmap) tr[tri] = r; return; }
     TileFlatE e; e.base = (u64)P.fsrc; e.a1_addr = (u64)P.fsrc; e.a1_sh = 4; e.K0 = e.K1 = 0; e.d1 = e.d2 = 0x7FFFFFFFu; e.qoff = 0; e.par0 = 0; e.pad = 0;
+    if (gmap && blockIdx.x + 1 == gridDim.x && threadIdx.x < FLAT_TPW) { const u64 u = (u64)gridDim.x * TILE_WG + threadIdx.x; TileIdx z = x; z.fast = 0; ti[u] = z; if (tsig) *(TileFlatE *)&tsig[u] = e; }
     if (t >= ntiles) {
-        if (t == ntiles) { tr[t] = ~0ull; ti[t] = x; if (tsig && spare) *(TileFlatE *)&tsig[t] = e; }
-        else if (tsig && t < ntiles + spare) { ti[t].fast = 0; *(TileFlatE *)&tsig[t] = e; }
+        if (t == ntiles || gmap) { tr[tri] = ~0ull; ti[ui] = x; if (tsig && spare) *(TileFlatE *)&tsig[ui] = e; }
+        else if (tsig && t < ntiles + spare) { ti[ui].fast = 0; *(TileFlatE *)&tsig[ui] = e; }
         return;
     }
-    tr[t] = r;
-    if (!inside) { ti[t] = x; if (tsig) *(TileFlatE *)&tsig[t] = e; list[atomicAdd(count, 1u)] = (u32)t; return; }
+    tr[tri] = r;
+    if (!inside) { ti[ui] = x; if (tsig) *(TileFlatE *)&tsig[ui] = e; list[atomicAdd(count, 1u)] = (u32)ui; return; }
     const u64 r_next = s_r[threadIdx.x + 1];
     x.khi = s_k[threadIdx.x + 1];
     const bool wrap = P.mode == EM_FASTA && P.L != 0;
@@ -827,11 +830,11 @@
             const u64 t1 = (f.A1 < 40 ? 40 : f.A1) - 40;
             e.a1_addr = (u64)P.fsrc + (t1 >> 3); e.a1_sh = (u32)(t1 & 7) + 4;
         }
-        *(TileFlatE *)&tsig[t] = e;
+        *(TileFlatE *)&tsig[ui] = e;
     }
     x.fast = fast ? 1u : (packed ? 2u : 0u);
-    ti[t] = x;
-    if (!fast) { if (packed) list2[atomicAdd(count + 1, 1u)] = (u32)t; else list[atomicAdd(count, 1u)] = (u32)t; }
+    ti[ui] = x;
+    if (!fast) { if (packed) list2[atomicAdd(count + 1, 1u)] = (u32)ui; else list[atomicAdd(count, 1u)] = (u32)ui; }
 }
 
 template <bool FOURBIT>
@@ -991,7 +994,6 @@
     }
     pair[t] = v;
 }
-#define FLAT_TPW 8
 template <u32 TPW>
 __global__ __launch_bounds__(256) void k_emit_tile_flat(EmitP P, const TileIdx *ti, const TileFlat *tsig, u8 *out, u64 ntiles, u32 xcd_chunk)
 {
@@ -1105,32 +1107,11 @@
     }
 }
 
-template <u32 TW>
-__global__ __launch_bounds__(64) void k_emit_tile_flat_wave(EmitP P, const TileIdx *ti, const TileFlat *tsig, u8 *out, u64 ntiles, u32 xcd_chunk)
-{
-    u32 wg = blockIdx.x;
-    if (xcd_chunk) { wg = (blockIdx.x & 7u) * xcd_chunk + (blockIdx.x >> 3); if ((u64)wg * TW >= ntiles) return; }
-    __shared__ u64 s_tog[TW][EMIT_TOG_LDS];
-    __shared__ uint4 s_spl[32];
-    __shared__ u32 s_pair[256];
+template <u32 TW, bool MASK>
+__device__ __forceinline__ void flat_wave_tiles(const EmitP &P, const TileIdx (&A)[TW], const TileFlatE (&F)[TW], const bool (&live)[TW], const u64 (&tn)[TW], u8 *out,
+                                                u64 (*s_tog)[EMIT_TOG_LDS], const uint4 *s_spl, const u32 *s_pair)
+{
     const u32 lane = threadIdx.x;
-    if (lane < 32) s_spl[lane] = ((const uint4 *)(P.fpair + 272))[lane];
-    ((uint4 *)s_pair)[lane] = ((const uint4 *)(P.fpair + 16))[lane];
-    TileIdx A[TW]; TileFlatE F[TW]; bool live[TW];
-    {
-        const u64 t0 = (u64)wg * TW;
-        const uint4 *pa = (const uint4 *)(ti + t0), *pf = (const uint4 *)(tsig + t0);
-        uint4 ra[2 * TW], rf[3 * TW];
-#pragma unroll
-        for (u32 i = 0; i < 2 * TW; i++) ra[i] = pa[i];
-#pragma unroll
-        for (u32 i = 0; i < 3 * TW; i++) rf[i] = pf[i];
-#pragma unroll
-        for (u32 j = 0; j < TW; j++) {
-            __builtin_memcpy(&A[j], &ra[2 * j], 32); __builtin_memcpy(&F[j], &rf[3 * j], 48);
-            live[j] = t0 + j < ntiles && A[j].fast == 1;
-        }
-    }
     u64 X[TW][4]; u32 grels[TW][4], pk[TW][4];
 #pragma unroll
     for (u32 j = 0; j < TW; j++) {
@@ -1160,7 +1141,7 @@
             pk[j][r] = nl_b | ((need > rem ? rem : 16u) << 8) | ((off & 7u) << 16);
         }
     }
-    if (P.masking) {
+    if (MASK && P.masking) {
 #pragma unroll
         for (u32 j = 0; j < TW; j++) {
             const u64 nt = A[j].khi - A[j].k;
@@ -1170,11 +1151,10 @@
     __syncthreads();
 #pragma unroll
     for (u32 j = 0; j < TW; j++) {
-        const u64 t = (u64)wg * TW + j;
         if (!live[j]) continue;
         const TileIdx &a = A[j];
         const u32 ntog = (u32)(a.khi - a.k < EMIT_TOG_LDS ? a.khi - a.k : EMIT_TOG_LDS);
-        const bool use_tog = P.masking && a.k < a.khi && a.khi - a.k <= EMIT_TOG_LDS;
+        const bool use_tog = MASK && P.masking && a.k < a.khi && a.khi - a.k <= EMIT_TOG_LDS;
 #pragma unroll
         for (u32 r = 0; r < 4; r++) {
             const u64 g0 = a.gline + grels[j][r];
@@ -1197,8 +1177,10 @@
                 }
                 lo = (u64)w0 | ((u64)w1 << 32); hi = (u64)w2 | ((u64)w3 << 32);
             }
-            if (use_tog) mask16_from(s_tog[j], ntog, a.k, g0, lo, hi);
-            else mask16(P, a.k, a.khi, P.masking && a.k < a.khi, g0, lo, hi);
+            if (MASK) {
+                if (use_tog) mask16_from(s_tog[j], ntog, a.k, g0, lo, hi);
+                else mask16(P, a.k, a.khi, P.masking && a.k < a.khi, g0, lo, hi);
+            }
             uint4 v; v.x = (u32)lo; v.y = (u32)(lo >> 32); v.z = (u32)hi; v.w = (u32)(hi >> 32);
             if (nl < 16) {
                 const uint4 sel = s_spl[2 * nl], orv = s_spl[2 * nl + 1];
@@ -1206,15 +1188,157 @@
                 v.x = __builtin_amdgcn_perm(x0, 0u, sel.x) | orv.x; v.y = __builtin_amdgcn_perm(x1, x0, sel.y) | orv.y;
                 v.z = __builtin_amdgcn_perm(x2, x1, sel.z) | orv.z; v.w = __builtin_amdgcn_perm(x3, x2, sel.w) | orv.w;
             }
-            st_text16(out + t * 4096 + (r * 64 + lane) * 16, v, P.nt_store);
-        }
-    }
+            st_text16(out + tn[j] * 4096 + (r * 64 + lane) * 16, v, P.nt_store);
+        }
+    }
+}
+template <u32 TW>
+__global__ __launch_bounds__(64) void k_emit_tile_flat_wave(EmitP P, const TileIdx *ti, const TileFlat *tsig, u8 *out, u64 ntiles, u32 xcd_chunk, const u32 *gmap, u64 ntext)
+{
+    u32 wg = blockIdx.x;
+    if (xcd_chunk) { wg = (blockIdx.x & 7u) * xcd_chunk + (blockIdx.x >> 3); if ((u64)wg * TW >= ntiles) return; }
+    __shared__ u64 s_tog[TW][EMIT_TOG_LDS];
+    __shared__ uint4 s_spl[32];
+    __shared__ u32 s_pair[256];
+    const u32 lane = threadIdx.x;
+    if (lane < 32) s_spl[lane] = ((const uint4 *)(P.fpair + 272))[lane];
+    ((uint4 *)s_pair)[lane] = ((const uint4 *)(P.fpair + 16))[lane];
+    TileIdx A[TW]; TileFlatE F[TW]; bool live[TW]; u64 tn[TW];
+    {
+        const u64 t0 = (u64)wg * TW;
+        const uint4 *pa = (const uint4 *)(ti + t0), *pf = (const uint4 *)(tsig + t0);
+        uint4 ra[2 * TW], rf[3 * TW];
+#pragma unroll
+        for (u32 i = 0; i < 2 * TW; i++) ra[i] = pa[i];
+#pragma unroll
+        for (u32 i = 0; i < 3 * TW; i++) rf[i] = pf[i];
+#pragma unroll
+        for (u32 j = 0; j < TW; j++) {
+            __builtin_memcpy(&A[j], &ra[2 * j], 32); __builtin_memcpy(&F[j], &rf[3 * j], 48);
+            live[j] = t0 + j < ntiles && A[j].fast == 1;
+            tn[j] = t0 + j;
+            if (gmap) {
+                const u32 u = (u32)(t0 + j), ci = u / TILE_WG;
+                tn[j] = t0 + j < ntiles ? (u64)gmap[ci] * TILE_WG + (u - ci * TILE_WG) : 0;
+                live[j] = live[j] && tn[j] < ntext;
+            }
+        }
+    }
+    flat_wave_tiles<TW, true>(P, A, F, live, tn, out, s_tog, s_spl, s_pair);
+}
+
+struct SpanG { u64 gline0, blk; u32 col0, s0, pure, pad; };
+static_assert(sizeof(SpanG) == 32, "one scalar load per entry");
+struct SpanU { u32 wrap, L, Lp1, Lm, Lsh, regen0, Rm, Rsh, per, Pm, Psh, n3, S, off[4], np, hso0; u64 off0; };
+#define SPAN_LMAX (1u << 20)
+#define SPAN_NMIN (2048u + 32u)
+static void span_magic(u32 d, u32 *m, u32 *sh)
+{
+    u32 l = 0; while ((2u << l) <= d) l++;
+    const u32 s = (d & (d - 1)) ? l : l - 1;
+    *sh = s; *m = (u32)((((u64)1 << (32 + s)) + d - 1) / d);
+}
+__device__ __forceinline__ void span_tile(const EmitP &P, const SpanU &U, const SpanG &G, u32 i, bool live, TileIdx &a, TileFlatE &e)
+{
+    const u32 bo = i * 4096u;
+    u32 col = 0, glrel = bo, mc = 0;
+    if (U.wrap) {
+        const u32 c = G.col0 + bo, dline = __umulhi(c, U.Lm) >> U.Lsh;
+        col = c - dline * U.Lp1; glrel = dline * U.L; mc = col < U.L ? col : U.L;
+    }
+    a.gline = G.gline0 + glrel; a.col = col; a.k = 0; a.khi = 0; a.fast = live ? 1u : 0u;
+    const u32 pg = ((u32)G.gline0 & 1u) + glrel;
+    const u32 hg = pg >> 1, hq = (pg + mc) >> 1;
+    const u32 sym = G.s0 + hq;
+    const u32 db = __umulhi(sym, U.Rm) >> U.Rsh, so = sym - db * U.regen0;
+    u32 s = __umulhi(so, U.Pm) >> U.Psh; if (s > 3) s = 3;
+    const u32 w = so - s * U.per;
+    const u32 s2 = (s + 1) & 3u, db2 = db + (s == 3 ? 1u : 0u);
+    const u32 n1 = s == 3 ? U.n3 : U.per, n2 = s2 == 3 ? U.n3 : U.per;
+    const u32 o1 = s == 0 ? U.off[0] : s == 1 ? U.off[1] : s == 2 ? U.off[2] : U.off[3];
+    const u32 o2 = s2 == 0 ? U.off[0] : s2 == 1 ? U.off[1] : s2 == 2 ? U.off[2] : U.off[3];
+    const u32 d1 = n1 - w, d2 = d1 + n2;
+    const i32 a2 = (i32)(8u * (db2 * U.S + o2) + 4u * n2);
+    const i32 t0 = (i32)(8u * (db * U.S + o1) + 4u * d1), t1 = a2 + (i32)(4u * d1);
+    const i32 tmin = t1 < t0 ? t1 : t0;
+    const i32 ub = (tmin - 40 - 4 * FLAT_QM) & ~7;
+    const i32 ta = a2 - 40;
+    e.base = G.blk + (u64)(i64)(ub >> 3); e.K0 = (u32)(t0 - 40 - ub); e.K1 = (u32)(t1 - 40 - ub);
+    e.d1 = d1; e.d2 = d2; e.qoff = hg - hq; e.par0 = pg & 1u; e.pad = 0;
+    e.a1_addr = G.blk + (u64)(i64)(ta >> 3); e.a1_sh = (u32)(ta & 7) + 4;
+    if (!live) { e.base = (u64)P.fsrc; e.a1_addr = (u64)P.fsrc; e.a1_sh = 4; e.K0 = e.K1 = 0; e.d1 = e.d2 = 0x7FFFFFFFu; e.qoff = 0; e.par0 = 0; }
+}
+__global__ __launch_bounds__(64) void k_emit_span_wave(EmitP P, SpanU U, const SpanG *grp, u8 *out, u64 ntiles, u32 xcd_chunk)
+{
+    constexpr u32 TW = 2;
+    u32 wg = blockIdx.x;
+    if (xcd_chunk) { wg = (blockIdx.x & 7u) * xcd_chunk + (blockIdx.x >> 3); if ((u64)wg * TW >= ntiles) return; }
+    __shared__ uint4 s_spl[32];
+    __shared__ u32 s_pair[256];
+    const u32 lane = threadIdx.x;
+    if (lane < 32) s_spl[lane] = ((const uint4 *)(P.fpair + 272))[lane];
+    ((uint4 *)s_pair)[lane] = ((const uint4 *)(P.fpair + 16))[lane];
+    TileIdx A[TW]; TileFlatE F[TW]; bool live[TW]; u64 tn[TW];
+    SpanG G[TW];
+#pragma unroll
+    for (u32 j = 0; j < TW; j++) G[j] = grp[(wg * TW + j) / TILE_WG];
+#pragma unroll
+    for (u32 j = 0; j < TW; j++) {
+        const u32 t = wg * TW + j, gi = t / TILE_WG;
+        live[j] = t < ntiles && G[j].pure != 0;
+        tn[j] = t;
+        span_tile(P, U, G[j], t - gi * TILE_WG, live[j], A[j], F[j]);
+    }
+    flat_wave_tiles<TW, false>(P, A, F, live, tn, out, nullptr, s_spl, s_pair);
+}
+__global__ __launch_bounds__(256) void k_group_index(EmitP P, SpanU U, u64 ntiles, u32 ngroups, SpanG *grp, u32 *glist, u32 *gcount)
+{
+    const u32 g = blockIdx.x * 256 + threadIdx.x;
+    if (g > ngroups) return;
+    SpanG e; e.gline0 = 0; e.blk = (u64)P.fsrc; e.col0 = 0; e.s0 = 0; e.pure = 0; e.pad = 0;
+    if (g < ngroups) {
+        const u64 T0 = (u64)g * TILE_WG, span = (u64)TILE_WG * 4096;
+        const u64 p = P.out_begin + T0 * 4096, pn = p + span;
+        bool ok = T0 + TILE_WG < ntiles && pn < P.out_end;
+        u64 gl = 0, gg = 0, gn = 0; u32 col = 0;
+        if (ok) {
+            if (P.mode == EM_SEQ) { gl = gg = p; gn = pn; }
+            else {
+                const u64 r = upper_bound_u64(P.rec_out, 0, P.N + 1, p) - 1;
+                const u64 off = p - P.rec_out[r], hl = P.hdr_len[r], len = P.rec_len[r], rb = P.rec_base[r];
+                if (pn >= P.rec_out[r + 1] || off < hl) ok = false;
+                else {
+                    const u64 q = off - hl, qn = q + span; u64 j, jn;
+                    if (U.wrap) {
+                        const u64 line = q / U.Lp1, c = q - line * U.Lp1, linen = qn / U.Lp1, cn = qn - linen * U.Lp1;
+                        j = line * U.L + (c < U.L ? c : U.L); jn = linen * U.L + (cn < U.L ? cn : U.L);
+                        gl = rb + line * U.L; col = (u32)c;
+                    } else { j = q; jn = qn; gl = rb + q; }
+                    if (j > len || jn > len) ok = false;
+                    gg = rb + j; gn = rb + jn;
+                }
+            }
+        }
+        if (ok && P.masking) {
+            const u64 k0 = upper_bound_u64(P.toggles, 0, P.n_toggles, gg), k1 = upper_bound_u64(P.toggles, k0, P.n_toggles, gn);
+            if (k0 != k1 || (k0 & 1)) ok = false;
+        }
+        if (ok && (gn >> 1) + 2048 + 16 + U.regen0 >= (u64)U.np * U.regen0) ok = false;
+        if (ok) {
+            const u64 hq = gl >> 1, b0 = hq / U.regen0;
+            e.gline0 = gl; e.col0 = col; e.s0 = (u32)(hq - b0 * U.regen0); e.pure = 1;
+            e.blk = (u64)P.fsrc + U.off0 + b0 * U.S + 3 + U.hso0;
+        } else glist[atomicAdd(gcount, 1u)] = g;
+    }
+    grp[g] = e;
 }
 
 template <bool FOURBIT>
-__device__ __forceinline__ void emit_rest_tile(const EmitP &P, const TileIdx *ti, const u64 *tr, u64 t, u8 *out, u32 chunk)
+__device__ __forceinline__ void emit_rest_tile(const EmitP &P, const TileIdx *ti, const u64 *tr, u64 t, u8 *out, u32 chunk, const u32 *gmap)
 {
     const TileIdx a = ti[t];
+    if (gmap) { const u32 ci = (u32)t / TILE_WG, i = (u32)t - ci * TILE_WG; tr += (u64)ci * (TILE_WG + 1) + i; t = (u64)gmap[ci] * TILE_WG + i; }
+    else tr += t;
     u64 p0 = P.out_begin + t * 4096 + chunk * 16;
     if (p0 >= P.out_end) return;
     u32 nbytes = P.out_end - p0 < 16 ? (u32)(P.out_end - p0) : 16;
@@ -1224,17 +1348,17 @@
         for (u32 bb = 0; bb < nbytes; bb++) o[bb] = (u8)emit_byte<FOURBIT>(P, p0 + bb, 0, 0, a.k, a.khi);
         return;
     }
-    u64 rlo = tr[t], rhi = tr[t + 1] == ~0ull ? P.N - 1 : tr[t + 1];
+    u64 rlo = tr[0], rhi = tr[1] == ~0ull ? P.N - 1 : tr[1];
     u64 r = upper_bound_u64(P.rec_out, rlo, rhi + 1, p0) - 1;
     GeoGlobal geo_g(P);
     compose_chunk<FOURBIT>(P, geo_g, p0, nbytes, r, a.k, a.khi, P.masking && a.k < a.khi, Lp1_32, o);
 }
 #define EMIT_REST_GRID 4096
 template <bool FOURBIT>
-__global__ __launch_bounds__(64) void k_emit_rest(EmitP P, const TileIdx *ti, const u64 *tr, const u32 *list, const u32 *count, u8 *out)
+__global__ __launch_bounds__(64) void k_emit_rest(EmitP P, const TileIdx *ti, const u64 *tr, const u32 *list, const u32 *count, u8 *out, const u32 *gmap)
 {
     const u32 n = *count;
-    for (u32 i = blockIdx.x; i < 4 * n; i += gridDim.x) emit_rest_tile<FOURBIT>(P, ti, tr, list[i >> 2], out, (i & 3) * 64 + threadIdx.x);
+    for (u32 i = blockIdx.x; i < 4 * n; i += gridDim.x) emit_rest_tile<FOURBIT>(P, ti, tr, list[i >> 2], out, (i & 3) * 64 + threadIdx.x, gmap);
 }
 
 __global__ void k_range_bases(EmitP P, u64 *out2)
@@ -1301,6 +1425,67 @@
     if (total < N) return ctx_fail(c, NAF_GPU_EFORMAT, names ? "corrupted names - can't read name %llu\n" : "currupted ids - can't read id %llu\n", (unsigned long long)total);
     if (tiles) LAUNCH(c, "unnaf_zero_scatter", k_zero_scatter, tiles, 256, 0, d_buf, n, (const u64 *)cnt, pos, N);
     *out = pos;
+    return 0;
+}
+
+static int unnaf_emit_spans(naf_gpu_ctx *c, EmitP &P, ZFlat &zf, u64 ntiles, u8 *d_out, bool *done)
+{
+    *done = false;
+    const ZFlatUni &zu = zf.uni;
+    const bool wrap = P.mode == EM_FASTA && P.L != 0;
+    if (ctx_opt_is(c, "EMIT_SPAN", '0') || ctx_opt_is(c, "EMIT_WAVE", '0')) return 0;
+    if (!zu.ok || zf.cls || zf.later || P.force_slow || (P.mode != EM_FASTA && P.mode != EM_SEQ && P.mode != EM_SEQUENCES)) return 0;
+    if (wrap && (P.L < 16 || P.L + 1 > SPAN_LMAX)) return 0;
+    if (zu.per < SPAN_NMIN || zu.n3 < SPAN_NMIN || zu.regen0 != 3 * zu.per + zu.n3 || zu.regen0 > (1u << 17) || zu.S > (1u << 18)) return 0;
+    if (ntiles <= TILE_WG || ntiles >= 0x7FFFFFFFull) return 0;
+    if (P.masking && P.n_toggles >= ntiles) return 0;
+    const u32 ngroups = cdiv(ntiles, TILE_WG);
+    SpanU U; memset(&U, 0, sizeof U);
+    U.wrap = wrap ? 1u : 0u; U.L = wrap ? (u32)P.L : 0u; U.Lp1 = U.L + 1; if (wrap) span_magic(U.Lp1, &U.Lm, &U.Lsh);
+    U.regen0 = zu.regen0; span_magic(zu.regen0, &U.Rm, &U.Rsh); U.per = zu.per; span_magic(zu.per, &U.Pm, &U.Psh); U.n3 = zu.n3; U.S = zu.S;
+    for (int k = 0; k < 4; k++) U.off[k] = zu.off[k];
+    U.np = zu.np; U.hso0 = zu.hso0; U.off0 = zu.off0;
+    SpanG *grp = arena_new<SpanG>(c, (size_t)ngroups + 1); u32 *glist = arena_new<u32>(c, (size_t)ngroups + 2);
+    if (!grp || !glist) return NAF_GPU_ENOMEM;
+    u32 *gcount = glist + ngroups;
+    HIP_TRY(c, hipMemsetAsync(gcount, 0, 4, c->stream));
+    LAUNCH(c, "unnaf_group_index", k_group_index, cdiv((u64)ngroups + 1, 256), 256, 0, P, U, ntiles, ngroups, grp, glist, gcount);
+    u32 nmix = 0; int rc;
+    if ((rc = ctx_readback(c, &nmix, gcount, 4))) return rc;
+    if (nmix > ngroups) nmix = ngroups;
+    if (ctx_tracing(c)) ctx_trace(c, "[flat spans] groups %u pure %u mixed %u\n", ngroups, ngroups - nmix, nmix);
+    if (nmix == ngroups) return 0;
+    u32 *fpair = arena_new<u32>(c, 400); if (!fpair) return NAF_GPU_ENOMEM;
+    LAUNCH(c, "unnaf_flat_pair", k_flat_pair, 1, 256, 0, P, fpair);
+    P.fpair = fpair;
+    const u64 nmt = (u64)nmix * TILE_WG;
+    TileIdx *ti = nullptr; u64 *tr = nullptr; u32 *list = nullptr, *cnt = nullptr; TileFlat *tsig = nullptr;
+    naf_gpu_ctx *xc = c;
+    if (nmix) {
+        ti = arena_new<TileIdx>(c, nmt + 2 + FLAT_TPW); tr = arena_new<u64>(c, (u64)nmix * (TILE_WG + 1) + 2);
+        list = arena_new<u32>(c, nmt + 1); cnt = arena_new<u32>(c, 2); tsig = arena_new<TileFlat>(c, nmt + 2 + FLAT_TPW);
+        if (!ti || !tr || !list || !cnt || !tsig) return NAF_GPU_ENOMEM;
+        HIP_TRY(c, hipMemsetAsync(cnt, 0, 8, c->stream));
+        if (zf.aux) {
+            HIP_TRY(c, hipEventRecord(c->split_ev[0], c->stream));
+            HIP_TRY(c, hipStreamWaitEvent(zf.aux->stream, c->split_ev[0], 0));
+            xc = zf.aux;
+        }
+        LAUNCH(xc, "unnaf_tile_index", k_tile_index, nmix, 256, 0, P, ntiles, ti, tr, list, cnt, tsig, (u32)FLAT_TPW, list, (const u32 *)glist);
+    }
+    { const u32 ch = (cdiv(ntiles, 2u) + 7) / 8; LAUNCH(c, "unnaf_emit_flat", k_emit_span_wave, ch * 8, 64, 0, P, U, (const SpanG *)grp, d_out, ntiles, ch); }
+    if (nmix) {
+        const u32 ch = (cdiv(nmt, 2u) + 7) / 8;
+        LAUNCH(xc, "unnaf_emit_flat_edge", k_emit_tile_flat_wave<2>, ch * 8, 64, 0, P, (const TileIdx *)ti, (const TileFlat *)tsig, d_out, nmt, ch, (const u32 *)glist, ntiles);
+        const u32 rest_grid = 4u * (u32)(nmt < EMIT_REST_GRID ? nmt : EMIT_REST_GRID);
+        LAUNCH(xc, "unnaf_emit_rest", k_emit_rest<true>, rest_grid, 64, 0, P, (const TileIdx *)ti, (const u64 *)tr, (const u32 *)list, (const u32 *)cnt, d_out, (const u32 *)glist);
+        if (xc != c) { HIP_TRY(c, hipEventRecord(c->split_ev[1], xc->stream)); HIP_TRY(c, hipStreamWaitEvent(c->stream, c->split_ev[1], 0)); }
+        if (ctx_tracing(c)) {
+            u32 hc[2] = { 0, 0 };
+            if (!ctx_readback(c, hc, cnt, 8)) ctx_trace(c, "[flat tiles] total %llu rest %u decoded %u\n", (unsigned long long)ntiles, hc[0], hc[1]);
+        }
+    }
+    *done = true;
     return 0;
 }
 
@@ -1872,13 +2057,16 @@
             else LAUNCH(c, "unnaf_emit", k_emit<false>, grid, 256, 0, pl.P, d_out);
         } else {
             u64 ntiles = cdiv(m_end - m_begin, 4096);
+            u64 Lp1 = pl.P.L + 1;
+            pl.P.Ldiv_magic = (Lp1 >= 2 && Lp1 < 32768) ? (u32)((1ull << 32) / Lp1 + 1) : 0;
+            bool span_done = false;
+            if (zflat.ready && !split.done && (rc = unnaf_emit_spans(c, pl.P, zflat, ntiles, d_out, &span_done))) return rc;
+            if (!span_done) {
             TileIdx *ti = arena_new<TileIdx>(c, ntiles + 2 + FLAT_TPW); u64 *tr = arena_new<u64>(c, ntiles + 2);
             u32 *list = arena_new<u32>(c, ntiles + 1), *cnt = arena_new<u32>(c, 2);
             u32 *list2 = (zflat.ready && zflat.cls) ? arena_new<u32>(c, ntiles + 1) : list;
             if (!ti || !tr || !list || !cnt || !list2) return NAF_GPU_ENOMEM;
             if (!split.done) HIP_TRY(c, hipMemsetAsync(cnt, 0, 8, c->stream));
-            u64 Lp1 = pl.P.L + 1;
-            pl.P.Ldiv_magic = (Lp1 >= 2 && Lp1 < 32768) ? (u32)((1ull << 32) / Lp1 + 1) : 0;
             naf_gpu_ctx *ic = split.done ? c->side2 : c;
             const bool tile_wave = !(ctx_opt(c, "EMIT_WAVE") && ctx_opt(c, "EMIT_WAVE")[0] == '0');
             if (split.done) HIP_TRY(c, hipMemsetAsync(cnt, 0, 8, ic->stream));
@@ -1888,7 +2076,7 @@
                 LAUNCH(ic, "unnaf_flat_pair", k_flat_pair, 1, 256, 0, pl.P, fpair);
                 pl.P.fpair = fpair;
             }
-            LAUNCH(ic, "unnaf_tile_index", k_tile_index, cdiv(ntiles + 1 + FLAT_TPW, TILE_WG), 256, 0, pl.P, ntiles, ti, tr, list, cnt, tsig, (u32)FLAT_TPW, list2);
+            LAUNCH(ic, "unnaf_tile_index", k_tile_index, cdiv(ntiles + 1 + FLAT_TPW, TILE_WG), 256, 0, pl.P, ntiles, ti, tr, list, cnt, tsig, (u32)FLAT_TPW, list2, (const u32 *)nullptr);
             naf_gpu_ctx *xc = c;
             const bool flat_job = zflat.ready && zflat.later;
             if (zflat.ready && zflat.aux) {
@@ -1918,8 +2106,8 @@
                 const char *ew = ctx_opt(c, "EMIT_WAVE");
                 const bool mixed = flat_job || (zflat.cls && zflat.n_decoded);
                 const bool wave = !(ew && ew[0] == '0') && (!mixed || zflat.n_walk == 0);
-                if (wave && pl.P.masking && pl.P.n_toggles >= ntiles) { const u32 ch = ((u32)ntiles + 7) / 8; LAUNCH(c, "unnaf_emit_flat", k_emit_tile_flat_wave<1>, ch * 8, 64, 0, pl.P, (const TileIdx *)ti, (const TileFlat *)tsig, d_out, (u64)ntiles, ch); }
-                else if (wave) { const u32 ch = (cdiv(ntiles, 2u) + 7) / 8; LAUNCH(c, "unnaf_emit_flat", k_emit_tile_flat_wave<2>, ch * 8, 64, 0, pl.P, (const TileIdx *)ti, (const TileFlat *)tsig, d_out, (u64)ntiles, ch); }
+                if (wave && pl.P.masking && pl.P.n_toggles >= ntiles) { const u32 ch = ((u32)ntiles + 7) / 8; LAUNCH(c, "unnaf_emit_flat", k_emit_tile_flat_wave<1>, ch * 8, 64, 0, pl.P, (const TileIdx *)ti, (const TileFlat *)tsig, d_out, (u64)ntiles, ch, (const u32 *)nullptr, (u64)ntiles); }
+                else if (wave) { const u32 ch = (cdiv(ntiles, 2u) + 7) / 8; LAUNCH(c, "unnaf_emit_flat", k_emit_tile_flat_wave<2>, ch * 8, 64, 0, pl.P, (const TileIdx *)ti, (const TileFlat *)tsig, d_out, (u64)ntiles, ch, (const u32 *)nullptr, (u64)ntiles); }
                 else
                 LAUNCH(c, "unnaf_emit_flat", k_emit_tile_flat<4>, chunk * 8, 256, 0, pl.P, (const TileIdx *)ti, (const TileFlat *)tsig, d_out, (u64)ntiles, chunk);
                 if (flat_job) {
@@ -1940,13 +2128,14 @@
                 else LAUNCH(c, "unnaf_emit", k_emit_tile<false>, (u32)(ntiles - t_done), 256, 0, pl.P, (const TileIdx *)(ti + t_done), d_out + t_done * 4096);
             }
             const u32 rest_grid = 4u * (u32)(ntiles < EMIT_REST_GRID ? ntiles : EMIT_REST_GRID);
-            if (pl.fourbit) LAUNCH(xc, "unnaf_emit_rest", k_emit_rest<true>, rest_grid, 64, 0, pl.P, (const TileIdx *)ti, (const u64 *)tr, (const u32 *)list, (const u32 *)cnt, d_out);
-            else LAUNCH(xc, "unnaf_emit_rest", k_emit_rest<false>, rest_grid, 64, 0, pl.P, (const TileIdx *)ti, (const u64 *)tr, (const u32 *)list, (const u32 *)cnt, d_out);
+            if (pl.fourbit) LAUNCH(xc, "unnaf_emit_rest", k_emit_rest<true>, rest_grid, 64, 0, pl.P, (const TileIdx *)ti, (const u64 *)tr, (const u32 *)list, (const u32 *)cnt, d_out, (const u32 *)nullptr);
+            else LAUNCH(xc, "unnaf_emit_rest", k_emit_rest<false>, rest_grid, 64, 0, pl.P, (const TileIdx *)ti, (const u64 *)tr, (const u32 *)list, (const u32 *)cnt, d_out, (const u32 *)nullptr);
             if (xc != c) { HIP_TRY(c, hipEventRecord(c->split_ev[1], xc->stream)); HIP_TRY(c, hipStreamWaitEvent(c->stream, c->split_ev[1], 0)); }
             if (split.done) HIP_TRY(c, hipStreamWaitEvent(c->stream, c->split_ev[ZSPLIT_MAX + 1], 0));
             if (zflat.ready && ctx_tracing(c)) {
                 u32 hc[2] = { 0, 0 };
                 if (!ctx_readback(c, hc, cnt, 8)) ctx_trace(c, "[flat tiles] total %llu rest %u decoded %u\n", (unsigned long long)ntiles, hc[0], hc[1]);
+            }
             }
         }
     }
diff --git a/naf_amd/csrc/zstd_dec.hip b/naf_amd/csrc/zstd_dec.hip
--- a/naf_amd/csrc/zstd_dec.hip
+++ b/naf_amd/csrc/zstd_dec.hip
@@ -3443,6 +3443,9 @@
                         const u32 tn = hu.last_raw & 0x7FFFFFFFu; const bool rle = (hu.last_raw >> 31) != 0;
                         zf->tail = flat_tail ? d_src + (hs.end_off - (rle ? 1u : tn)) : nullptr; zf->tail_q = hu.total_out - (flat_tail ? tn : 0u);
                         zf->tail_n = flat_tail ? (rle ? tn | 0x80000000u : tn) : 0u;
+                        ZFlatUni &zu = zf->uni;
+                        zu.ok = hu.nstreams0 == 4; zu.np = hu.np; zu.regen0 = hu.regen0; zu.per = hu.per; zu.n3 = hu.n[3]; zu.S = S; zu.hso0 = hu.hso0; zu.off0 = fh.hdr_size;
+                        for (int k = 0; k < 4; k++) zu.off[k] = hu.off[k];
                         if (rg) { rg->got_lo = 0; rg->got_hi = hu.total_out; rg->ranged = false; }
                         *out_len = hu.total_out;
                         if (fh.has_fcs && fh.content_size != hu.total_out) return zerr(c, ZE_CORRUPT, "content size mismatch");
diff --git a/naf_amd/synth.py b/naf_amd/synth.py
--- a/naf_amd/synth.py
+++ b/naf_amd/synth.py
@@ -95,6 +95,31 @@
         body[:, width] = 10
         pos += rows_per * (width + 1)
     return out
+
+
+def fasta_records_device(lengths, width: int = 80, seed: int = 1, device="cuda", lower=()):
+    import torch
+    lut = torch.tensor(list(b"ACGT"), dtype=torch.uint8, device=device)
+    parts = []
+    for k, n in enumerate(lengths):
+        g = torch.Generator(device=device)
+        g.manual_seed(seed * 1000003 + k)
+        bases = lut[torch.randint(0, 4, (n,), dtype=torch.int64, device=device, generator=g)]
+        for r, a, b in lower:
+            if r == k:
+                bases[a:b] |= 0x20
+        parts.append(torch.tensor(list(b">span%d record of %d bases\n" % (k, n)), dtype=torch.uint8, device=device))
+        w = width if width else n
+        rows, rem = n // w, n % w
+        body = torch.empty(rows * (w + 1) + (rem + 1 if rem else 0), dtype=torch.uint8, device=device)
+        full = body[:rows * (w + 1)].view(rows, w + 1)
+        full[:, :w] = bases[:rows * w].view(rows, w)
+        full[:, w] = 10
+        if rem:
+            body[rows * (w + 1):-1] = bases[rows * w:]
+            body[-1] = 10
+        parts.append(body)
+    return torch.cat(parts)
 
 
 def fastq_reads_device(total_bytes: int, read_len: int = 150, seed: int = 7, device="cuda", chunk_reads: int = 1 << 22):
```

New measurement: 4311 GB/s (median of 6 runs). +1.5%, better.
